# frank-xwang/InstanceDiffusion

Measured on AMD Instinct MI355X. Metric: images/sec at 512x512, 50 PLMS steps, N=8 instances (Multi-instance Sampler), higher is better.
Workload: dtype bf16; 1 GPU; C3: SD-1.5 InstanceDiffusion UNet (1.228B params, seeded random weights), 64x64 latent (512x512), 50 PLMS steps, CFG 7.5, N=8 boxes, MIS 0.36, alpha [0.8,0,0.2]; images_per_gpu=32, unet_forwards_per_image=406

## Files before the change

include/idf.h:

```cpp
#ifndef IDF_H_
#define IDF_H_

#include <stdint.h>

#ifdef __cplusplus
extern "C" {
#endif

#define IDF_ABI_VERSION 5

enum { IDF_BF16 = 0, IDF_F16 = 1 };
enum { IDF_E_ARG = -1, IDF_E_ALIGN = -2, IDF_E_UNSUPPORTED = -3 };

enum {
  IDF_EPI_BIAS     = 1,
  IDF_EPI_ROWBIAS  = 2,
  IDF_EPI_RES      = 4,
  IDF_EPI_GATE     = 8,
  IDF_EPI_SILU     = 16,
  IDF_EPI_GELU     = 32,
  IDF_EPI_GEGLU    = 64,
  IDF_EPI_OUT_F32  = 128,
  IDF_EPI_OUT_NCHW = 256,
  IDF_EPI_LN_ROW   = 512,
  IDF_EPI_LN_COL   = 1024,
  IDF_EPI_GEGLU_P32 = 2048,
  IDF_EPI_QUICKGELU = 4096
};

int idf_abi_version(void);
const char* idf_build_info(void);

enum { IDF_TUNE_GEMM_BIG = 0, IDF_TUNE_ATTN2 = 1, IDF_TUNE_GEMM_RING = 2, IDF_TUNE_BIG_MIN_EFF = 3, IDF_TUNE_ATTN8 = 4, IDF_TUNE_MLP = 5,
       IDF_TUNE_QKV_ROW = 6, IDF_TUNE_GEGLU_ROW = 7, IDF_TUNE_PROJ_ROW = 9  };
int idf_set_tuning(int knob, int value);
enum { IDF_STAT_GEMM_BIG_LAUNCHES = 0, IDF_STAT_ATTN2_LAUNCHES = 1, IDF_STAT_GEMM_RING_LAUNCHES = 2, IDF_STAT_ATTN8_LAUNCHES = 3,
       IDF_STAT_GN_EPI_LAUNCHES = 4 ,
       IDF_STAT_QKV_ROW_LAUNCHES = 6 ,
       IDF_STAT_GEGLU_ROW_LAUNCHES = 7 ,
       IDF_STAT_PROJ_ROW_LAUNCHES = 8 ,
       IDF_STAT_PROJ_ROW_MIN_M = 9 ,
       IDF_STAT_ATTN_RES_LAUNCHES = 10 ,
       IDF_STAT_CLIP_PREPROC_LAUNCHES = 12  };
long long idf_get_stat(int stat);

typedef struct {
  const void* A; const void* W; void* out;
  const float* bias; const void* rowbias; const void* res; const float* gate;
  int M, N, K;
  int lda, ldw, ldo, ldr, ld_rowbias;
  int rows_per_batch;
  int batch; long long strideA, strideW, strideO, strideR;
  int epi; int dtype;
  void* ws; long long ws_bytes;
  const float* ln_stats; long long stride_ln_stats;
  const float* ln_c;
  const float* ln_d;
  float* out_stats; float out_stats_eps;
  float ln_eps; float* ln_stats_out;
  void* vt_out; int ld_vt; int vt_col0;
} idf_gemm_args;
int idf_gemm(const idf_gemm_args* a, void* stream);

typedef struct {
  const void* x; int ldx;
  const float* ln_stats;
  const void* w1; int ldw1;
  const float* cd;
  const void* w2p; int ldw2;
  const float* b2;
  const float* gate;
  void* out; int ldo;
  int M, C;
  int dtype;
} idf_mlp_args;
int idf_mlp_geglu(const idf_mlp_args* a, void* stream);

int idf_row_stats(const void* x, int ldx, float* stats, int M, int C, float eps, int dtype, void* stream);

typedef struct {
  const void* x; const void* W; void* out;
  const float* bias; const void* rowbias; const void* res;
  int B, Hin, Win, Cin, Cout;
  int stride;
  int upsample;
  int ldx, ldo, ldr, ld_rowbias;
  int n_valid;
  int epi; int dtype;
  void* ws; long long ws_bytes;
  float* gn_partial;
} idf_conv3x3_args;
int idf_conv3x3(const idf_conv3x3_args* a, void* stream);
int idf_conv3x3_down(const idf_conv3x3_args* a, void* stream);
int idf_conv_up2x_folded(const idf_conv3x3_args* a, void* stream);

int idf_conv_in(const float* x_nchw, const float* w , const float* bias, void* out,
                int B, int Cin, int H, int W, int Cout, int dtype, void* stream);

typedef struct {
  const void* q; int ldq; long long strideQ; int nq;
  const void* k0; int ldk0; long long strideK0; const void* vt0; int ldv0; long long strideV0; int n0;
  const void* k1; int ldk1; long long strideK1; const void* vt1; int ldv1; long long strideV1; int n1;
  void* out; int ldo; long long strideO;
  int B, H, d;
  float scale;
  int dtype;
  const void* qbits; long long strideQb;
  const void* kbits0; long long strideKb0;
  const void* kbits1; long long strideKb1;
} idf_attn_args;
int idf_attention(const idf_attn_args* a, void* stream);

long long idf_groupnorm_ws_floats(int B, int HW);
int idf_groupnorm(const void* x, void* out, const float* gamma, const float* beta, float* ws,
                  int B, int HW, int C, float eps, int silu, int dtype, void* stream);
int idf_groupnorm_stats(const void* x, float* partial, int B, int HW, int C, int nchunks, int dtype, void* stream);
int idf_groupnorm_apply(const void* x, void* out, const float* gamma, const float* beta, const float* partial,
                        int B, int HW, int C, int nchunks, float eps, int silu, int dtype, void* stream);

int idf_layernorm(const void* x, int ldx, void* out, int ldo, const float* gamma, const float* beta,
                  int M, int C, float eps, int dtype, void* stream);

int idf_layernorm_patch2(const void* x, void* out, int ldo, const float* gamma, const float* beta,
                         int B, int H, int W, int C, float eps, int dtype, void* stream);

int idf_seg_in_conv(const float* segs, const float* w , const float* bias, void* out,
                    int B, int Cin, int S, int ldo, int dtype, void* stream);
int idf_dwconv7x7(const void* x, const float* w_tap_major, const float* bias, void* out, int B, int H, int W, int C,
                  int dtype, void* stream);

int idf_scaleu_concat(const void* h, const void* skip, void* out, const float* hscale, const float* sm1,
                      float* ws, int B, int H, int W, int Ch, int Cs, int dtype, void* stream);

int idf_timestep_embedding(const float* t, void* out, int B, int dim, int dtype, void* stream);

int idf_unifusion_embed(const float* text, const float* loc, const float* tmask, const float* lmask,
                        const float* null_text, const float* null_loc, const float* freqs , void* out,
                        int rows, int text_dim, int D, int dtype, void* stream);

int idf_cfg_combine(const float* eps_cond, const float* eps_uncond, float guidance, float* e_t,
                    long long n, void* stream);
int idf_plms_update(const float* x, const float* e_t, const float* e1, const float* e2, const float* e3,
                    const float* e_next, int mode, float a_t, float a_prev, float sqrt_1m_at,
                    float* x_out, long long n, void* stream);

int idf_ddim_update(const float* x, const float* eps_cond, const float* eps_uncond , float guidance,
                    float a_t, float a_prev, float sigma_t, float sqrt_1m_at, const float* noise ,
                    float* x_prev, float* pred_x0 , long long n, void* stream);
int idf_q_sample_blend(const float* x0, const float* noise, const float* mask, const float* img, float sqrt_ac, float sqrt_1m_ac,
                       float* out, int B, int C, long long HW, int mask_channels , void* stream);
int idf_ddim_update_units(const float* x, const float* eps_cond, const float* eps_uncond , float guidance,
                          float a_t, float a_prev, float sigma_t, float sqrt_1m_at, const float* noise ,
                          const int* img_of , float* x_prev, float* pred_x0 , int U, int B,
                          long long chw, void* stream);
int idf_q_sample_blend_units(const float* x0, const float* noise, const float* mask, const float* img, const int* img_of,
                             float sqrt_ac, float sqrt_1m_ac, float* out, int U, int B, int C, long long HW,
                             int mask_channels , void* stream);

int idf_dpmpp_update(const float* x, const float* eps_cond, const float* eps_uncond , float guidance,
                     float sqrt_at, float sqrt_1m_at, float c_x, float c_0, float c_1,
                     const float* x0_last ,
                     float* x_prev, float* x0_out , long long n, void* stream);

int idf_mis_merge(const float* lat, const int* boxes, float* out, int n_inst, int B, int C, int H, int W,
                  int mode, void* stream);
int idf_mis_merge_ragged(const float* lat, const int* unit_off, const int* boxes , float* out, int B, int U,
                         int C, int H, int W, int mode, void* stream);

int idf_softmax_rows(const float* s, void* p, long long rows, int n, long long lds, long long ldp, float scale,
                     int dtype, void* stream);
int idf_pointwise_nchw(const float* x, const float* w , const float* bias, float* out, int B, int Cin,
                       int Cout, long long HW, float in_scale, void* stream);

int idf_vae_posterior(const float* h, const float* w , const float* bias, const float* noise, float scale, float* z,
                      float* moments, int B, int C2, int E, long long HW, void* stream);

int idf_attention_causal(const void* qkv, int ld, void* out, int ldo, int B, int T, int H, int d, float scale, int dtype, void* stream);
int idf_clip_embed(const int* ids, const void* tok_emb, const void* pos_emb, void* out, int ldo, int B, int T, int C, int vocab,
                   int dtype, void* stream);

#define IDF_ATTENTION_QKV_TMAX 288
int idf_attention_qkv(const void* qkv, int ld, void* out, int ldo, int B, int T, int H, int d, float scale, int dtype, void* stream);
int idf_clip_patchify(const float* pixels, void* patches, int ldp, const void* cls_row, void* x, int ldx, int B, int S, int P, int C,
                      int dtype, void* stream);

enum { IDF_CLIP_SRC_U8 = 0, IDF_CLIP_SRC_F32 = 1 };
#define IDF_CLIP_RESIZE_KMAX 32
int idf_clip_crop_resize(const void* src, int kind, int B, int H, int W, const int* crops, int Ncrop, const int* tables, int Ntab,
                         const float* lut, float* out, int S, int K, void* stream);

int idf_rle_decode_planes(const unsigned* ends, int n_ends, const int* run_begin, const int* run_end, const int* src_hw,
                          const int* dst_plane, int M, float* out, int P, int S, int* area, void* stream);

int idf_cast_f32_to_16(const float* x, void* out, long long n, int dtype, void* stream);

#ifdef __cplusplus
}
#endif
#endif
```

instancediffusion_amd/_lib.py:

```python
from __future__ import annotations

import ctypes as C
import os

_HERE = os.path.dirname(os.path.abspath(__file__))
LIB_PATH = os.environ.get("IDF_LIB_PATH", os.path.join(_HERE, "libidf_gfx950.so"))

IDF_BF16, IDF_F16 = 0, 1
IDF_STAT_GEMM_BIG_LAUNCHES, IDF_STAT_ATTN2_LAUNCHES, IDF_STAT_GEMM_RING_LAUNCHES, IDF_STAT_ATTN8_LAUNCHES, IDF_STAT_GN_EPI_LAUNCHES = 0, 1, 2, 3, 4
IDF_STAT_QKV_ROW_LAUNCHES, IDF_STAT_GEGLU_ROW_LAUNCHES = 6, 7
IDF_STAT_PROJ_ROW_LAUNCHES, IDF_STAT_PROJ_ROW_MIN_M = 8, 9
IDF_STAT_ATTN_RES_LAUNCHES = 10
IDF_STAT_CLIP_PREPROC_LAUNCHES = 12
IDF_CLIP_SRC_U8, IDF_CLIP_SRC_F32 = 0, 1
CLIP_RESIZE_KMAX = 32
IDF_TUNE_PROJ_ROW = 9
IDF_TUNE_GEMM_BIG, IDF_TUNE_ATTN2, IDF_TUNE_GEMM_RING, IDF_TUNE_BIG_MIN_EFF, IDF_TUNE_ATTN8, IDF_TUNE_MLP, IDF_TUNE_QKV_ROW, IDF_TUNE_GEGLU_ROW = 0, 1, 2, 3, 4, 5, 6, 7
EPI_LN_ROW, EPI_LN_COL, EPI_GEGLU_P32, EPI_QUICKGELU = 512, 1024, 2048, 4096
EPI_BIAS, EPI_ROWBIAS, EPI_RES, EPI_GATE, EPI_SILU, EPI_GELU, EPI_GEGLU, EPI_OUT_F32, EPI_OUT_NCHW = \
    1, 2, 4, 8, 16, 32, 64, 128, 256

vp, ll, ci, cf = C.c_void_p, C.c_longlong, C.c_int, C.c_float


class GemmArgs(C.Structure):
    _fields_ = [("A", vp), ("W", vp), ("out", vp), ("bias", vp), ("rowbias", vp), ("res", vp), ("gate", vp),
                ("M", ci), ("N", ci), ("K", ci),
                ("lda", ci), ("ldw", ci), ("ldo", ci), ("ldr", ci), ("ld_rowbias", ci),
                ("rows_per_batch", ci),
                ("batch", ci), ("strideA", ll), ("strideW", ll), ("strideO", ll), ("strideR", ll),
                ("epi", ci), ("dtype", ci), ("ws", vp), ("ws_bytes", ll),
                ("ln_stats", vp), ("stride_ln_stats", ll), ("ln_c", vp), ("ln_d", vp),
                ("out_stats", vp), ("out_stats_eps", cf),
                ("ln_eps", cf), ("ln_stats_out", vp),
                ("vt_out", vp), ("ld_vt", ci), ("vt_col0", ci)]


E_UNSUPPORTED = -3
ATTENTION_QKV_TMAX = 288


class ConvArgs(C.Structure):
    _fields_ = [("x", vp), ("W", vp), ("out", vp), ("bias", vp), ("rowbias", vp), ("res", vp),
                ("B", ci), ("Hin", ci), ("Win", ci), ("Cin", ci), ("Cout", ci),
                ("stride", ci), ("upsample", ci),
                ("ldx", ci), ("ldo", ci), ("ldr", ci), ("ld_rowbias", ci),
                ("n_valid", ci), ("epi", ci), ("dtype", ci), ("ws", vp), ("ws_bytes", ll), ("gn_partial", vp)]


class AttnArgs(C.Structure):
    _fields_ = [("q", vp), ("ldq", ci), ("strideQ", ll), ("nq", ci),
                ("k0", vp), ("ldk0", ci), ("strideK0", ll), ("vt0", vp), ("ldv0", ci), ("strideV0", ll), ("n0", ci),
                ("k1", vp), ("ldk1", ci), ("strideK1", ll), ("vt1", vp), ("ldv1", ci), ("strideV1", ll), ("n1", ci),
                ("out", vp), ("ldo", ci), ("strideO", ll),
                ("B", ci), ("H", ci), ("d", ci), ("scale", cf), ("dtype", ci),
                ("qbits", vp), ("strideQb", ll), ("kbits0", vp), ("strideKb0", ll), ("kbits1", vp), ("strideKb1", ll)]


class MlpArgs(C.Structure):
    _fields_ = [("x", vp), ("ldx", ci), ("ln_stats", vp), ("w1", vp), ("ldw1", ci), ("cd", vp), ("w2p", vp), ("ldw2", ci),
                ("b2", vp), ("gate", vp), ("out", vp), ("ldo", ci), ("M", ci), ("C", ci), ("dtype", ci)]


SYMBOLS = {
    "idf_abi_version": (ci, []),
    "idf_build_info": (C.c_char_p, []),
    "idf_set_tuning": (ci, [ci, ci]),
    "idf_get_stat": (ll, [ci]),
    "idf_gemm": (ci, [C.POINTER(GemmArgs), vp]),
    "idf_conv3x3": (ci, [C.POINTER(ConvArgs), vp]),
    "idf_conv3x3_down": (ci, [C.POINTER(ConvArgs), vp]),
    "idf_conv_up2x_folded": (ci, [C.POINTER(ConvArgs), vp]),
    "idf_mlp_geglu": (ci, [C.POINTER(MlpArgs), vp]),
    "idf_conv_in": (ci, [vp, vp, vp, vp, ci, ci, ci, ci, ci, ci, vp]),
    "idf_attention": (ci, [C.POINTER(AttnArgs), vp]),
    "idf_groupnorm_ws_floats": (ll, [ci, ci]),
    "idf_groupnorm": (ci, [vp, vp, vp, vp, vp, ci, ci, ci, cf, ci, ci, vp]),
    "idf_groupnorm_stats": (ci, [vp, vp, ci, ci, ci, ci, ci, vp]),
    "idf_groupnorm_apply": (ci, [vp, vp, vp, vp, vp, ci, ci, ci, ci, cf, ci, ci, vp]),
    "idf_layernorm": (ci, [vp, ci, vp, ci, vp, vp, ci, ci, cf, ci, vp]),
    "idf_row_stats": (ci, [vp, ci, vp, ci, ci, cf, ci, vp]),
    "idf_layernorm_patch2": (ci, [vp, vp, ci, vp, vp, ci, ci, ci, ci, cf, ci, vp]),
    "idf_seg_in_conv": (ci, [vp, vp, vp, vp, ci, ci, ci, ci, ci, vp]),
    "idf_dwconv7x7": (ci, [vp, vp, vp, vp, ci, ci, ci, ci, ci, vp]),
    "idf_scaleu_concat": (ci, [vp, vp, vp, vp, vp, vp, ci, ci, ci, ci, ci, ci, vp]),
    "idf_timestep_embedding": (ci, [vp, vp, ci, ci, ci, vp]),
    "idf_unifusion_embed": (ci, [vp, vp, vp, vp, vp, vp, vp, vp, ci, ci, ci, ci, vp]),
    "idf_cfg_combine": (ci, [vp, vp, cf, vp, ll, vp]),
    "idf_plms_update": (ci, [vp, vp, vp, vp, vp, vp, ci, cf, cf, cf, vp, ll, vp]),
    "idf_ddim_update": (ci, [vp, vp, vp, cf, cf, cf, cf, cf, vp, vp, vp, ll, vp]),
    "idf_q_sample_blend": (ci, [vp, vp, vp, vp, cf, cf, vp, ci, ci, ll, ci, vp]),
    "idf_ddim_update_units": (ci, [vp, vp, vp, cf, cf, cf, cf, cf, vp, vp, vp, vp, ci, ci, ll, vp]),
    "idf_q_sample_blend_units": (ci, [vp, vp, vp, vp, vp, cf, cf, vp, ci, ci, ci, ll, ci, vp]),
    "idf_dpmpp_update": (ci, [vp, vp, vp, cf, cf, cf, cf, cf, cf, vp, vp, vp, ll, vp]),
    "idf_mis_merge": (ci, [vp, vp, vp, ci, ci, ci, ci, ci, ci, vp]),
    "idf_mis_merge_ragged": (ci, [vp, vp, vp, vp, ci, ci, ci, ci, ci, ci, vp]),
    "idf_cast_f32_to_16": (ci, [vp, vp, ll, ci, vp]),
    "idf_softmax_rows": (ci, [vp, vp, ll, ci, ll, ll, cf, ci, vp]),
    "idf_pointwise_nchw": (ci, [vp, vp, vp, vp, ci, ci, ci, ll, cf, vp]),
    "idf_vae_posterior": (ci, [vp, vp, vp, vp, cf, vp, vp, ci, ci, ci, ll, vp]),
    "idf_attention_causal": (ci, [vp, ci, vp, ci, ci, ci, ci, ci, cf, ci, vp]),
    "idf_clip_embed": (ci, [vp, vp, vp, vp, ci, ci, ci, ci, ci, ci, vp]),
    "idf_attention_qkv": (ci, [vp, ci, vp, ci, ci, ci, ci, ci, cf, ci, vp]),
    "idf_clip_patchify": (ci, [vp, vp, ci, vp, vp, ci, ci, ci, ci, ci, ci, vp]),
    "idf_clip_crop_resize": (ci, [vp, ci, ci, ci, ci, vp, ci, vp, ci, vp, vp, ci, ci, vp]),
    "idf_rle_decode_planes": (ci, [vp, ci, vp, vp, vp, vp, ci, vp, ci, ci, vp, vp]),
}

_lib = None


def load() -> C.CDLL:
    global _lib
    if _lib is not None:
        return _lib
    if not os.path.exists(LIB_PATH):
        raise RuntimeError(
            f"{LIB_PATH} is missing: the MI355X HIP extension has not been built "
            f"(run instancediffusion_amd/csrc/build.sh or __graft_entry__.build()). "
            f"There is no CPU fallback for the InstanceDiffusion sampling path.")
    import torch
    lib = C.CDLL(LIB_PATH)
    for name, (res, args) in SYMBOLS.items():
        fn = getattr(lib, name)
        fn.restype = res
        fn.argtypes = args
    if lib.idf_abi_version() != 5:
        raise RuntimeError("libidf_gfx950.so ABI version mismatch")
    _lib = lib
    return lib


class IdfError(RuntimeError):
    pass


def check(status: int, what: str):
    if status != 0:
        kind = {-1: "invalid argument", -2: "misaligned pointer/leading dimension", -3: "unsupported"}.get(
            status, f"hipError_t {status}")
        raise IdfError(f"{what} failed: {kind}")
```

instancediffusion_amd/csrc/gemm_big.hip:

```cpp
#include "gemm_core.h"
#include <cstdlib>

using namespace idfcore;

namespace {

IDF_ZERO_PAGE(idf_zero_page);

constexpr int WM = 64, TM = 2, NWAVES = 8;

template <int I> struct IC { static constexpr int value = I; };
template <int I, int N, int STEP, class F> __device__ __forceinline__ void static_for(F&& f) {
  if constexpr (I < N) { f(IC<I>{}); static_for<I + STEP, N, STEP>(f); }
}

template <int N, int L>
__device__ __forceinline__ void gst_scatter_step(float* t, int l31) {
  constexpr int H = N / 2;
  const bool up = (l31 & H) != 0;
#pragma unroll
  for (int i = 0; i < H; ++i) {
    const float keep = up ? t[i + H] : t[i];
    const float send = up ? t[i] : t[i + H];
    t[i] = keep + __shfl_xor(send, H, 64);
  }
}
__device__ __forceinline__ void swap16(const f32x16& c, float* v) {
#pragma unroll
  for (int e = 0; e < 4; ++e) {
    const auto s02 = __builtin_amdgcn_permlane32_swap(__float_as_uint(c[e]), __float_as_uint(c[8 + e]), false, false);
    const auto s13 = __builtin_amdgcn_permlane32_swap(__float_as_uint(c[4 + e]), __float_as_uint(c[12 + e]), false, false);
    v[e] = __uint_as_float(s02[0]); v[4 + e] = __uint_as_float(s02[1]);
    v[8 + e] = __uint_as_float(s13[0]); v[12 + e] = __uint_as_float(s13[1]);
  }
}
template <int DT, int BM, int BN, int TN, bool SPLIT, bool LNS = false, bool STATS = false, bool GLU = false, bool GST = false,
          bool QG = true >
__device__ __forceinline__ void big_epilogue(const CoreParams& p, f32x16 (&acc)[TN][TM], int seq, int slice, int tiles_n, int wm,
                                             int wn, int l31_in, int hi_in, float gate, char* stg_in, const float* lnm = nullptr,
                                             const float* lnr = nullptr) {
  constexpr int WN = BN / 2;
  const int epi = p.epi;
  int l31 = l31_in, hi = hi_in;
  asm volatile("" : "+v"(l31), "+v"(hi));
  char* const stg = stg_in;
  const int m_tile = seq / tiles_n;
  const int n0 = (seq - m_tile * tiles_n) * BN, m0 = m_tile * BM;
  const int mw = m0 + wm * WM, nw = n0 + wn * WN;
  if constexpr (LNS) {
    if (p.ln_stats_out && n0 == 0 && wn == 0 && hi == 0) {
#pragma unroll
      for (int b = 0; b < TM; ++b) {
        const int m = mw + b * 32 + l31;
        if (m < p.M) *reinterpret_cast<f32x2*>(p.ln_stats_out + 2 * (size_t)m) = f32x2{lnm[b], lnr[b]};
      }
    }
  }
  if constexpr (SPLIT) {
    static_for<0, TN, 1>([&](auto AI) {
      constexpr int a = decltype(AI)::value;
      const int n = nw + a * 32 + 16 * hi;
#pragma unroll
      for (int b = 0; b < TM; ++b) {
        float v[16];
        swap16(acc[a][b], v);
        const int m = mw + b * 32 + l31;
        if (m >= p.M) continue;
        float* o = p.ws + ((size_t)slice * p.tail_rows + (m - p.tail_m0)) * p.N + n;
#pragma unroll
        for (int j = 0; j < 4; ++j) *reinterpret_cast<f32x4*>(o + 4 * j) = f32x4{v[4 * j], v[4 * j + 1], v[4 * j + 2], v[4 * j + 3]};
      }
    });
    return;
  }
  if (GLU || (((TN & 1) == 0) && (epi & IDF_EPI_GEGLU) && (epi & IDF_EPI_GEGLU_P32))) {
   if constexpr (GLU || ((TN & 1) == 0)) {
#pragma unroll
    for (int b = 0; b < TM; ++b) {
     static_for<0, TN, 1>([&](auto AI) {
      constexpr int a = decltype(AI)::value;
      const int npk = nw + a * 32;
      {
        float o[8];
        f32x2 st = {0.0f, 1.0f};
        if (epi & IDF_EPI_LN_ROW) {
          const int mr = min(mw + b * 32 + l31, p.M - 1);
          if constexpr (LNS) st = f32x2{lnm[b], lnr[b]};
          else st = *reinterpret_cast<const f32x2*>(p.ln_stats + 2 * (size_t)mr);
        }
#pragma unroll
        for (int q = 0; q < 2; ++q) {
          const f32x4 bv = *reinterpret_cast<const f32x4*>(p.bias + npk + 8 * q + 4 * hi);
          const f32x4 bg = *reinterpret_cast<const f32x4*>(p.bias + npk + 16 + 8 * q + 4 * hi);
          f32x4 cv = {0.f, 0.f, 0.f, 0.f}, cg = {0.f, 0.f, 0.f, 0.f};
          if (epi & IDF_EPI_LN_ROW) {
            cv = *reinterpret_cast<const f32x4*>(p.ln_c + npk + 8 * q + 4 * hi);
            cg = *reinterpret_cast<const f32x4*>(p.ln_c + npk + 16 + 8 * q + 4 * hi);
          }
#pragma unroll
          for (int e = 0; e < 4; ++e) {
            float val = acc[a][b][4 * q + e], gat = acc[a][b][4 * (q + 2) + e];
            if (epi & IDF_EPI_LN_ROW) {
              val = fmaf(st[1], fmaf(-st[0], cv[e], val), bv[e]);
              gat = fmaf(st[1], fmaf(-st[0], cg[e], gat), bg[e]);
            } else {
              val += bv[e];
              gat += bg[e];
            }
            o[4 * q + e] = val * gelu_erf_f(gat);
          }
        }
        float v[8];
#pragma unroll
        for (int e = 0; e < 4; ++e) {
          const auto sw = __builtin_amdgcn_permlane32_swap(__float_as_uint(o[e]), __float_as_uint(o[4 + e]), false, false);
          v[e] = __uint_as_float(sw[0]); v[4 + e] = __uint_as_float(sw[1]);
        }
        const int m = mw + b * 32 + l31;
        unsigned short* const obase = reinterpret_cast<unsigned short*>(p.out);
        if (m < p.M) {
          unsigned short* op = obase + (size_t)m * p.ldo + (npk >> 1) + 8 * hi;
          *reinterpret_cast<u32x4*>(op) = pack8<DT>(v);
        }
      }
     });
    }
   }
  } else if (!GLU && (epi & IDF_EPI_GEGLU)) {
    if constexpr (!GLU && (TN & 1) == 0) {
      static_for<0, TN, 2>([&](auto AI) {
        constexpr int a = decltype(AI)::value;
        const int npk = nw + a * 32;
        f32x4 bv[4], bg[4], cv[4], cg[4];
#pragma unroll
        for (int q = 0; q < 4; ++q) {
          bv[q] = *reinterpret_cast<const f32x4*>(p.bias + npk + 8 * q + 4 * hi);
          bg[q] = *reinterpret_cast<const f32x4*>(p.bias + npk + 32 + 8 * q + 4 * hi);
          if (epi & IDF_EPI_LN_ROW) {
            cv[q] = *reinterpret_cast<const f32x4*>(p.ln_c + npk + 8 * q + 4 * hi);
            cg[q] = *reinterpret_cast<const f32x4*>(p.ln_c + npk + 32 + 8 * q + 4 * hi);
          }
        }
#pragma unroll
        for (int b = 0; b < TM; ++b) {
          f32x16 o;
          if (epi & IDF_EPI_LN_ROW) {
            const int mr = min(mw + b * 32 + l31, p.M - 1);
            f32x2 st;
            if constexpr (LNS) st = f32x2{lnm[b], lnr[b]};
            else st = *reinterpret_cast<const f32x2*>(p.ln_stats + 2 * (size_t)mr);
#pragma unroll
            for (int q = 0; q < 4; ++q)
#pragma unroll
              for (int e = 0; e < 4; ++e) {
                const float val = fmaf(st[1], fmaf(-st[0], cv[q][e], acc[a][b][4 * q + e]), bv[q][e]);
                const float gat = fmaf(st[1], fmaf(-st[0], cg[q][e], acc[a + 1][b][4 * q + e]), bg[q][e]);
                o[4 * q + e] = val * gelu_erf_f(gat);
              }
          } else {
#pragma unroll
          for (int q = 0; q < 4; ++q)
#pragma unroll
            for (int e = 0; e < 4; ++e)
              o[4 * q + e] = (acc[a][b][4 * q + e] + bv[q][e]) * gelu_erf_f(acc[a + 1][b][4 * q + e] + bg[q][e]);
          }
          float v[16];
          swap16(o, v);
          const int m = mw + b * 32 + l31;
          if (m < p.M) {
            unsigned short* op = reinterpret_cast<unsigned short*>(p.out) + (size_t)m * p.ldo + (npk >> 1) + 16 * hi;
            *reinterpret_cast<u32x4*>(op) = pack8<DT>(v);
            *reinterpret_cast<u32x4*>(op + 8) = pack8<DT>(v + 8);
          }
        }
      });
    }
  } else if constexpr (!GLU) {
    float st_p[TM], st_s1[TM], st_s2[TM];
#pragma unroll
    for (int b = 0; b < TM; ++b) { st_p[b] = 0.0f; st_s1[b] = 0.0f; st_s2[b] = 0.0f; }
    float gacc[GST ? TN : 1];
    static_for<0, TN, 1>([&](auto AI) {
      constexpr int a = decltype(AI)::value;
      const int n = nw + a * 32 + 16 * hi;
      f32x4 bs[4], cs[4];
      float gt[GST ? 32 : 1];
      if (epi & IDF_EPI_BIAS) {
#pragma unroll
        for (int j = 0; j < 4; ++j) bs[j] = *reinterpret_cast<const f32x4*>(p.bias + n + 4 * j);
      }
      if (epi & IDF_EPI_LN_ROW) {
#pragma unroll
        for (int j = 0; j < 4; ++j) cs[j] = *reinterpret_cast<const f32x4*>(p.ln_c + n + 4 * j);
      }
#pragma unroll
// ... 107 lines not shown
#pragma unroll
      for (int a = 0; a < TN; ++a) csl[(l31 >> 4) * WNC + a * 32 + 16 * hi + (l31 & 15)] = gacc[a];
      asm volatile("s_waitcnt lgkmcnt(0)" ::: "memory");
      __builtin_amdgcn_wave_barrier();
      const int cpg = p.N >> 5;
      const int g = l31 + 32 * hi;
      if (g * cpg < WNC && mw < p.M) {
        constexpr float rows = (float)WM, inv_rows = 1.0f / (float)WM;
        const float inv_cpg = 1.0f / (float)cpg;
        float ms = 0.f, q = 0.f;
        for (int j = 0; j < cpg; ++j) {
          const int col = g * cpg + j;
          const float s1 = csl[col], s2 = csl[WNC + col];
          float pc = (epi & IDF_EPI_BIAS) ? p.bias[nw + col] : 0.0f;
          if (epi & IDF_EPI_ROWBIAS)
            pc += Elem<DT>::to_f32(p.rowbias[(size_t)(mw / p.rows_per_batch) * p.ld_rowbias + nw + col]);
          const float dm = s1 * inv_rows;
          ms += pc + dm;
          q += fmaxf(s2 - s1 * dm, 0.0f);
        }
        const float mean = ms * inv_cpg;
        float dev = 0.f;
        for (int j = 0; j < cpg; ++j) {
          const int col = g * cpg + j;
          float pc = (epi & IDF_EPI_BIAS) ? p.bias[nw + col] : 0.0f;
          if (epi & IDF_EPI_ROWBIAS)
            pc += Elem<DT>::to_f32(p.rowbias[(size_t)(mw / p.rows_per_batch) * p.ld_rowbias + nw + col]);
          const float dd = pc + csl[col] * inv_rows - mean;
          dev = fmaf(dd, dd, dev);
        }
        const int smp = mw / p.gn_hw, chunk = (mw - smp * p.gn_hw) / WM, nch = p.gn_hw / WM;
        *reinterpret_cast<f32x2*>(p.gn_partial + (((size_t)smp * nch + chunk) * 32 + nw / cpg + g) * 2) =
            f32x2{mean, fmaf(rows, dev, q)};
      }
      __builtin_amdgcn_wave_barrier();
    }
    if constexpr (STATS) {
      constexpr float cnt = 16.0f * TN;
      const int n_tile = (seq - m_tile * tiles_n);
#pragma unroll
      for (int b = 0; b < TM; ++b) {
        const float mean = st_p[b] + st_s1[b] * (1.0f / cnt);
        const float m2 = fmaxf(st_s2[b] - st_s1[b] * st_s1[b] * (1.0f / cnt), 0.0f);
        const float mean_o = __shfl_xor(mean, 32, 64), m2_o = __shfl_xor(m2, 32, 64);
        const float dlt = mean_o - mean;
        const int m = mw + b * 32 + l31;
        if (hi == 0 && m < p.M)
          *reinterpret_cast<f32x2*>(p.stat_parts + ((size_t)m * p.parts + n_tile * 2 + wn) * 2) =
              f32x2{0.5f * (mean + mean_o), m2 + m2_o + dlt * dlt * (0.5f * cnt)};
      }
    }
  }
}

template <int DT, int BM, int BN, int TN>
__device__ __forceinline__ void big_epilogue_vt(const CoreParams& p, f32x16 (&acc)[TN][TM], int seq, int tiles_n, int wm, int wn,
                                                int l31, int hi, const float* stats , int stats_row0) {
  constexpr int WN = BN / 2;
  const int epi = p.epi;
  const int m_tile = seq / tiles_n;
  const int n0 = (seq - m_tile * tiles_n) * BN, m0 = m_tile * BM;
  const int mw = m0 + wm * WM, nw = n0 + wn * WN;
  static_for<0, TN, 1>([&](auto AI) {
    constexpr int a = decltype(AI)::value;
    const int n = nw + a * 32 + l31;
    const float cn = (epi & IDF_EPI_LN_ROW) ? p.ln_c[n] : 0.0f;
    const float bn = (epi & IDF_EPI_BIAS) ? p.bias[n] : 0.0f;
    unsigned short* orow = p.vt_out + (size_t)(n - p.vt_col0) * p.ld_vt;
#pragma unroll
    for (int b = 0; b < TM; ++b) {
#pragma unroll
      for (int half = 0; half < 2; ++half) {
        float v[8];
#pragma unroll
        for (int e = 0; e < 4; ++e) {
          const auto sw = __builtin_amdgcn_permlane32_swap(__float_as_uint(acc[a][b][4 * half + e]),
                                                           __float_as_uint(acc[a][b][4 * half + 8 + e]), false, false);
          v[e] = __uint_as_float(sw[0]); v[4 + e] = __uint_as_float(sw[1]);
        }
        const int mb = mw + b * 32 + 16 * hi + 8 * half;
        if (epi & IDF_EPI_LN_ROW) {
          const f32x4* st4 = reinterpret_cast<const f32x4*>(stats + 2 * (size_t)(min(mb, p.M - 8) - stats_row0));
#pragma unroll
          for (int j = 0; j < 4; ++j) {
            const f32x4 t = st4[j];
            v[2 * j] = t[1] * fmaf(-t[0], cn, v[2 * j]);
            v[2 * j + 1] = t[3] * fmaf(-t[2], cn, v[2 * j + 1]);
          }
        }
#pragma unroll
        for (int j = 0; j < 8; ++j) v[j] += bn;
        if (mb < p.M) *reinterpret_cast<u32x4*>(orow + mb) = pack8<DT>(v);
      }
    }
  });
}

template <int DT, int BM, int BN, int TN>
__device__ __forceinline__ void big_epilogue_fold(const CoreParams& p, f32x16 (&acc)[TN][TM], int tile, int ph, int tiles_n, int wm,
                                                  int wn, int l31_in, int hi_in) {
  constexpr int WN = BN / 2;
  int l31 = l31_in, hi = hi_in;
  asm volatile("" : "+v"(l31), "+v"(hi));
  const int m_tile = tile / tiles_n;
  const int n0 = (tile - m_tile * tiles_n) * BN, m0 = m_tile * BM;
  const int mw = m0 + wm * WM, nw = n0 + wn * WN;
  const int ph_row = (ph >> 1) * 2 * p.Wo + (ph & 1);
  unsigned short* orow[TM];
#pragma unroll
  for (int b = 0; b < TM; ++b) {
    const int m = min(mw + b * 32 + l31, p.M - 1);
    const int x = m % p.Wo;
    orow[b] = reinterpret_cast<unsigned short*>(p.out) + (size_t)(4 * m - 2 * x + ph_row) * p.ldo;
  }
  static_for<0, TN, 1>([&](auto AI) {
    constexpr int a = decltype(AI)::value;
    const int n = nw + a * 32 + 16 * hi;
    f32x4 bs[4];
    if (p.epi & IDF_EPI_BIAS) {
#pragma unroll
      for (int j = 0; j < 4; ++j) bs[j] = *reinterpret_cast<const f32x4*>(p.bias + n + 4 * j);
    }
#pragma unroll
    for (int b = 0; b < TM; ++b) {
      float v[16];
      swap16(acc[a][b], v);
      if (p.epi & IDF_EPI_BIAS) {
#pragma unroll
        for (int j = 0; j < 16; ++j) v[j] += bs[j >> 2][j & 3];
      }
      if (mw + b * 32 + l31 < p.M) {
        *reinterpret_cast<u32x4*>(orow[b] + n) = pack8<DT>(v);
        *reinterpret_cast<u32x4*>(orow[b] + n + 8) = pack8<DT>(v + 8);
      }
    }
  });
}

#ifdef IDF_BIG_TRACE
__device__ unsigned long long idf_big_trace_buf[4][8];
#define TR_DECL unsigned long long tr_last = __builtin_readcyclecounter(), tr_acc[8] = {0, 0, 0, 0, 0, 0, 0, 0};
#define TR(i) { const unsigned long long tr_now = __builtin_readcyclecounter(); tr_acc[i] += tr_now - tr_last; tr_last = tr_now; }
#define TR_COUNT(i) { tr_acc[i] += 1; }
#define TR_DUMP { const int trb = blockIdx.x == 0 ? 0 : ((int)blockIdx.x == (int)gridDim.x / 2 ? 1 : -1);                     \
    if (trb >= 0 && lane == 0 && (wave == 0 || wave == NWAVES / 2)) { for (int i = 0; i < 8; ++i) idf_big_trace_buf[trb * 2 + (wave ? 1 : 0)][i] = tr_acc[i]; } }
#else
#define TR_DECL
#define TR(i)
#define TR_COUNT(i)
#define TR_DUMP
#endif

template <int DT, int BM, int BN, int BKT, int NSTG, bool CONV, bool SPLIT, bool LNS = false, bool VT = false, bool STATS = false,
          bool GLU = false, bool GST = false, bool FOLD = false>
__global__ __launch_bounds__(64 * NWAVES, 1) void gemm_kernel_big(const CoreParams p, const int tiles_total) {
  constexpr int WN = BN / 2, TN = WN / 32;
  constexpr int NW = NWAVES;
  constexpr int RS = BKT;
  constexpr int CPR = BKT / 8;
  constexpr int RPI = 64 / CPR;
  constexpr int W_INST = BN / (RPI * NW), A_INST = BM / (RPI * NW);
  constexpr int DPW = W_INST + A_INST;
  constexpr int STAGE = (BM + BN) * RS;
  static_assert(BN % (RPI * NW) == 0 && BM % (RPI * NW) == 0, "tile rows must split evenly over the DMA instructions");
  extern __shared__ __attribute__((aligned(16))) unsigned short smem[];

  const int tid = threadIdx.x;
  const int lane = tid & 63, wave = __builtin_amdgcn_readfirstlane(tid >> 6);
  const int l31 = lane & 31, hi = lane >> 5;
  const int wn = wave & 1, wm = wave >> 1;
  const int G = gridDim.x;
  const int slot = ((G & 7) == 0) ? (int)(blockIdx.x & 7) * (G >> 3) + (int)(blockIdx.x >> 3) : (int)blockIdx.x;
  const int tiles_n = p.N / BN;
  int seq_step = G, seq_end = tiles_total, seq0 = slot;
  if (!SPLIT && p.tile_walk == 1 && tiles_total > G) {
    const int q = tiles_total / G, r = tiles_total - q * G;
    seq0 = slot * q + min(slot, r);
    seq_end = seq0 + q + (slot < r ? 1 : 0);
    seq_step = 1;
  }
  const int S = SPLIT ? p.splitk : 1;
  const int nk = p.kt_per_slice;
  const int full = SPLIT ? p.full_items : tiles_total;
  auto item_map = [&](int item, int& tile, int& slice, int& nki) {
    if (!SPLIT || item < full) { tile = item; slice = 0; nki = SPLIT ? p.kt_full : nk; }
    else { const int r = item - full; const int t = r / S; tile = full + t; slice = r - t * S; nki = nk; }
  };

  const int dr = lane / CPR, dc = lane % CPR;
  auto swz = [](int row) { return CPR == 8 ? ((row >> 1) & 7) : ((row >> 2) & 3); };
  unsigned woff[W_INST], aoff[A_INST];
  int ayx[A_INST];
  int l_seq, l_kt = 0, l_k0 = 0, l_nk = 0, tap = 0, ci0 = 0;

  auto setup_loader = [&](int item) {
    int tile, slice;
    item_map(item, tile, slice, l_nk);
    [[maybe_unused]] int ph = 0;
    if constexpr (FOLD) { ph = tile / p.fold_tiles; tile -= ph * p.fold_tiles; }
    const int m_tile = tile / tiles_n;
    const int n0 = (tile - m_tile * tiles_n) * BN, m0 = m_tile * BM;
    l_k0 = slice * nk;
#pragma unroll
    for (int j = 0; j < W_INST; ++j) {
      const int row = RPI * (wave + NW * j) + dr;
      if constexpr (FOLD) woff[j] = (unsigned)(ph * p.N + n0 + row) * (unsigned)p.ldw + (unsigned)((dc ^ swz(row)) * 8);
      else woff[j] = (unsigned)(n0 + row) * (unsigned)p.ldw + (unsigned)((dc ^ swz(row)) * 8);
    }
#pragma unroll
    for (int j = 0; j < A_INST; ++j) {
      const int row = RPI * (wave + NW * j) + dr;
      const int m = min(m0 + row, p.M - 1);
      const unsigned sw = (unsigned)((dc ^ swz(row)) * 8);
      if (CONV) {
        const auto [b, yo, xo] = conv_pixel(p, m);
        if constexpr (FOLD) {
          const int y0 = yo - 1 + (ph >> 1), x0 = xo - 1 + (ph & 1);
          int mask = 0;
#pragma unroll
          for (int t = 0; t < 4; ++t) {
            const int yi = y0 + (t >> 1), xi = x0 + (t & 1);
            mask |= ((yi >= 0) & (yi < p.Hin) & (xi >= 0) & (xi < p.Win)) << t;
          }
          ayx[j] = mask;
          aoff[j] = (unsigned)b * (unsigned)(p.Hin * p.Win) * (unsigned)p.lda + (unsigned)((y0 * p.Win + x0) * p.lda) + sw;
          continue;
        }
        const int y0 = yo * p.stride - p.pad_lo, x0 = xo * p.stride - p.pad_lo;
        if (p.up == 0) {
          int mask = 0;
#pragma unroll
          for (int t = 0; t < 9; ++t) {
            const int yi = y0 + t / 3, xi = x0 + t % 3;
            mask |= ((yi >= 0) & (yi < p.Hin) & (xi >= 0) & (xi < p.Win)) << t;
          }
          ayx[j] = mask;
          aoff[j] = (unsigned)b * (unsigned)(p.Hin * p.Win) * (unsigned)p.lda + (unsigned)((y0 * p.Win + x0) * p.lda) + sw;
        } else {
          ayx[j] = (y0 << 16) | (x0 & 0xffff);
          aoff[j] = (unsigned)b * (unsigned)(p.Hin * p.Win) * (unsigned)p.lda + sw;
        }
      } else {
        ayx[j] = 0;
        aoff[j] = (unsigned)m * (unsigned)p.lda + sw;
      }
    }
    if (CONV) conv_tap_at(p, l_k0 * BKT, tap, ci0);
  };

  auto issue_piece = [&](int stage, auto II) {
    constexpr int i = decltype(II)::value;
    unsigned short* Al = smem + stage * STAGE;
    if constexpr (i < W_INST) {
      constexpr int j = i;
      dma16_sv(p.W + (size_t)(l_k0 + l_kt) * BKT, woff[j] * 2u, lds_addr(Al + BM * RS + RPI * (wave + NW * j) * RS));
    } else {
      constexpr int j = i - W_INST;
      const unsigned dst = lds_addr(Al + RPI * (wave + NW * j) * RS);
      if constexpr (FOLD) {
        const unsigned tapoff = (unsigned)(((tap >> 1) * p.Win + (tap & 1)) * p.lda + ci0);
        const bool ok = (ayx[j] >> tap) & 1;
        const unsigned short* src = ok ? p.A + (aoff[j] + tapoff) : idf_zero_page + dc * 8;
        dma16_v(src, dst);
      } else if (CONV && p.up == 0) {
        const int ky = tap / 3, kx = tap - ky * 3;
        const unsigned tapoff = (unsigned)((ky * p.Win + kx) * p.lda + ci0);
        const bool ok = (ayx[j] >> tap) & 1;
        const unsigned short* src = ok ? p.A + (aoff[j] + tapoff) : idf_zero_page + dc * 8;
        dma16_v(src, dst);
      } else if (CONV) {
        const int ky = tap / 3, kx = tap - ky * 3;
        const int Hup = p.Hin << p.up, Wup = p.Win << p.up;
        const int yi = (ayx[j] >> 16) + ky, xi = (int)(short)(ayx[j] & 0xffff) + kx;
        const bool ok = conv_tap_inside(yi, xi, Hup, Wup);
        const int ys = yi >> p.up, xs = xi >> p.up;
        const unsigned short* src = ok ? p.A + ci0 + (aoff[j] + (unsigned)(ys * p.Win + xs) * (unsigned)p.lda) : idf_zero_page + dc * 8;
        dma16_v(src, dst);
      } else {
        dma16_sv(p.A + (size_t)(l_k0 + l_kt) * BKT, aoff[j] * 2u, dst);
      }
    }
  };
  auto advance_loader = [&]() {
    if (CONV) conv_tap_step(p, BKT, tap, ci0);
    if (++l_kt == l_nk) {
      l_kt = 0;
      l_seq += seq_step;
      if (l_seq < seq_end) setup_loader(l_seq);
    }
  };
  auto issue_dma = [&](int stage) {
    static_for<0, DPW, 1>([&](auto II) { issue_piece(stage, II); });
    advance_loader();
  };

  const int f_sw = swz(l31);
  int issued = 0;
  constexpr int NPOS = (BKT / 16) * TN;
  constexpr bool OLD_LATE = BN == 320;
  constexpr int LATE_POS = OLD_LATE ? NPOS * 7 / 8 : NPOS / 2;
  auto compute = [&](auto SWAPT, f32x16 (&acc)[TN][TM], float (&lsx)[TM], float (&lsq)[TM], int stage, bool late_fill, int st_fill) {
    constexpr bool SWAP = decltype(SWAPT)::value;
    const unsigned short* Al = smem + stage * STAGE;
    const unsigned short* Wl = Al + BM * RS;
    const unsigned short* af_base = Al + (wm * WM + l31) * RS;
    const unsigned short* wf_base = Wl + (wn * WN + l31) * RS;
    u32x4 wf[2][TN], af[2][TM];
    {
      const int s8 = (hi ^ f_sw) * 8;
#pragma unroll
      for (int a = 0; a < TN; ++a) wf[0][a] = *reinterpret_cast<const u32x4*>(wf_base + a * 32 * RS + s8);
#pragma unroll
      for (int b = 0; b < TM; ++b) af[0][b] = *reinterpret_cast<const u32x4*>(af_base + b * 32 * RS + s8);
    }
    static_for<0, BKT / 16, 1>([&](auto KS) {
      constexpr int ks = decltype(KS)::value;
      constexpr int cur = ks & 1, nxt = cur ^ 1;
      if constexpr (ks + 1 < BKT / 16) {
        const int s8 = (((ks + 1) * 2 + hi) ^ f_sw) * 8;
#pragma unroll
        for (int a = 0; a < TN; ++a) wf[nxt][a] = *reinterpret_cast<const u32x4*>(wf_base + a * 32 * RS + s8);
#pragma unroll
        for (int b = 0; b < TM; ++b) af[nxt][b] = *reinterpret_cast<const u32x4*>(af_base + b * 32 * RS + s8);
      }
      static_for<0, TN, 1>([&](auto AI) {
        constexpr int a = decltype(AI)::value;
        constexpr int pos = ks * TN + a;
#pragma unroll
        for (int b = 0; b < TM; ++b) {
          if constexpr (SWAP) acc[a][b] = Elem<DT>::mfma32(af[cur][b], wf[cur][a], acc[a][b]);
          else acc[a][b] = Elem<DT>::mfma32(wf[cur][a], af[cur][b], acc[a][b]);
        }
        if constexpr (LNS && a == 0) {
#pragma unroll
          for (int b = 0; b < TM; ++b)
#pragma unroll
            for (int w = 0; w < 4; ++w) {
              Elem<DT>::dot2c(lsx[b], af[cur][b][w], Elem<DT>::ONES2);
              Elem<DT>::dot2c(lsq[b], af[cur][b][w], af[cur][b][w]);
            }
        }
        if constexpr (pos == LATE_POS - 1) {
          if (late_fill) static_for<0, DPW, 1>([&](auto II) { issue_piece(st_fill, II); });
        }
      });
    });
    if (late_fill) { advance_loader(); ++issued; }
  };

  int seq = seq0;
  if (seq >= seq_end) return;
  if (p.dephase > 1) {
    const int ph = (int)(blockIdx.x >> 3) % p.dephase;
    const int units = ph * p.dephase_units / p.dephase;
    for (int i = 0; i < units; ++i) __builtin_amdgcn_s_sleep(16);
  }
  l_seq = seq;
  setup_loader(l_seq);
#pragma unroll
  for (int j = 0; j < NSTG - 1; ++j)
    if (l_seq < seq_end) { issue_dma(j); ++issued; }
  int it = 0, st_it = 0;
  int young_stores = 0;
  TR_DECL
  const int epi = p.epi;
  const float gate = (epi & IDF_EPI_GATE) ? p.gate[0] : 0.0f;
  char* const stg = reinterpret_cast<char*>(smem + NSTG * STAGE) + wave * 2048;

  auto run_tile = [&](auto SWAPT, auto SPLT) {
    constexpr bool SWAP = decltype(SWAPT)::value;
    constexpr bool SPL = decltype(SPLT)::value;
    int tile, slice, nki;
    item_map(seq, tile, slice, nki);
    [[maybe_unused]] int ph = 0;
    if constexpr (FOLD) { ph = tile / p.fold_tiles; tile -= ph * p.fold_tiles; }
    f32x16 acc[TN][TM];
    float lsx[TM], lsq[TM];
#pragma unroll
    for (int a = 0; a < TN; ++a)
#pragma unroll
      for (int b = 0; b < TM; ++b)
#pragma unroll
        for (int r = 0; r < 16; ++r) acc[a][b][r] = 0.0f;
#pragma unroll
    for (int b = 0; b < TM; ++b) { lsx[b] = 0.0f; lsq[b] = 0.0f; }
    TR(5) TR_COUNT(7)

    for (int kt = 0; kt < nki; ++kt) {
      if (NSTG > 2 && issued - it == NSTG - 1) asm volatile("s_waitcnt vmcnt(%0)" ::"n"((NSTG - 2) * DPW) : "memory");
      else if (NSTG == 2 && kt == 0 && young_stores > 0) {
        if (young_stores >= 40) asm volatile("s_waitcnt vmcnt(40)" ::: "memory");
        else if (young_stores >= 20) asm volatile("s_waitcnt vmcnt(20)" ::: "memory");
        else if (young_stores >= 16) asm volatile("s_waitcnt vmcnt(16)" ::: "memory");
        else if (young_stores >= 10) asm volatile("s_waitcnt vmcnt(10)" ::: "memory");
        else if (young_stores >= 8) asm volatile("s_waitcnt vmcnt(8)" ::: "memory");
        else asm volatile("s_waitcnt vmcnt(0)" ::: "memory");
      }
      else asm volatile("s_waitcnt vmcnt(0)" ::: "memory");
      TR(0)
      __builtin_amdgcn_s_barrier();
      asm volatile("" ::: "memory");
      TR(1)
      const bool fill = l_seq < seq_end;
      int st_fill = st_it + NSTG - 1;
      if (st_fill >= NSTG) st_fill -= NSTG;
      const bool late = fill && (OLD_LATE ? wave < NW / 2 : wave >= NW / 2);
      if (fill && !late) {
        issue_dma(st_fill);
        ++issued;
      }
      TR(2)
      compute(SWAPT, acc, lsx, lsq, st_it, late, st_fill);
      TR(3) TR_COUNT(6)
      ++it;
      if (++st_it == NSTG) st_it = 0;
    }

    float lnm[TM], lnr[TM];
    if constexpr (LNS) {
      const float inv_k = 1.0f / (float)p.K;
#pragma unroll
      for (int b = 0; b < TM; ++b) {
        const float sx = lsx[b] + __shfl_xor(lsx[b], 32, 64), sq = lsq[b] + __shfl_xor(lsq[b], 32, 64);
        const float mu = sx * inv_k;
        lnm[b] = mu;
        lnr[b] = rsqrtf(fmaxf(fmaf(-mu, mu, sq * inv_k), 0.0f) + p.ln_eps);
      }
    }
    if constexpr (SWAP) {
      if constexpr (LNS) {
        float* stw = reinterpret_cast<float*>(stg);
        if (hi == 0) {
#pragma unroll
          for (int b = 0; b < TM; ++b) *reinterpret_cast<f32x2*>(stw + 2 * (b * 32 + l31)) = f32x2{lnm[b], lnr[b]};
        }
        asm volatile("s_waitcnt lgkmcnt(0)" ::: "memory");
        __builtin_amdgcn_wave_barrier();
        big_epilogue_vt<DT, BM, BN, TN>(p, acc, seq, tiles_n, wm, wn, l31, hi, stw, (seq / tiles_n) * BM + wm * WM);
      } else {
        big_epilogue_vt<DT, BM, BN, TN>(p, acc, seq, tiles_n, wm, wn, l31, hi, p.ln_stats, 0);
      }
    } else if constexpr (FOLD) {
      big_epilogue_fold<DT, BM, BN, TN>(p, acc, tile, ph, tiles_n, wm, wn, l31, hi);
    } else {
      big_epilogue<DT, BM, BN, TN, SPL, LNS, STATS, GLU, GST, !CONV>(p, acc, tile, slice, tiles_n, wm, wn, l31, hi, gate, stg, lnm, lnr);
    }
    TR(4)
    young_stores = 0;
    if (p.epi_vmcnt && (tile / tiles_n) * BM + BM <= p.M) {
      if constexpr (SWAP) young_stores = 2 * TN * TM;
      else if constexpr (SPL) young_stores = 4 * TN * TM;
      else if constexpr (GLU) young_stores = TN * TM;
      else young_stores = (epi & IDF_EPI_GEGLU) ? TN * TM : ((epi & IDF_EPI_OUT_F32) ? 4 * TN * TM : 2 * TN * TM);
    }
  };

  for (; seq < seq_end; seq += seq_step) {
    if constexpr (VT) {
      if ((seq % tiles_n) * BN >= p.vt_col0) run_tile(IC<1>{}, IC<0>{});
      else run_tile(IC<0>{}, IC<0>{});
    } else if constexpr (SPLIT) {
      if (seq < full) run_tile(IC<0>{}, IC<0>{});
      else run_tile(IC<0>{}, IC<1>{});
    } else {
      run_tile(IC<0>{}, IC<0>{});
    }
  }
  TR_DUMP
}

int g_num_cu = 0;

int num_cu() {
  if (g_num_cu == 0) {
    int dev = 0, n = 0;
    if (hipGetDevice(&dev) != hipSuccess || hipDeviceGetAttribute(&n, hipDeviceAttributeMultiprocessorCount, dev) != hipSuccess || n <= 0) n = 256;
    g_num_cu = n;
  }
  return g_num_cu;
}

enum : unsigned { KB_CONV = 1, KB_SPLIT = 2, KB_LNS = 4, KB_VT = 8, KB_STATS = 16, KB_GLU = 32, KB_GST = 64, KB_FOLD = 128 };

template <int DT, int BN, int NSTG, unsigned FLAGS = 0>
int launch_big_cfg(const CoreParams& p, hipStream_t s, int splitk = 1) {
  constexpr int BM = 256, BKT = 64;
  constexpr bool CONV = FLAGS & KB_CONV, SPLIT = FLAGS & KB_SPLIT, LNS = FLAGS & KB_LNS, VT = FLAGS & KB_VT, STATS = FLAGS & KB_STATS,
                 GLU = FLAGS & KB_GLU, GST = FLAGS & KB_GST, FOLD = FLAGS & KB_FOLD;
  if constexpr (!(FLAGS & ~KB_CONV) && NSTG == 2) {
    if (splitk > 1) return launch_big_cfg<DT, BN, NSTG, (FLAGS & KB_CONV) | KB_SPLIT>(p, s, splitk);
  }
  if constexpr (!(FLAGS & (KB_SPLIT | KB_LNS | KB_CONV | KB_STATS | KB_GST)) && NSTG == 2) {
    if ((p.epi & IDF_EPI_LN_ROW) && !p.ln_stats) return launch_big_cfg<DT, BN, NSTG, (FLAGS & (KB_VT | KB_GLU)) | KB_LNS>(p, s, 1);
  }
  void (*kern)(const CoreParams, const int) = gemm_kernel_big<DT, BM, BN, BKT, NSTG, CONV, SPLIT, LNS, VT, STATS, GLU, GST, FOLD>;
  constexpr int smem = NSTG * (BM + BN) * BKT * 2 + NWAVES * 2048;
  static std::atomic<unsigned long long> attr_done{0};
  if (const int e = idf_lds_optin(reinterpret_cast<const void*>(kern), smem, attr_done)) return e;
  CoreParams q = p;
  q.splitk = splitk; q.kt_per_slice = p.K / BKT / splitk; q.kt_full = p.K / BKT;
  const int tiles_all = (p.N / BN) * ((p.M + BM - 1) / BM);
  if (!SPLIT) { q.full_items = tiles_all; q.tail_m0 = 0; q.tail_rows = p.M; }
  int tiles = q.full_items + (tiles_all - q.full_items) * splitk;
  if constexpr (FOLD) { q.fold_tiles = tiles_all; tiles = 4 * tiles_all; }
  const int slots = num_cu();
  const int grid = tiles < slots ? tiles : slots;
  q.tile_walk = !SPLIT && p.N / BN >= 32;
  q.epi_vmcnt = 1;
  q.dephase = 0; q.dephase_units = 0;
  hipLaunchKernelGGL(kern, dim3(grid), dim3(64 * NWAVES), smem, s, q, tiles);
  return idf_launch_status();
}

}

std::atomic<long long> idf_stat_big_launches{0};
int idf_num_cu() { return num_cu(); }

#ifndef IDF_BIG_MIN_EFF_DEFAULT
#define IDF_BIG_MIN_EFF_DEFAULT 50
#endif
int idf_big_min_eff_pct(int set) {
  static int v = -1;
  if (v < 0) {
    const char* e = getenv("IDF_BIG_MIN_EFF");
    const int x = e ? atoi(e) : IDF_BIG_MIN_EFF_DEFAULT;
    v = (x < 1 || x > 100) ? IDF_BIG_MIN_EFF_DEFAULT : x;
  }
  const int prev = v;
  if (set >= 0) v = set;
  return prev;
}

int idf_launch_big(const CoreParams& p, int dtype, bool conv, bool force, hipStream_t s, int* splitk_out, int* parts_out,
                   int* tail_m0_out, int* gst_out) {
  if (gst_out) *gst_out = 0;
  if (splitk_out) *splitk_out = 1;
  if (parts_out) *parts_out = 0;
  if (tail_m0_out) *tail_m0_out = 0;
  const bool geglu = (p.epi & IDF_EPI_GEGLU) != 0;
  if (p.K < 2 * BK || (p.K % BK) != 0) return IDF_BIG_UNSUPPORTED;
  if (p.epi & IDF_EPI_OUT_NCHW) return IDF_BIG_UNSUPPORTED;
  if (p.n_valid != p.N) return IDF_BIG_UNSUPPORTED;
  if ((p.lda % 8) || (p.ldw % 8)) return IDF_BIG_UNSUPPORTED;
  if ((p.ldo % 8) || ((p.epi & IDF_EPI_RES) && (p.ldr % 8)) || ((p.epi & IDF_EPI_ROWBIAS) && (p.ld_rowbias % 8))) return IDF_BIG_UNSUPPORTED;
  if (!aligned16(p.out) || ((p.epi & IDF_EPI_RES) && !aligned16(p.res)) || ((p.epi & IDF_EPI_ROWBIAS) && !aligned16(p.rowbias)) ||
      ((p.epi & (IDF_EPI_BIAS | IDF_EPI_GEGLU)) && !aligned16(p.bias))) return IDF_BIG_UNSUPPORTED;
  if ((p.epi & (IDF_EPI_LN_ROW | IDF_EPI_LN_COL)) && (!aligned16(p.ln_c) || !aligned16(p.ln_stats))) return IDF_BIG_UNSUPPORTED;
  const bool self_ln = (p.epi & IDF_EPI_LN_ROW) && !p.ln_stats;
  if (self_ln && conv) return IDF_BIG_UNSUPPORTED;
  const bool vt = p.vt_out != nullptr;
  if (vt && (conv || geglu || (p.N % 320) || (p.vt_col0 % 320) || p.vt_col0 <= 0 || p.vt_col0 >= p.N || (p.M % 16) || (p.ld_vt % 8) ||
             !aligned16(p.vt_out) || (p.epi & ~(IDF_EPI_BIAS | IDF_EPI_LN_ROW)))) return IDF_BIG_UNSUPPORTED;
  int bn = 0;
  if (geglu && (p.epi & IDF_EPI_GEGLU_P32)) bn = (p.N % 320 == 0) ? 320 : ((p.N % 256 == 0) ? 256 : 0);
  else if (geglu) bn = (p.N % 256 == 0) ? 256 : 0;
  else if (p.N % 320 == 0) bn = 320;
  else if (p.N % 256 == 0) bn = 256;
  else if (p.N % 128 == 0 && !self_ln) bn = 128;
  if (!bn) return IDF_BIG_UNSUPPORTED;
  const int bm = 256;
  const long long slots = (long long)num_cu();
  const long long tiles = (long long)(p.N / bn) * ((p.M + bm - 1) / bm);
  int splitk = 1;
  if (splitk_out && bn != 128 && !geglu && !self_ln && !vt && p.ws && tiles * 2 <= slots) {
    const int nkt = p.K / BK;
    for (int cand = (int)(slots / tiles); cand >= 2; --cand) {
      if (nkt % cand || nkt / cand < 16) continue;
      if ((size_t)cand * p.M * p.N * sizeof(float) > p.ws_bytes) continue;
      splitk = cand;
      break;
    }
  }
  long long full_items = 0;
  int tail_m0 = 0;
  if (!force) {
    const long long items = tiles * splitk;
    const long long rounds = (items + slots - 1) / slots;
    const double eff = (double)items / (double)(rounds * slots);
    if (eff * 100.0 < (double)idf_big_min_eff_pct(-1)) {
      const int tiles_n = p.N / bn;
      const long long whole = ((tiles / slots) * slots / tiles_n) * tiles_n;
      const long long rem = tiles - whole;
      const int nkt = p.K / BK;
      int S = 0;
      if (splitk == 1 && splitk_out && tail_m0_out && whole > 0 && rem > 0 && bn != 128 && !geglu && !self_ln && !vt && p.ws)
        for (int cand = (int)(slots / rem); cand >= 2; --cand) {
          if (nkt % cand || nkt / cand < 4) continue;
          S = cand;
          break;
        }
      tail_m0 = (int)(whole / tiles_n) * bm;
      if (S < 2 || (size_t)S * (size_t)(p.M - tail_m0) * p.N * sizeof(float) > p.ws_bytes) return IDF_BIG_UNSUPPORTED;
      full_items = whole;
      splitk = S;
    }
  }
  if (splitk_out) *splitk_out = splitk;
  if (tail_m0_out) *tail_m0_out = tail_m0;
  {
    const unsigned long long rows = conv ? (unsigned long long)(p.M / (p.Ho * p.Wo)) * p.Hin * p.Win : (unsigned long long)p.M;
    if (rows * (unsigned long long)p.lda >= (1ull << 31) || (unsigned long long)p.N * p.ldw >= (1ull << 31)) return IDF_BIG_UNSUPPORTED;
  }
  ++idf_stat_big_launches;
  const bool stats = parts_out && p.stat_parts && !conv && !geglu && !vt && !self_ln && splitk == 1 && bn != 128 &&
                     !(p.epi & IDF_EPI_OUT_F32) && (((uintptr_t)p.stat_parts) & 7u) == 0 &&
                     (size_t)p.M * (size_t)(2 * (p.N / bn)) * 2 * sizeof(float) <= p.ws_bytes;
  CoreParams ps = p;
  if (stats) { ps.parts = 2 * (p.N / bn); *parts_out = ps.parts; }
  const bool gst = gst_out && p.gn_partial && conv && bn == 320 && splitk == 1 && full_items == 0 && !(p.epi & IDF_EPI_OUT_F32) &&
                   p.gn_hw > 0 && (p.gn_hw % 64) == 0 && (p.M % p.gn_hw) == 0 && (p.N % 32) == 0 && (160 % (p.N / 32)) == 0 &&
                   (((uintptr_t)p.gn_partial) & 7u) == 0;
  if (gst) *gst_out = 1;
  CoreParams pq = p;
  pq.full_items = (int)full_items; pq.tail_m0 = tail_m0; pq.tail_rows = p.M - tail_m0;
  const bool glu320 = geglu && (p.epi & IDF_EPI_GEGLU_P32) && bn == 320;
#define IDF_BIG_DISPATCH(DT)                                                                                              \
  if (glu320) return launch_big_cfg<DT, 320, 2, KB_GLU>(p, s);                                                            \
  if (stats) return bn == 320 ? launch_big_cfg<DT, 320, 2, KB_STATS>(ps, s) : launch_big_cfg<DT, 256, 2, KB_STATS>(ps, s); \
  if (vt) return launch_big_cfg<DT, 320, 2, KB_VT>(p, s);                                                                 \
  if (bn == 128) {                         \
    if (conv) return launch_big_cfg<DT, 128, 3, KB_CONV>(p, s);                                                           \
    return launch_big_cfg<DT, 128, 3>(p, s);                                                                              \
  }                                                                                                                       \
  if (gst) return launch_big_cfg<DT, 320, 2, KB_CONV | KB_GST>(p, s);                                                     \
  if (conv) return bn == 320 ? launch_big_cfg<DT, 320, 2, KB_CONV>(pq, s, splitk) : launch_big_cfg<DT, 256, 2, KB_CONV>(pq, s, splitk);   \
  return bn == 320 ? launch_big_cfg<DT, 320, 2>(pq, s, splitk) : launch_big_cfg<DT, 256, 2>(pq, s, splitk);
  if (dtype == IDF_BF16) { IDF_BIG_DISPATCH(IDF_BF16) }
  if (dtype == IDF_F16) { IDF_BIG_DISPATCH(IDF_F16) }
#undef IDF_BIG_DISPATCH
  return IDF_E_UNSUPPORTED;
}

int idf_launch_big_fold(const CoreParams& p, int dtype, bool force, hipStream_t s) {
  if (p.Cin <= 0 || (p.Cin % BK) != 0 || p.K != 4 * p.Cin || p.ldw != p.K) return IDF_BIG_UNSUPPORTED;
  if ((p.N % 320) != 0 || p.n_valid != p.N || (p.epi & ~IDF_EPI_BIAS)) return IDF_BIG_UNSUPPORTED;
  if ((p.lda % 8) || (p.ldo % 8) || !aligned16(p.A) || !aligned16(p.W) || !aligned16(p.out)) return IDF_BIG_UNSUPPORTED;
  if ((p.epi & IDF_EPI_BIAS) && !aligned16(p.bias)) return IDF_BIG_UNSUPPORTED;
  if (p.Ho != p.Hin || p.Wo != p.Win || p.M <= 0 || (p.M % (p.Hin * p.Win)) != 0) return IDF_BIG_UNSUPPORTED;
  const long long slots = (long long)num_cu();
  const long long items = 4ll * (p.N / 320) * ((p.M + 255) / 256);
  if (!force) {
    const long long rounds = (items + slots - 1) / slots;
    if ((double)items / (double)(rounds * slots) * 100.0 < (double)idf_big_min_eff_pct(-1)) return IDF_BIG_UNSUPPORTED;
  }
  if ((unsigned long long)p.M * (unsigned long long)p.lda >= (1ull << 31) || 4ull * p.N * p.ldw >= (1ull << 31) ||
      items >= (1ll << 30) || (unsigned long long)p.M * 4ull >= (1ull << 31)) return IDF_BIG_UNSUPPORTED;
  ++idf_stat_big_launches;
  if (dtype == IDF_BF16) return launch_big_cfg<IDF_BF16, 320, 2, KB_CONV | KB_FOLD>(p, s);
  if (dtype == IDF_F16) return launch_big_cfg<IDF_F16, 320, 2, KB_CONV | KB_FOLD>(p, s);
  return IDF_E_UNSUPPORTED;
}
```

instancediffusion_amd/csrc/gemm_conv.hip:

```cpp
#include "gemm_core.h"
#include "attn_core.h"
#include <cstdlib>
extern std::atomic<long long> idf_stat_clip_preproc_launches;

using namespace idfcore;

namespace {

#ifndef IDF_GEMM_BIG_DEFAULT
#define IDF_GEMM_BIG_DEFAULT 1
#endif
constexpr int LSTR = 72;

template <int BM, int BN, int WM, int WN> constexpr int dma_lds_bytes(int stages) {
  const int kloop = stages * (BM + BN) * 64 * 2, cstage = 4 * WM * (WN + 4) * 4;
  return kloop > cstage ? kloop : cstage;
}

template <int DT, int BM, int BN, int WM, int WN, int KLOOP_LDS_BYTES>
__device__ __forceinline__ void tile_epilogue(const CoreParams& p, f32x16 (&acc)[WN / 32][WM / 32], unsigned short* smem,
                                              int m0, int n0, int bz, int wm, int wn, int lane, int wave) {
  constexpr int TM = WM / 32, TN = WN / 32;
  const int l31 = lane & 31, hi = lane >> 5;
  constexpr int CSTR = WN + 4;
// ... 247 lines not shown
    ktile_mfma<DT, TN, TM, RS, true>(acc, Al + BM * RS + (wn * WN + l31) * RS, Al + (wm * WM + l31) * RS, hi, f_sw);
  };

  dma_tile(0, 0);
  __syncthreads();
  for (int kt = 0; kt < nk; ++kt) {
    if (kt + 1 < nk) dma_tile(kt + 1, (kt + 1) & 1);
    compute(kt & 1);
    __syncthreads();
  }
  tile_epilogue<DT, BM, BN, WM, WN, dma_lds_bytes<BM, BN, WM, WN>(2)>(p, acc, smem, t.m0, t.n0, t.bz, wm, wn, lane, wave);
}

IDF_ZERO_PAGE(ring_zero_page);

template <int PT, int MAXA> __device__ __forceinline__ void ring_wait(int ahead) {
  if constexpr (MAXA <= 0) {
    asm volatile("s_waitcnt vmcnt(0)" ::: "memory");
  } else {
    static_assert(MAXA * PT < 64, "vmcnt is a 6-bit field");
    if (ahead >= MAXA) asm volatile("s_waitcnt vmcnt(%0)" ::"n"(MAXA * PT) : "memory");
    else ring_wait<PT, MAXA - 1>(ahead);
  }
}

template <int DT, int BM, int BN, int WM, int WN, bool CONV, int NS>
__global__ __launch_bounds__(256, 1) void gemm_kernel_ring(const CoreParams p) {
  constexpr int TM = WM / 32, TN = WN / 32;
  constexpr int WAVES_N = BN / WN;
  constexpr int RS = 64;
  constexpr int BUF = (BM + BN) * RS;
  constexpr int W_INST = BN / 8 / 4, A_INST = BM / 8 / 4;
  constexpr int PER_TILE = W_INST + A_INST;
  constexpr int LDS_BYTES = dma_lds_bytes<BM, BN, WM, WN>(NS);
  static_assert((BM / WM) * (BN / WN) == 4, "4 waves per workgroup");
  static_assert(NS >= 3 && LDS_BYTES <= 160 * 1024, "ring must fit the CU's LDS");
  extern __shared__ __attribute__((aligned(16))) unsigned short smem[];

  const int tid = threadIdx.x;
  const int lane = tid & 63, wave = __builtin_amdgcn_readfirstlane(tid >> 6);
  const int l31 = lane & 31, hi = lane >> 5;
  const int wn = wave % WAVES_N, wm = wave / WAVES_N;
  TileSlice t;
  tile_slice<BM, BN>(p, xcd_tile(blockIdx.x, gridDim.x), t);
  const int nk = t.nk;

  const int dc = lane & 7;
  const unsigned short* wsrc[W_INST];
  dma_src_rows(wsrc, t.Wb, p.ldw, t.n0, p.N, (size_t)t.kt_begin * BK, wave, lane);
  const unsigned short* asrc[A_INST];
  [[maybe_unused]] int ay[A_INST], ax[A_INST];
  int tap = 0, ci0 = 0;
  if constexpr (!CONV) {
    dma_src_rows(asrc, t.Ab, p.lda, t.m0, p.M, (size_t)t.kt_begin * BK, wave, lane);
  } else {
#pragma unroll
    for (int j = 0; j < A_INST; ++j) {
      const int row = dma_row(wave, j, lane);
      const int m = min(t.m0 + row, p.M - 1);
      asrc[j] = t.Ab + conv_row_origin(p, m, ay[j], ax[j]) + dma_chunk(row, lane);
    }
    conv_tap_at(p, t.kt_begin * BK, tap, ci0);
  }
  int kt_issue = 0, st_issue = 0;

  auto issue_tile = [&]() {
    unsigned short* Al = smem + st_issue * BUF;
    unsigned short* Wl = Al + BM * RS;
#pragma unroll
    for (int j = 0; j < W_INST; ++j) dma16_v(wsrc[j] + (size_t)kt_issue * BK, lds_addr(Wl + 8 * (wave + 4 * j) * RS));
    if constexpr (!CONV) {
#pragma unroll
      for (int j = 0; j < A_INST; ++j) dma16_v(asrc[j] + (size_t)kt_issue * BK, lds_addr(Al + 8 * (wave + 4 * j) * RS));
    } else {
      const int ky = tap / 3, kx = tap - ky * 3;
      const int Hup = p.Hin << p.up, Wup = p.Win << p.up;
#pragma unroll
      for (int j = 0; j < A_INST; ++j) {
        const int yi = ay[j] + ky, xi = ax[j] + kx;
        const bool ok = conv_tap_inside(yi, xi, Hup, Wup);
        const int ys = yi >> p.up, xs = xi >> p.up;
        const unsigned short* src = ok ? asrc[j] + ((size_t)ys * p.Win + xs) * p.lda + ci0 : ring_zero_page + dc * 8;
        dma16_v(src, lds_addr(Al + 8 * (wave + 4 * j) * RS));
      }
      conv_tap_step(p, BK, tap, ci0);
    }
    ++kt_issue;
    st_issue = (st_issue + 1 == NS) ? 0 : st_issue + 1;
  };

  f32x16 acc[TN][TM];
  clear_acc(acc);
  const int f_sw = (l31 >> 1) & 7;
  auto compute = [&](int st) {
    const unsigned short* Al = smem + st * BUF;
    ktile_mfma<DT, TN, TM, RS, true>(acc, Al + BM * RS + (wn * WN + l31) * RS, Al + (wm * WM + l31) * RS, hi, f_sw);
  };

  const int pre = min(NS - 1, nk);
  for (int i = 0; i < pre; ++i) issue_tile();
  int st = 0;
  for (int kt = 0; kt < nk; ++kt) {
    ring_wait<PER_TILE, NS - 2>(kt_issue - kt - 1);
    __builtin_amdgcn_s_barrier();
    if (kt_issue < nk) issue_tile();
    compute(st);
    st = (st + 1 == NS) ? 0 : st + 1;
  }
  tile_epilogue<DT, BM, BN, WM, WN, LDS_BYTES>(p, acc, smem, t.m0, t.n0, t.bz, wm, wn, lane, wave);
}

template <int DT>
__global__ __launch_bounds__(256) void splitk_reduce_kernel(const CoreParams p) {
  const int n8 = (p.N + 7) / 8;
  const size_t i = (size_t)blockIdx.x * 256 + threadIdx.x;
  if (i >= (size_t)p.tail_rows * n8) return;
  const int ml = (int)(i / n8), n = (int)(i - (size_t)ml * n8) * 8;
  const int m = p.tail_m0 + ml;
  float v[8] = {0.f, 0.f, 0.f, 0.f, 0.f, 0.f, 0.f, 0.f};
  const bool vec = (n + 7 < p.N) && ((p.N & 3) == 0);
  const size_t slab = (size_t)p.tail_rows * p.N;
  const float* w = p.ws + (size_t)ml * p.N + n;
  if (vec) {
    int s = 0;
    for (; s + 4 <= p.splitk; s += 4) {
      f32x4 a[4][2];
#pragma unroll
      for (int u = 0; u < 4; ++u) {
        a[u][0] = *reinterpret_cast<const f32x4*>(w + (size_t)(s + u) * slab);
        a[u][1] = *reinterpret_cast<const f32x4*>(w + (size_t)(s + u) * slab + 4);
      }
#pragma unroll
      for (int u = 0; u < 4; ++u)
#pragma unroll
        for (int e = 0; e < 4; ++e) { v[e] += a[u][0][e]; v[e + 4] += a[u][1][e]; }
    }
    for (; s < p.splitk; ++s) {
      const f32x4 w0 = *reinterpret_cast<const f32x4*>(w + (size_t)s * slab), w1 = *reinterpret_cast<const f32x4*>(w + (size_t)s * slab + 4);
#pragma unroll
      for (int e = 0; e < 4; ++e) { v[e] += w0[e]; v[e + 4] += w1[e]; }
    }
  } else {
    for (int s = 0; s < p.splitk; ++s) {
#pragma unroll
      for (int e = 0; e < 8; ++e) if (n + e < p.N) v[e] += w[(size_t)s * slab + e];
    }
  }
  const float gate = (p.epi & IDF_EPI_GATE) ? p.gate[0] : 0.0f;
  epilogue8<DT>(p, 0, m, n, v, gate);
}

std::atomic<long long> idf_stat_gn_epi_launches{0};
std::atomic<long long> idf_stat_ring_launches{0};
std::atomic<long long> idf_stat_gegluw_launches{0};
std::atomic<long long> idf_stat_qkvw_launches{0};
std::atomic<long long> idf_stat_projw_launches{0};
int g_big_mode = -2;
inline int gemm_big_mode() {
  if (g_big_mode == -2) {
    const char* e = getenv("IDF_GEMM_BIG");
    const int v = e ? atoi(e) : IDF_GEMM_BIG_DEFAULT;
    g_big_mode = (v < 0 || v > 3) ? IDF_GEMM_BIG_DEFAULT : v;
  }
  return g_big_mode;
}

template <int DT>
void launch_reduce(const CoreParams& q, hipStream_t s) {
  const size_t n8 = (size_t)q.tail_rows * ((q.N + 7) / 8);
  hipLaunchKernelGGL(splitk_reduce_kernel<DT>, dim3((unsigned)((n8 + 255) / 256)), dim3(256), 0, s, q);
}

template <int DT, int BM, int BN, void (*KERN)(const CoreParams), int SMEM>
int launch_kloop(const CoreParams& p, int batch, int want, hipStream_t s, std::atomic<long long>* launches = nullptr) {
  static std::atomic<unsigned long long> attr_done{0};
  if (const int e = idf_lds_optin(reinterpret_cast<const void*>(KERN), SMEM, attr_done)) return e;
  CoreParams q = p;
  const int tiles = ((p.N + BN - 1) / BN) * ((p.M + BM - 1) / BM);
  const int nk = p.K / BK;
  q.splitk = 1; q.kt_per_slice = nk;
  q.tail_m0 = 0; q.tail_rows = p.M;
  while (want > 1 && (size_t)want * p.M * p.N * sizeof(float) > p.ws_bytes) --want;
  if (want > 1) {
    q.kt_per_slice = (nk + want - 1) / want;
    q.splitk = (nk + q.kt_per_slice - 1) / q.kt_per_slice;
  }
  dim3 grid(tiles, 1, q.splitk > 1 ? q.splitk : batch);
  hipLaunchKernelGGL(KERN, grid, dim3(256), SMEM, s, q);
  if (launches) ++*launches;
  if (q.splitk > 1) launch_reduce<DT>(q, s);
  return idf_launch_status();
}

template <int DT, int BM, int BN, int WM, int WN, bool CONV>
int launch_cfg(const CoreParams& p, int batch, hipStream_t s) {
  const int tiles = ((p.N + BN - 1) / BN) * ((p.M + BM - 1) / BM);
  const int nk = p.K / BK;
  int want = 1;
  if (batch == 1 && p.ws && !(p.epi & IDF_EPI_GEGLU) && tiles < 192 && nk >= 8) {
    want = (512 + tiles - 1) / tiles;
    if (want > nk / 4) want = nk / 4;
    if (want > 64) want = 64;
  }
  if constexpr (CONV) return launch_kloop<DT, BM, BN, gemm_kernel<DT, BM, BN, WM, WN>, 2 * (BM + BN) * LSTR * 2>(p, batch, want, s);
  else return launch_kloop<DT, BM, BN, gemm_kernel_dma<DT, BM, BN, WM, WN>, dma_lds_bytes<BM, BN, WM, WN>(2)>(p, batch, want, s);
}

#ifndef IDF_GEMM_RING_DEFAULT
#define IDF_GEMM_RING_DEFAULT 256
#endif
int g_ring_tiles = -1;
inline int gemm_ring_tiles() {
  if (g_ring_tiles < 0) {
    const char* e = getenv("IDF_GEMM_RING");
    const int v = e ? atoi(e) : IDF_GEMM_RING_DEFAULT;
    g_ring_tiles = v < 0 ? IDF_GEMM_RING_DEFAULT : v;
  }
  return g_ring_tiles;
}

constexpr int RING_SLICE_KT = 8;

template <int DT, int BM, int BN, int WM, int WN, bool CONV, int NS>
int launch_ring_cfg(const CoreParams& p, int batch, hipStream_t s) {
  const int tiles = ((p.N + BN - 1) / BN) * ((p.M + BM - 1) / BM);
  const int nk = p.K / BK;
  if ((long long)tiles * batch > gemm_ring_tiles()) return IDF_BIG_UNSUPPORTED;
  const int slots = idf_num_cu();
  if (batch == 1 && p.ws && !(p.epi & IDF_EPI_GEGLU) && tiles * 2 > slots && tiles < 192 && nk >= 8) return IDF_BIG_UNSUPPORTED;
  int want = 1;
  if (batch == 1 && p.ws && !(p.epi & IDF_EPI_GEGLU) && tiles * 2 <= slots && nk >= 2 * RING_SLICE_KT) {
    want = slots / tiles;
    if (want > nk / RING_SLICE_KT) want = nk / RING_SLICE_KT;
    if (want > 64) want = 64;
  }
  return launch_kloop<DT, BM, BN, gemm_kernel_ring<DT, BM, BN, WM, WN, CONV, NS>, dma_lds_bytes<BM, BN, WM, WN>(NS)>(
      p, batch, want, s, &idf_stat_ring_launches);
}

template <int DT, bool CONV>
int launch(const CoreParams& p, int batch, hipStream_t s, int* parts_out = nullptr, int* gst_out = nullptr) {
  const bool geglu = (p.epi & IDF_EPI_GEGLU) != 0;
  constexpr bool use_wide = CONV;
  const int big = gemm_big_mode();
  const bool t128p = geglu || (p.N % 128 == 0) || p.N > 1024 || (use_wide && p.N > 128);
  const long long tiles_small = (long long)((p.N + (t128p ? 127 : 63)) / (t128p ? 128 : 64)) * ((p.M + 127) / 128);
  const bool ring_first = big != 2 && gemm_ring_tiles() > 0 && tiles_small <= 128 && tiles_small <= gemm_ring_tiles();
  if (big > 0 && batch == 1 && !ring_first) {
    int splitk = 1, tail_m0 = 0;
    const int rc = idf_launch_big(p, DT, CONV, big == 2, s, &splitk, parts_out, big == 3 ? &tail_m0 : nullptr, gst_out);
    if (rc != IDF_BIG_UNSUPPORTED) {
      if (rc == 0 && splitk > 1) {
        CoreParams q = p;
        q.splitk = splitk; q.tail_m0 = tail_m0; q.tail_rows = p.M - tail_m0;
        launch_reduce<DT>(q, s);
        return idf_launch_status();
      }
      return rc;
    }
  }
  CoreParams q = p;
  if ((p.epi & IDF_EPI_LN_ROW) && !p.ln_stats) {
    float* st = p.ln_stats_out ? p.ln_stats_out : p.ws;
    if (!st || (!p.ln_stats_out && p.ws_bytes < (size_t)p.M * 2 * sizeof(float))) return IDF_E_ARG;
    const int rc = idf_row_stats(p.A, p.lda, st, p.M, p.K, p.ln_eps, DT, s);
    if (rc) return rc;
    q.ln_stats = st; q.stride_ln_stats = 0;
    if (!p.ln_stats_out) { q.ws = nullptr; q.ws_bytes = 0; }
  }
  const bool t128 = geglu || (q.N % 128 == 0) || q.N > 1024 || (use_wide && q.N > 128);
  if (gemm_ring_tiles() > 0) {
    const int rc = t128 ? launch_ring_cfg<DT, 128, 128, 64, 64, CONV, 4>(q, batch, s) : launch_ring_cfg<DT, 128, 64, 64, 32, CONV, 5>(q, batch, s);
    if (rc != IDF_BIG_UNSUPPORTED) return rc;
  }
  if (t128) return launch_cfg<DT, 128, 128, 64, 64, CONV>(q, batch, s);
  return launch_cfg<DT, 128, 64, 64, 32, CONV>(q, batch, s);
}

template <bool CONV>
int launch_dt(int dtype, const CoreParams& p, int batch, hipStream_t s, int* parts_out = nullptr, int* gst_out = nullptr) {
  if (dtype == IDF_BF16) return launch<IDF_BF16, CONV>(p, batch, s, parts_out, gst_out);
  if (dtype == IDF_F16) return launch<IDF_F16, CONV>(p, batch, s, parts_out, gst_out);
  return IDF_E_UNSUPPORTED;
}

}

__global__ __launch_bounds__(256) void stats_finalize_kernel(const float* __restrict__ parts, int P, float cols, float* __restrict__ out,
                                                            int M, float eps) {
  const int m = blockIdx.x * 256 + threadIdx.x;
  if (m >= M) return;
  const f32x2* pp = reinterpret_cast<const f32x2*>(parts) + (size_t)m * P;
  f32x2 t = pp[0];
  float mean = t[0], m2 = t[1], n = cols;
  for (int i = 1; i < P; ++i) {
    t = pp[i];
    const float dlt = t[0] - mean, nn = n + cols;
    mean += dlt * (cols / nn);
    m2 += t[1] + dlt * dlt * (n * cols / nn);
    n = nn;
  }
  reinterpret_cast<f32x2*>(out)[m] = f32x2{mean, rsqrtf(m2 / n + eps)};
}

int idf_stats_finalize(const float* stat_parts, int parts, int cols_per_part, float* out_stats, int M, float eps, hipStream_t s) {
  hipLaunchKernelGGL(stats_finalize_kernel, dim3((M + 255) / 256), dim3(256), 0, s, stat_parts, parts, (float)cols_per_part,
                     out_stats, M, eps);
  return idf_launch_status();
}

extern "C" int idf_set_tuning(int knob, int value) {
  if (knob == IDF_TUNE_GEMM_BIG) {
    if (value < 0 || value > 3) return IDF_E_ARG;
    const int prev = gemm_big_mode();
    g_big_mode = value;
    return prev;
  }
  if (knob == IDF_TUNE_GEMM_RING) {
    if (value < 0) return IDF_E_ARG;
    const int prev = gemm_ring_tiles();
    g_ring_tiles = value;
    return prev;
  }
  if (knob == IDF_TUNE_BIG_MIN_EFF) {
    if (value < 1 || value > 100) return IDF_E_ARG;
    return idf_big_min_eff_pct(value);
  }
  if (knob == IDF_TUNE_ATTN2) {
    if (value < 0 || value > 6) return IDF_E_ARG;
    return idf_attn2_set_mode(value);
  }
  if (knob == IDF_TUNE_ATTN8) {
    if (value < 0 || value > 6) return IDF_E_ARG;
    return idf_attn8_set_mode(value);
  }
  if (knob == IDF_TUNE_GEGLU_ROW) {
    if (value < 0 || value > 1) return IDF_E_ARG;
    return idf_gegluw_set_mode(value);
  }
  if (knob == IDF_TUNE_QKV_ROW) {
    if (value < 0 || value > 1) return IDF_E_ARG;
    return idf_qkvw_set_mode(value);
  }
  if (knob == IDF_TUNE_PROJ_ROW) {
    if (value < 0 || value > 1) return IDF_E_ARG;
    return idf_projw_set_mode(value);
  }
  if (knob == IDF_TUNE_MLP) {
    if (value < 0 || value > 1) return IDF_E_ARG;
    return idf_mlp_set_mode(value);
  }
  return IDF_E_ARG;
}

extern "C" long long idf_get_stat(int stat) {
  if (stat == IDF_STAT_GEMM_BIG_LAUNCHES) return idf_stat_big_launches.load();
  if (stat == IDF_STAT_ATTN2_LAUNCHES) return idf_stat_attn2_launches.load();
  if (stat == IDF_STAT_GEMM_RING_LAUNCHES) return idf_stat_ring_launches.load();
  if (stat == IDF_STAT_ATTN8_LAUNCHES) return idf_stat_attn8_launches.load();
  if (stat == IDF_STAT_GN_EPI_LAUNCHES) return idf_stat_gn_epi_launches.load();
  if (stat == IDF_STAT_QKV_ROW_LAUNCHES) return idf_stat_qkvw_launches.load();
  if (stat == IDF_STAT_GEGLU_ROW_LAUNCHES) return idf_stat_gegluw_launches.load();
  if (stat == IDF_STAT_PROJ_ROW_LAUNCHES) return idf_stat_projw_launches.load();
  if (stat == IDF_STAT_PROJ_ROW_MIN_M) return gemm_big_mode() > 0 ? idf_projw_min_rows() : 0;
  if (stat == IDF_STAT_ATTN_RES_LAUNCHES) return idf_stat_attn_res_launches.load();
  if (stat == IDF_STAT_CLIP_PREPROC_LAUNCHES) return idf_stat_clip_preproc_launches.load();
  return -1;
}

extern "C" int idf_gemm(const idf_gemm_args* a, void* stream) {
  if (!a || !a->A || !a->W || !a->out) return IDF_E_ARG;
  if (a->M <= 0 || a->N <= 0 || a->K <= 0 || (a->K % BK) != 0) return IDF_E_ARG;
  if ((a->lda % 8) || (a->ldw % 8) || !aligned16(a->A) || !aligned16(a->W)) return IDF_E_ALIGN;
  if ((a->epi & IDF_EPI_GATE) && !(a->epi & IDF_EPI_RES)) return IDF_E_ARG;
  if ((a->epi & IDF_EPI_RES) && !a->res) return IDF_E_ARG;
  if ((a->epi & (IDF_EPI_BIAS | IDF_EPI_GEGLU)) && !a->bias) return IDF_E_ARG;
  if ((a->epi & IDF_EPI_GEGLU) && ((a->N % 64) || (a->ldo % 4))) return IDF_E_ARG;
  if ((a->epi & IDF_EPI_GEGLU_P32) && !(a->epi & IDF_EPI_GEGLU)) return IDF_E_ARG;
  if ((a->epi & IDF_EPI_ROWBIAS) && (!a->rowbias || a->rows_per_batch <= 0)) return IDF_E_ARG;
  if (a->epi & IDF_EPI_OUT_NCHW) return IDF_E_ARG;
  if ((a->epi & IDF_EPI_QUICKGELU) && (a->epi & (IDF_EPI_SILU | IDF_EPI_GELU | IDF_EPI_GEGLU))) return IDF_E_ARG;
  CoreParams p{};
  p.W = (const unsigned short*)a->W; p.ldw = a->ldw; p.strideW = a->strideW; p.N = a->N;
  p.A = (const unsigned short*)a->A; p.lda = a->lda; p.strideA = a->strideA; p.M = a->M; p.K = a->K;
  p.out = a->out; p.ldo = a->ldo; p.strideO = a->strideO;
  p.bias = a->bias; p.rowbias = (const unsigned short*)a->rowbias; p.ld_rowbias = a->ld_rowbias;
  p.rows_per_batch = a->rows_per_batch;
  p.res = (const unsigned short*)a->res; p.ldr = a->ldr; p.strideR = a->strideR;
  p.gate = a->gate; p.epi = a->epi; p.n_valid = a->N;
  p.ws = (float*)a->ws; p.ws_bytes = a->ws ? (size_t)a->ws_bytes : 0;
  const int batch = a->batch > 0 ? a->batch : 1;
  if (a->epi & (IDF_EPI_LN_ROW | IDF_EPI_LN_COL)) {
    if ((a->epi & IDF_EPI_LN_ROW) && (a->epi & IDF_EPI_LN_COL)) return IDF_E_ARG;
    if (!a->ln_c) return IDF_E_ARG;
    if (!a->ln_stats) {
      if (!(a->epi & IDF_EPI_LN_ROW) || batch != 1 || (a->K % 8) || a->K > 1536 || !(a->ln_eps > 0.0f)) return IDF_E_ARG;
      if (a->ln_stats_out && (((uintptr_t)a->ln_stats_out) & 7u)) return IDF_E_ALIGN;
      p.ln_eps = a->ln_eps; p.ln_stats_out = a->ln_stats_out;
    }
    if ((a->epi & IDF_EPI_LN_ROW) && !(a->epi & IDF_EPI_BIAS)) return IDF_E_ARG;
    if ((a->epi & IDF_EPI_LN_COL) && (!a->ln_d || (a->epi & IDF_EPI_GEGLU))) return IDF_E_ARG;
    if ((((uintptr_t)a->ln_stats) & 7u) || (a->stride_ln_stats & 1)) return IDF_E_ALIGN;
    p.ln_stats = a->ln_stats; p.stride_ln_stats = a->stride_ln_stats; p.ln_c = a->ln_c; p.ln_d = a->ln_d;
  }
  if (a->out_stats) {
    if ((a->epi & (IDF_EPI_GEGLU | IDF_EPI_OUT_F32)) || (a->N % 8) || a->N > 1536 || (a->ldo % 8)) return IDF_E_ARG;
    if (batch > 1 && a->strideO != (long long)a->M * a->ldo) return IDF_E_ARG;
  }
  hipStream_t s = (hipStream_t)stream;
  int rc = IDF_E_UNSUPPORTED;
  if (a->vt_out) {
    const int Nv = a->N - a->vt_col0;
    if (a->vt_col0 <= 0 || Nv <= 0 || batch != 1 || a->ld_vt < a->M || (a->ld_vt % 8) || !aligned16(a->vt_out)) return IDF_E_ARG;
    if (a->epi & ~(IDF_EPI_BIAS | IDF_EPI_LN_ROW)) return IDF_E_ARG;
    if (!(a->epi & IDF_EPI_LN_ROW)) return IDF_E_ARG;
    if (a->out_stats) return IDF_E_ARG;
    const bool self_ln = (a->epi & IDF_EPI_LN_ROW) && !a->ln_stats;
    if (self_ln && !a->ln_stats_out) return IDF_E_ARG;
    p.vt_out = (unsigned short*)a->vt_out; p.ld_vt = a->ld_vt; p.vt_col0 = a->vt_col0;
    if (gemm_big_mode() > 0) {
      int r = idf_launch_qkv320w(p, a->dtype, s);
      if (r == IDF_BIG_UNSUPPORTED) r = idf_launch_qkv640w(p, a->dtype, s);
      if (r != IDF_BIG_UNSUPPORTED) { if (r == 0) { ++idf_stat_big_launches; ++idf_stat_qkvw_launches; } return r; }
    }
    if (gemm_big_mode() > 0) {
      const int r = idf_launch_big(p, a->dtype, false, gemm_big_mode() == 2, s, nullptr);
      if (r != IDF_BIG_UNSUPPORTED) return r;
    }
    CoreParams p1 = p;
    p1.vt_out = nullptr; p1.vt_col0 = 0; p1.N = a->vt_col0; p1.n_valid = a->vt_col0;
    rc = launch_dt<false>(a->dtype, p1, 1, s);
    if (rc) return rc;
    CoreParams p2{};
    p2.A = p.W + (size_t)a->vt_col0 * p.ldw; p2.lda = p.ldw; p2.M = Nv; p2.K = a->K;
    p2.W = p.A; p2.ldw = p.lda; p2.N = a->M; p2.n_valid = a->M;
    p2.out = a->vt_out; p2.ldo = a->ld_vt;
    p2.ws = p.ws; p2.ws_bytes = p.ws_bytes;
    p2.epi = 0;
    if (a->epi & IDF_EPI_LN_ROW) {
      p2.epi |= IDF_EPI_LN_COL;
      p2.ln_stats = self_ln ? a->ln_stats_out : a->ln_stats; p2.stride_ln_stats = 0;
      p2.ln_c = a->ln_c + a->vt_col0; p2.ln_d = a->bias + a->vt_col0;
    }
    return launch_dt<false>(a->dtype, p2, 1, s);
  }
  int parts = 0;
  if ((a->epi & IDF_EPI_GEGLU) && batch == 1 && !a->out_stats && gemm_big_mode() > 0) {
    const int r = idf_launch_geglu640w(p, a->dtype, s);
    if (r != IDF_BIG_UNSUPPORTED) { if (r == 0) { ++idf_stat_big_launches; ++idf_stat_gegluw_launches; } return r; }
  }
  if (batch == 1 && gemm_big_mode() > 0) {
    const int r = idf_launch_proj320s(p, a->dtype, a->out_stats, a->out_stats_eps, s);
    if (r != IDF_BIG_UNSUPPORTED) { if (r == 0) { ++idf_stat_big_launches; ++idf_stat_projw_launches; } return r; }
  }
  if (a->out_stats && batch == 1 && p.ws) p.stat_parts = p.ws;
  rc = launch_dt<false>(a->dtype, p, batch, s, &parts);
  if (rc == 0 && a->out_stats) {
    if (parts > 0) rc = idf_stats_finalize(p.stat_parts, parts, a->N / parts, a->out_stats, a->M, a->out_stats_eps, s);
    else rc = idf_row_stats(a->out, a->ldo, a->out_stats, batch * a->M, a->N, a->out_stats_eps, a->dtype, stream);
  }
  return rc;
}

static int conv3x3_launch(const idf_conv3x3_args* a, int pad_lo, void* stream) {
  if (!a || !a->x || !a->W || !a->out) return IDF_E_ARG;
  if (a->B <= 0 || a->Cin <= 0 || (a->Cin % BK) != 0 || a->Cout <= 0) return IDF_E_ARG;
  if (a->stride != 1 && a->stride != 2) return IDF_E_ARG;
  if (a->upsample != 0 && a->upsample != 1) return IDF_E_ARG;
  if ((a->ldx % 8) || !aligned16(a->x) || !aligned16(a->W)) return IDF_E_ALIGN;
  if (a->epi & (IDF_EPI_GEGLU | IDF_EPI_GATE | IDF_EPI_QUICKGELU)) return IDF_E_ARG;
  if ((a->epi & IDF_EPI_RES) && !a->res) return IDF_E_ARG;
  if ((a->epi & IDF_EPI_BIAS) && !a->bias) return IDF_E_ARG;
  CoreParams p{};
  const int Hup = a->Hin << a->upsample, Wup = a->Win << a->upsample;
  p.Ho = (Hup + pad_lo - 2) / a->stride + 1; p.Wo = (Wup + pad_lo - 2) / a->stride + 1;
  p.W = (const unsigned short*)a->W; p.ldw = 9 * a->Cin; p.strideW = 0; p.N = a->Cout;
  p.A = (const unsigned short*)a->x; p.lda = a->ldx; p.strideA = 0; p.M = a->B * p.Ho * p.Wo; p.K = 9 * a->Cin;
  p.Hin = a->Hin; p.Win = a->Win; p.Cin = a->Cin; p.stride = a->stride; p.up = a->upsample; p.pad_lo = pad_lo;
  p.out = a->out; p.ldo = a->ldo; p.strideO = 0;
  p.bias = a->bias; p.rowbias = (const unsigned short*)a->rowbias; p.ld_rowbias = a->ld_rowbias;
  p.rows_per_batch = p.Ho * p.Wo;
  p.res = (const unsigned short*)a->res; p.ldr = a->ldr; p.strideR = 0;
  p.gate = nullptr; p.epi = a->epi; p.n_valid = a->n_valid > 0 ? a->n_valid : a->Cout;
  p.ws = (float*)a->ws; p.ws_bytes = a->ws ? (size_t)a->ws_bytes : 0;
  if ((a->epi & IDF_EPI_ROWBIAS) && !a->rowbias) return IDF_E_ARG;
  hipStream_t s = (hipStream_t)stream;
  if (a->gn_partial) {
    const int hw = p.Ho * p.Wo;
    if ((hw % 64) || (a->Cout % 32) || a->ldo != a->Cout || (a->epi & (IDF_EPI_OUT_F32 | IDF_EPI_OUT_NCHW))) return IDF_E_ARG;
    if (((uintptr_t)a->gn_partial) & 7u) return IDF_E_ALIGN;
    p.gn_partial = a->gn_partial; p.gn_hw = hw;
  }
  int gst = 0;
  int rc = launch_dt<true>(a->dtype, p, 1, s, nullptr, &gst);
  if (rc == 0 && gst) ++idf_stat_gn_epi_launches;
  if (rc == 0 && a->gn_partial && !gst)
    rc = idf_groupnorm_stats(a->out, a->gn_partial, a->B, p.Ho * p.Wo, a->Cout, p.Ho * p.Wo / 64, a->dtype, stream);
  return rc;
}

extern "C" int idf_conv3x3(const idf_conv3x3_args* a, void* stream) { return conv3x3_launch(a, 1, stream); }

extern "C" int idf_conv3x3_down(const idf_conv3x3_args* a, void* stream) {
  if (!a || a->stride != 2 || a->upsample != 0 || a->Hin < 2 || a->Win < 2) return IDF_E_ARG;
  return conv3x3_launch(a, 0, stream);
}

extern "C" int idf_conv_up2x_folded(const idf_conv3x3_args* a, void* stream) {
  if (!a || !a->x || !a->W || !a->out) return IDF_E_ARG;
  if (a->B <= 0 || a->Hin <= 0 || a->Win <= 0 || a->Cin <= 0 || (a->Cin % BK) != 0 || a->Cout <= 0) return IDF_E_ARG;
  if (a->stride != 1 || a->upsample != 1) return IDF_E_ARG;
  if ((a->epi & ~IDF_EPI_BIAS) || a->rowbias || a->res || a->gn_partial || a->n_valid) return IDF_E_ARG;
  if ((a->epi & IDF_EPI_BIAS) && !a->bias) return IDF_E_ARG;
  if ((a->ldx % 8) || (a->ldo % 8) || !aligned16(a->x) || !aligned16(a->W) || !aligned16(a->out)) return IDF_E_ALIGN;
  if (a->dtype != IDF_BF16 && a->dtype != IDF_F16) return IDF_E_UNSUPPORTED;
  const int big = gemm_big_mode();
  if (big == 0) return IDF_E_UNSUPPORTED;
  CoreParams p{};
  p.W = (const unsigned short*)a->W; p.ldw = 4 * a->Cin; p.N = a->Cout; p.n_valid = a->Cout;
  p.A = (const unsigned short*)a->x; p.lda = a->ldx; p.K = 4 * a->Cin;
  p.Hin = a->Hin; p.Win = a->Win; p.Cin = a->Cin; p.Ho = a->Hin; p.Wo = a->Win; p.stride = 1; p.up = 0; p.pad_lo = 1;
  p.M = a->B * a->Hin * a->Win;
  p.out = a->out; p.ldo = a->ldo; p.bias = a->bias; p.epi = a->epi; p.rows_per_batch = a->Hin * a->Win;
  const int rc = idf_launch_big_fold(p, a->dtype, big == 2, (hipStream_t)stream);
  return rc == IDF_BIG_UNSUPPORTED ? IDF_E_UNSUPPORTED : rc;
}
```

instancediffusion_amd/csrc/gemm_core.h:

```cpp
#pragma once
#include "common.h"
#include <atomic>

namespace idfcore {

struct CoreParams {
  const unsigned short* W; int ldw; long long strideW; int N;
  const unsigned short* A; int lda; long long strideA; int M; int K;
  int Hin, Win, Cin, Ho, Wo, stride, up;
  void* out; int ldo; long long strideO;
  const float* bias; const unsigned short* rowbias; int ld_rowbias; int rows_per_batch;
  const unsigned short* res; int ldr; long long strideR;
  const float* gate; int epi; int n_valid;
  float* ws; size_t ws_bytes; int splitk; int kt_per_slice;
  int full_items; int kt_full; int tail_m0; int tail_rows;
  const float* ln_stats; long long stride_ln_stats; const float* ln_c; const float* ln_d;
  float ln_eps; float* ln_stats_out;
  unsigned short* vt_out; int ld_vt; int vt_col0;
  float* stat_parts; int parts;
  float* gn_partial; int gn_hw;
  int tile_walk; int dephase; int dephase_units; int epi_vmcnt;
  int pad_lo;
  int fold_tiles;
};

constexpr int BK = 64;

__device__ __forceinline__ int xcd_tile(int L, int T) {
  const int q = T >> 3, r = T & 7, xcd = L & 7, i = L >> 3;
  return (xcd < r ? xcd * (q + 1) : r * (q + 1) + (xcd - r) * q) + i;
}
struct TileSlice { int m0, n0, bz; const unsigned short* Wb; const unsigned short* Ab; int kt_begin, nk; };
template <int BM, int BN>
__device__ __forceinline__ void tile_slice(const CoreParams& p, int tile, TileSlice& t) {
  const int tiles_n = (p.N + BN - 1) / BN;
  const int m_tile = tile / tiles_n;
  t.n0 = (tile - m_tile * tiles_n) * BN, t.m0 = m_tile * BM;
  t.bz = (p.splitk > 1) ? 0 : blockIdx.z;
  t.Wb = p.W + (size_t)t.bz * p.strideW;
  t.Ab = p.A + (size_t)t.bz * p.strideA;
  const int nk_all = p.K / BK;
  t.kt_begin = (p.splitk > 1) ? blockIdx.z * p.kt_per_slice : 0;
  t.nk = (p.splitk > 1) ? min(p.kt_per_slice, nk_all - t.kt_begin) : nk_all;
}

struct ConvPixel { int b, yo, xo; };
__device__ __forceinline__ ConvPixel conv_pixel(const CoreParams& p, int m) {
  const int hw = p.Ho * p.Wo;
  const int b = m / hw, rem = m - b * hw;
  const int yo = rem / p.Wo;
  return {b, yo, rem - yo * p.Wo};
}
__device__ __forceinline__ size_t conv_row_origin(const CoreParams& p, int m, int& ay, int& ax) {
  const ConvPixel px = conv_pixel(p, m);
  ay = px.yo * p.stride - p.pad_lo;
  ax = px.xo * p.stride - p.pad_lo;
  return (size_t)px.b * p.Hin * p.Win * p.lda;
}
__device__ __forceinline__ void conv_tap_at(const CoreParams& p, int k_elem, int& tap, int& ci0) {
  tap = k_elem / p.Cin;
  ci0 = k_elem - tap * p.Cin;
}
__device__ __forceinline__ void conv_tap_step(const CoreParams& p, int bk, int& tap, int& ci0) {
  ci0 += bk;
  if (ci0 >= p.Cin) { ci0 = 0; ++tap; }
}
__device__ __forceinline__ bool conv_tap_inside(int yi, int xi, int Hup, int Wup) { return (yi >= 0) & (yi < Hup) & (xi >= 0) & (xi < Wup); }

__device__ __forceinline__ int dma_row(int wave, int j, int lane) { return 8 * (wave + 4 * j) + (lane >> 3); }
__device__ __forceinline__ int dma_chunk(int row, int lane) { return ((lane & 7) ^ ((row >> 1) & 7)) * 8; }
__device__ __forceinline__ const unsigned short* dma_src_row(const unsigned short* base, int ld, int r0, int rows, size_t k0, int wave,
                                                             int j, int lane) {
  const int row = dma_row(wave, j, lane);
  const int n = min(r0 + row, rows - 1);
  return base + (size_t)n * ld + k0 + dma_chunk(row, lane);
}
template <int INST>
__device__ __forceinline__ void dma_src_rows(const unsigned short* (&src)[INST], const unsigned short* base, int ld, int r0, int rows,
                                             size_t k0, int wave, int lane) {
#pragma unroll
  for (int j = 0; j < INST; ++j) src[j] = dma_src_row(base, ld, r0, rows, k0, wave, j, lane);
}

template <int TN, int TM>
__device__ __forceinline__ void clear_acc(f32x16 (&acc)[TN][TM]) {
#pragma unroll
  for (int a = 0; a < TN; ++a)
#pragma unroll
    for (int b = 0; b < TM; ++b)
#pragma unroll
      for (int r = 0; r < 16; ++r) acc[a][b][r] = 0.0f;
}
template <int DT, int TN, int TM, int RS, bool SWZ>
__device__ __forceinline__ void ktile_mfma(f32x16 (&acc)[TN][TM], const unsigned short* wf_base, const unsigned short* af_base, int hi,
                                           int f_sw) {
  u32x4 wf[2][TN], af[2][TM];
  {
    const int slot = SWZ ? (hi ^ f_sw) * 8 : hi * 8;
#pragma unroll
    for (int a = 0; a < TN; ++a) wf[0][a] = *reinterpret_cast<const u32x4*>(wf_base + a * 32 * RS + slot);
#pragma unroll
    for (int b = 0; b < TM; ++b) af[0][b] = *reinterpret_cast<const u32x4*>(af_base + b * 32 * RS + slot);
  }
#pragma unroll
  for (int ks = 0; ks < BK / 16; ++ks) {
    const int cur = ks & 1, nxt = cur ^ 1;
    if (ks + 1 < BK / 16) {
      const int slot = SWZ ? (((ks + 1) * 2 + hi) ^ f_sw) * 8 : (ks + 1) * 16 + hi * 8;
#pragma unroll
      for (int a = 0; a < TN; ++a) wf[nxt][a] = *reinterpret_cast<const u32x4*>(wf_base + a * 32 * RS + slot);
#pragma unroll
      for (int b = 0; b < TM; ++b) af[nxt][b] = *reinterpret_cast<const u32x4*>(af_base + b * 32 * RS + slot);
    }
#pragma unroll
    for (int a = 0; a < TN; ++a)
#pragma unroll
      for (int b = 0; b < TM; ++b) acc[a][b] = Elem<DT>::mfma32(wf[cur][a], af[cur][b], acc[a][b]);
  }
}

template <int DT>
__device__ __forceinline__ void epilogue8(const CoreParams& p, int bz, int m, int n, float* v, float gate) {
  const int epi = p.epi;
  const bool full = (n + 7 < p.N);
  if (epi & IDF_EPI_LN_ROW) {
    const f32x2 st = *reinterpret_cast<const f32x2*>(p.ln_stats + (size_t)bz * p.stride_ln_stats + 2 * (size_t)m);
#pragma unroll
    for (int e = 0; e < 8; ++e) if (n + e < p.N) v[e] = st[1] * fmaf(-st[0], p.ln_c[n + e], v[e]);
  }
  if (epi & IDF_EPI_LN_COL) {
    const float cm = p.ln_c[m], dm = p.ln_d[m];
    const float* st = p.ln_stats + (size_t)bz * p.stride_ln_stats + 2 * (size_t)n;
#pragma unroll
    for (int e = 0; e < 8; ++e) if (n + e < p.N) v[e] = fmaf(st[2 * e + 1], fmaf(-cm, st[2 * e], v[e]), dm);
  }
  if (epi & IDF_EPI_BIAS) {
    if (full) {
      const f32x4 b0 = *reinterpret_cast<const f32x4*>(p.bias + n), b1 = *reinterpret_cast<const f32x4*>(p.bias + n + 4);
#pragma unroll
      for (int e = 0; e < 4; ++e) { v[e] += b0[e]; v[e + 4] += b1[e]; }
    } else {
#pragma unroll
      for (int e = 0; e < 8; ++e) if (n + e < p.N) v[e] += p.bias[n + e];
    }
  }
  if (epi & IDF_EPI_ROWBIAS) {
    const unsigned short* rb = p.rowbias + (size_t)(m / p.rows_per_batch) * p.ld_rowbias + n;
    if (full && ((p.ld_rowbias & 7) == 0)) {
      float r[8];
      unpack8<DT>(*reinterpret_cast<const u32x4*>(rb), r);
#pragma unroll
      for (int e = 0; e < 8; ++e) v[e] += r[e];
    } else {
#pragma unroll
      for (int e = 0; e < 8; ++e) if (n + e < p.N) v[e] += Elem<DT>::to_f32(rb[e]);
    }
  }
  if (epi & IDF_EPI_SILU) {
#pragma unroll
    for (int e = 0; e < 8; ++e) v[e] = silu_f(v[e]);
  }
  if (epi & IDF_EPI_GELU) {
#pragma unroll
    for (int e = 0; e < 8; ++e) v[e] = gelu_erf_f(v[e]);
  }
  if (epi & IDF_EPI_QUICKGELU) {
#pragma unroll
    for (int e = 0; e < 8; ++e) v[e] = quick_gelu_f(v[e]);
  }
  if (epi & IDF_EPI_RES) {
    const unsigned short* rr = p.res + (size_t)bz * p.strideR + (size_t)m * p.ldr + n;
    const float gm = (epi & IDF_EPI_GATE) ? gate : 1.0f;
    if (full && ((p.ldr & 7) == 0)) {
      float r[8];
      unpack8<DT>(*reinterpret_cast<const u32x4*>(rr), r);
#pragma unroll
      for (int e = 0; e < 8; ++e) v[e] = fmaf(gm, v[e], r[e]);
    } else {
#pragma unroll
      for (int e = 0; e < 8; ++e) if (n + e < p.N) v[e] = fmaf(gm, v[e], Elem<DT>::to_f32(rr[e]));
    }
  }
  if (epi & IDF_EPI_OUT_NCHW) {
    const int hw = p.Ho * p.Wo;
    const int bb = m / hw, rem = m - bb * hw;
    float* o = reinterpret_cast<float*>(p.out);
#pragma unroll
    for (int e = 0; e < 8; ++e)
      if (n + e < p.n_valid) o[((size_t)bb * p.n_valid + (n + e)) * hw + rem] = v[e];
  } else if (epi & IDF_EPI_OUT_F32) {
    float* o = reinterpret_cast<float*>(p.out) + (size_t)bz * p.strideO + (size_t)m * p.ldo + n;
    if (full && ((p.ldo & 3) == 0)) {
      *reinterpret_cast<f32x4*>(o) = f32x4{v[0], v[1], v[2], v[3]};
      *reinterpret_cast<f32x4*>(o + 4) = f32x4{v[4], v[5], v[6], v[7]};
    } else {
#pragma unroll
      for (int e = 0; e < 8; ++e) if (n + e < p.N) o[e] = v[e];
    }
  } else {
    unsigned short* o = reinterpret_cast<unsigned short*>(p.out) + (size_t)bz * p.strideO + (size_t)m * p.ldo + n;
    if (full && ((p.ldo & 7) == 0)) {
      *reinterpret_cast<u32x4*>(o) = pack8<DT>(v);
    } else {
#pragma unroll
      for (int e = 0; e < 8; ++e) if (n + e < p.N) o[e] = Elem<DT>::from_f32(v[e]);
    }
  }
}

}

#define IDF_BIG_UNSUPPORTED (-100)
extern std::atomic<long long> idf_stat_big_launches;
int idf_launch_big(const idfcore::CoreParams& p, int dtype, bool conv, bool force, hipStream_t s, int* splitk_out,
                   int* parts_out = nullptr, int* tail_m0_out = nullptr, int* gst_out = nullptr);
int idf_launch_big_fold(const idfcore::CoreParams& p, int dtype, bool force, hipStream_t s);
int idf_launch_qkv320w(const idfcore::CoreParams& p, int dtype, hipStream_t s);
int idf_launch_geglu640w(const idfcore::CoreParams& p, int dtype, hipStream_t s);
// ... 11 lines not shown
```

instancediffusion_amd/engine.py:

```python
from __future__ import annotations

import dataclasses
import os
from typing import Dict, List, Optional, Sequence, Tuple

import torch

from .engine_base import EngineBase, _Lin, capture_graph, pack_conv3x3
from .host.attention import SpatialTransformer
from .host.unet import Downsample, ResBlock, UNetModel, Upsample


OBJ_TOKENS = 184
MASK_RES = 64


def _round_up(x: int, m: int) -> int:
    return (x + m - 1) // m * m


@dataclasses.dataclass(frozen=True)
class EngineKnobs:
    ln_self: int = 1
    qkv_row: bool = True
    geglu_period: int = 32
    mlp_fused: bool = True
    mlp_min_m: int = 32768
    pair_hoist: bool = True
    gn_epi: bool = True
    up_fold: bool = True
    vt_global: bool = True
    vt_min_n: int = 256
    debug_paired: bool = False

    _ENV = (("ln_self", "IDF_LN_SELF", "1", int), ("qkv_row", "IDF_QKV_ROW", "1", lambda s: s != "0"), ("geglu_period", "IDF_GEGLU_PERIOD", "32", int),
            ("mlp_fused", "IDF_MLP_FUSED", "1", bool), ("mlp_min_m", "IDF_MLP_MIN_M", "32768", int), ("pair_hoist", "IDF_PAIR_HOIST", "1", bool),
            ("gn_epi", "IDF_GN_EPI", "1", bool), ("up_fold", "IDF_UP_FOLD", "1", bool), ("vt_global", "IDF_VT_GLOBAL", "1", lambda s: s != "0"),
            ("vt_min_n", "IDF_VT_MIN_N", "256", int), ("debug_paired", "IDF_DEBUG_PAIRED", "0", lambda s: s == "1"))

    def __post_init__(self):
        if self.ln_self not in (0, 1, 2):
            raise ValueError(f"IDF_LN_SELF={self.ln_self}: must be 0, 1 or 2")
        if self.geglu_period not in (32, 64):
            raise ValueError(f"IDF_GEGLU_PERIOD={self.geglu_period}: must be 32 or 64")
        if self.mlp_fused and self.geglu_period != 32:
            raise ValueError("mlp_fused needs geglu_period 32 (the fused kernel's operand images are packed from it)")
        if self.vt_min_n < 64 or self.vt_min_n % 64:
            raise ValueError(f"IDF_VT_MIN_N={self.vt_min_n}: a positive multiple of 64 (tokens per sample from which the fused "
                             "q | k | v launch is used; default 256)")

    @classmethod
    def from_env(cls) -> "EngineKnobs":
        v = {}
        for field, env, default, parse in cls._ENV:
            raw = os.environ.get(env, default)
            if parse is bool and raw not in ("0", "1"):
                raise ValueError(f"{env}={raw}: must be 0 or 1")
            v[field] = raw == "1" if parse is bool else parse(raw)
        v["mlp_fused"] = v["mlp_fused"] and v["geglu_period"] == 32
        return cls(**v)


def pack_geglu(w: torch.Tensor, b: torch.Tensor, period: int = 64) -> Tuple[torch.Tensor, torch.Tensor]:
    n2, k = w.shape
    n = n2 // 2
    h = period // 2
    assert n % h == 0
    wv, wg = w[:n].reshape(n // h, h, k), w[n:].reshape(n // h, h, k)
    bv, bg = b[:n].reshape(n // h, h), b[n:].reshape(n // h, h)
    return torch.cat([wv, wg], dim=1).reshape(n2, k).contiguous(), torch.cat([bv, bg], dim=1).reshape(n2).contiguous()


def pack_conv_up2x(w: torch.Tensor) -> torch.Tensor:
    assert w.dim() == 4 and tuple(w.shape[2:]) == (3, 3) and w.dtype == torch.float32
    co, ci = w.shape[0], w.shape[1]
    rows = ((w[:, :, 0], w[:, :, 1] + w[:, :, 2]), (w[:, :, 0] + w[:, :, 1], w[:, :, 2]))
    out = w.new_empty(4, co, 4 * ci)
    for py in range(2):
        for px in range(2):
            taps = []
            for ty in range(2):
                r = rows[py][ty]
                cols = (r[:, :, 0], r[:, :, 1] + r[:, :, 2]) if px == 0 else (r[:, :, 0] + r[:, :, 1], r[:, :, 2])
                taps += [cols[0], cols[1]]
            out[py * 2 + px] = torch.stack(taps, dim=1).reshape(co, 4 * ci)
    return out


class Cond:

    _next_uid = 0

    def __init__(self, B: int):
        Cond._next_uid += 1
        self.uid = Cond._next_uid
        self.B = B
        self.objs: Optional[torch.Tensor] = None
        self.k_ctx: List[torch.Tensor] = []
        self.vt_ctx: List[torch.Tensor] = []
        self.k_obj: List[torch.Tensor] = []
        self.vt_obj: List[torch.Tensor] = []
        self.n_ctx = 0
        self.vis: List[torch.Tensor] = []

    @staticmethod
    def cat(conds: Sequence["Cond"]) -> "Cond":
        out = Cond(sum(c.B for c in conds))
        out.n_ctx = conds[0].n_ctx
        out.objs = torch.cat([c.objs for c in conds], 0)
        for name in ("k_ctx", "vt_ctx", "k_obj", "vt_obj", "vis"):
            lists = [getattr(c, name) for c in conds]
            setattr(out, name, [torch.cat(ts, 0) for ts in zip(*lists)])
        return out

    def _tensors(self):
        return [self.objs] + self.k_ctx + self.vt_ctx + self.k_obj + self.vt_obj + self.vis

    def clone(self) -> "Cond":
        out = Cond(self.B)
        out.n_ctx = self.n_ctx
        out.objs = self.objs.clone()
        for name in ("k_ctx", "vt_ctx", "k_obj", "vt_obj", "vis"):
            setattr(out, name, [t.clone() for t in getattr(self, name)])
        return out

    def copy_from(self, other: "Cond"):
        for dst, src in zip(self._tensors(), other._tensors()):
            dst.copy_(src)

    def same_layout(self, other: "Cond") -> bool:
        a, b = self._tensors(), other._tensors()
        return len(a) == len(b) and all(x.shape == y.shape for x, y in zip(a, b)) and self.n_ctx == other.n_ctx

    def select(self, idx: torch.Tensor) -> "Cond":
        out = Cond(int(idx.numel()))
        out.n_ctx = self.n_ctx
        out.objs = self.objs[idx].contiguous()
        for name in ("k_ctx", "vt_ctx", "k_obj", "vt_obj", "vis"):
            setattr(out, name, [t[idx].contiguous() for t in getattr(self, name)])
        return out


class UNetEngine(EngineBase):
    def __init__(self, model: UNetModel, ops=None, dtype: torch.dtype = torch.bfloat16, use_graphs: bool = True,
                 knobs: Optional[EngineKnobs] = None):
        super().__init__(ops, dtype, use_graphs)
        self.model = model
        self.heads = model.num_heads
        self.masked_fuser = not getattr(model, "efficient_attention", True)
        self.knobs = knobs or EngineKnobs.from_env()
        self._paired_checked: set = set()
        self._cond_cache: Dict[tuple, Cond] = {}
        self._slots: Dict[int, Cond] = {}
        self._slot_bound: Dict[int, int] = {}
        self.fuser_scale = None
        self._pack(model)
        self.set_fuser_scale(1.0)

    def _pack_up(self, m) -> dict:
        if self.knobs.up_fold and hasattr(self.ops, "conv_up2x"):
            return dict(kind="up", conv=None, fold=self._w16(pack_conv_up2x(m.weight.detach().float())), b=self._f32(m.bias), mod=m)
        return dict(kind="up", conv=self._conv(m), fold=None)

    def _up_conv3(self, p) -> _Lin:
        if p["conv"] is None:
            p["conv"] = self._conv(p["mod"])
        return p["conv"]

    def _pack_ff(self, ff, norm):
        w = ff.net[0].proj.weight.detach().float()
        g, b = norm.weight.detach().float(), norm.bias.detach().float()
        wp, dp = pack_geglu(w * g[None, :], ff.net[0].proj.bias.detach().float() + w @ b, self.knobs.geglu_period)
        w16 = self._w16(wp)
        f = dict(w1=w16, b1=self._f32(dp), c1=w16.float().sum(1).contiguous(), l2=self._lin(ff.net[2]))
        C = w.shape[1]
        if self.knobs.mlp_fused and hasattr(self.ops, "mlp_geglu") and self.ops.mlp_supported(128, C):
            f["cd"], f["w2p"] = self.ops.mlp_pack(w16, f["c1"], f["b1"], f["l2"].w)
        return f

    def _attn(self, a, norm, self_attn: bool):
        d = dict(out=self._lin(a.to_out[0]))
        if self_attn:
            w3, c3, d3 = self._fold_ln(torch.cat([a.to_q.weight.detach(), a.to_k.weight.detach(), a.to_v.weight.detach()], 0),
                                       None, norm)
            C2 = 2 * a.to_q.weight.shape[0]
            d["wqkv"], d["cqkv"], d["dqkv"] = w3, c3, d3
            d["wqk"], d["cqk"], d["dqk"] = w3[:C2], c3[:C2], d3[:C2]
            d["wv"], d["cv"], d["dv"] = w3[C2:], c3[C2:], d3[C2:]
        else:
            d["wq"], d["cq"], d["dq"] = self._fold_ln(a.to_q.weight, None, norm)
            d["wk"], d["wv"] = self._w16(a.to_k.weight), self._w16(a.to_v.weight)
        return d

    def _attn_kv_plain(self, a):
        return dict(wk=self._w16(a.to_k.weight), wv=self._w16(a.to_v.weight))

    def _pack_res(self, rb: ResBlock, emb_w: list, emb_b: list, off: list):
        p = dict(kind="res", cin=rb.channels, cout=rb.out_channels,
                 gn1=(self._f32(rb.in_layers[0].weight), self._f32(rb.in_layers[0].bias)),
                 conv1=self._conv(rb.in_layers[2]),
                 gn2=(self._f32(rb.out_layers[0].weight), self._f32(rb.out_layers[0].bias)),
                 conv2=self._conv(rb.out_layers[3]),
                 skip=None if isinstance(rb.skip_connection, torch.nn.Identity) else self._lin(rb.skip_connection),
                 emb_off=off[0])
        emb_w.append(rb.emb_layers[1].weight.detach().float())
        emb_b.append(rb.emb_layers[1].bias.detach().float())
        off[0] += rb.out_channels
        return p

    def _pack_st(self, st: SpatialTransformer, tanh_alphas: list):
        blk = st.transformer_blocks[0]
        fz = blk.fuser
        idx = len(tanh_alphas)
        tanh_alphas.append(torch.stack([torch.tanh(fz.alpha_attn.detach().float()),
                                        torch.tanh(fz.alpha_dense.detach().float())]))
        return dict(kind="st", c=st.in_channels, idx=idx,
                    norm=(self._f32(st.norm.weight), self._f32(st.norm.bias)),
                    proj_in=self._lin(st.proj_in), proj_out=self._lin(st.proj_out),
                    n1=(self._f32(blk.norm1.weight), self._f32(blk.norm1.bias)),
                    n2=(self._f32(blk.norm2.weight), self._f32(blk.norm2.bias)),
                    n3=(self._f32(blk.norm3.weight), self._f32(blk.norm3.bias)),
                    attn1=self._attn(blk.attn1, blk.norm1, True), attn2=self._attn(blk.attn2, blk.norm2, False),
                    ff=self._pack_ff(blk.ff, blk.norm3),
                    f_lin=self._lin(fz.linear), f_attn=self._attn(fz.attn, fz.norm1, True), f_kv=self._attn_kv_plain(fz.attn),
                    f_ff=self._pack_ff(fz.ff, fz.norm2),
                    f_n1=(self._f32(fz.norm1.weight), self._f32(fz.norm1.bias)),
                    f_n2=(self._f32(fz.norm2.weight), self._f32(fz.norm2.bias)))

    def _pack_layers(self, seq, emb_w, emb_b, off, tanh_alphas):
        out = []
        for _, layer in seq.items():
            if isinstance(layer, ResBlock):
                out.append(self._pack_res(layer, emb_w, emb_b, off))
            elif isinstance(layer, SpatialTransformer):
                out.append(self._pack_st(layer, tanh_alphas))
            elif isinstance(layer, Downsample):
                out.append(dict(kind="down", conv=self._conv(layer.op)))
            elif isinstance(layer, Upsample):
                out.append(self._pack_up(layer.conv))
            else:
                out.append(dict(kind="conv_in", w=self._f32(layer.weight), b=self._f32(layer.bias)))
        return out

    def _pack(self, model: UNetModel):
        emb_w, emb_b, off, tanh_alphas = [], [], [0], []
        self.te0 = self._lin(model.time_embed[0])
        self.te2 = self._lin(model.time_embed[2])
        self.in_blocks = [self._pack_layers(b, emb_w, emb_b, off, tanh_alphas) for b in model.input_blocks]
        self.mid_block = self._pack_layers(model.middle_block, emb_w, emb_b, off, tanh_alphas)
        self.out_blocks = [self._pack_layers(b, emb_w, emb_b, off, tanh_alphas) for b in model.output_blocks]
        self.emb_all = _Lin(self._w16(torch.cat(emb_w, 0)), self._f32(torch.cat(emb_b, 0)))
        self.emb_total = off[0]
        self.tanh_alphas = torch.stack(tanh_alphas).to(self.device)
        self.gates = torch.zeros_like(self.tanh_alphas)
        self.n_st = len(tanh_alphas)
        self.scaleu = []
        for i in range(len(model.output_blocks)):
            b = getattr(model, f"scaleu_b_{i}").detach().float()
            s = getattr(model, f"scaleu_s_{i}").detach().float()
            self.scaleu.append((self._f32(torch.tanh(b) + 1.0), self._f32(torch.tanh(s))))
        self.out_gn = (self._f32(model.out[0].weight), self._f32(model.out[0].bias))
        self.out_conv = self._conv_out_padded(model.out[2])
        self.n_out = model.out[2].weight.shape[0]
        self._pack_tokenizer(model.position_net)

    def repack_first_conv(self, conv):
        p = self.in_blocks[0][0]
        p["w"].copy_(conv.weight.detach().float())
        p["b"].copy_(conv.bias.detach().float())

    def _pack_tokenizer(self, pn):
        self.pn = pn
        self.tok_mlps = []
        for i in range(5):
            seq = pn.linears_list[i]
            self.tok_mlps.append([self._lin(seq[0]), self._lin(seq[2]), self._lin(seq[4])])
        self.tok_null = dict(
            text=self._f32(pn.null_positive_feature), box=self._f32(pn.null_position_feature),
            point=self._f32(pn.null_point_feature), scribble=self._f32(pn.null_scribble_feature),
            polygon=self._f32(pn.null_polygon_feature), seg=self._f32(pn.null_seg_feature))
        self.tok_pos = self._f32(pn.pos_embedding)
        self.tok_freqs = (100.0 ** (torch.arange(16) / 16)).to(device=self.device, dtype=torch.float32)
        self._pack_convnext(pn)

    def _pack_convnext(self, pn):
        bb = pn.convnext_tiny_backbone
        cn = dict(in_w=self._f32(pn.in_conv.weight), in_b=self._f32(pn.in_conv.bias), stages=[], down=[])
        stem = bb.downsample_layers[0]
        w = stem[0].weight.detach().float().reshape(stem[0].weight.shape[0], -1)
        wp = torch.zeros(w.shape[0], 64)
        wp[:, :w.shape[1]] = w
        cn["stem"] = _Lin(self._w16(wp), self._f32(stem[0].bias))
        cn["stem_ln"] = (self._f32(stem[1].weight), self._f32(stem[1].bias))
        for i in range(1, 4):
            dl = bb.downsample_layers[i]
            wd = dl[1].weight.detach().float()
            cn["down"].append(dict(ln=(self._f32(dl[0].weight), self._f32(dl[0].bias)),
                                   conv=_Lin(self._w16(wd.permute(0, 2, 3, 1).reshape(wd.shape[0], -1)),
                                             self._f32(dl[1].bias))))
        for i in range(4):
            blocks = []
            for _, blk in bb.stages[i].items():
                C = blk.dwconv.weight.shape[0]
                kpad = _round_up(C, 64)
                w1 = torch.zeros(4 * C, kpad)
                w1[:, :C] = blk.pwconv1.weight.detach().float()
                g = blk.gamma.detach().float()
                blocks.append(dict(
                    C=C, kpad=kpad,
                    dw_w=self._f32(blk.dwconv.weight.detach().float().reshape(C, 49).t().contiguous()),
                    dw_b=self._f32(blk.dwconv.bias), ln=(self._f32(blk.norm.weight), self._f32(blk.norm.bias)),
                    l1=_Lin(self._w16(w1), self._f32(blk.pwconv1.bias)),
                    l2=_Lin(self._w16(g[:, None] * blk.pwconv2.weight.detach().float()),
                            self._f32(g * blk.pwconv2.bias.detach().float()))))
            cn["stages"].append(blocks)
        self.cn = cn
        t = torch.arange(64)
        i = torch.arange(3072)
        self.seg_gather = (((i[None, :] % 4) * 4 + t[:, None] // 16) * 16 + (t[:, None] % 16)) * 768 + i[None, :] // 4
        self.seg_gather = self.seg_gather.to(self.device)

    def convnext_features(self, segs: torch.Tensor) -> torch.Tensor:
        ops, cn = self.ops, self.cn
        B, Cin, S, _ = segs.shape
        P = S // 4
        pm = ops.zeros((B * P * P, 64))
        ops.seg_in_conv(segs.contiguous(), cn["in_w"], cn["in_b"], pm)
        x = ops.gemm(pm, cn["stem"].w, ops.empty((B * P * P, cn["stem"].w.shape[0])), bias=cn["stem"].b)
        C = x.shape[1]
        x = ops.layernorm(x, ops.empty(x.shape), cn["stem_ln"][0], cn["stem_ln"][1], 1e-6).view(B, P, P, C)
        H = P
        for i in range(4):
            if i > 0:
                d = cn["down"][i - 1]
                pmat = ops.layernorm_patch2(x, ops.empty((B * (H // 2) * (H // 2), 4 * C)), d["ln"][0], d["ln"][1], 1e-6)
                H //= 2
                Cn = d["conv"].w.shape[0]
                x = ops.gemm(pmat, d["conv"].w, ops.empty((B * H * H, Cn)), bias=d["conv"].b).view(B, H, H, Cn)
                C = Cn
            M = B * H * H
            for blk in cn["stages"][i]:
                y = ops.dwconv7x7(x, blk["dw_w"], blk["dw_b"], ops.empty(x.shape))
                ln = ops.zeros((M, blk["kpad"])) if blk["kpad"] != C else ops.empty((M, C))
                ops.layernorm(y.view(M, C), ln[:, :C], blk["ln"][0], blk["ln"][1], 1e-6)
                hmid = ops.gemm(ln, blk["l1"].w, ops.empty((M, 4 * C)), bias=blk["l1"].b, act="gelu")
                ops.gemm(hmid, blk["l2"].w, x.view(M, C), bias=blk["l2"].b, res=x.view(M, C))
        return x

    def set_fuser_scale(self, scale: float):
        scale = float(scale)
        if scale != self.fuser_scale:
            self.fuser_scale = scale
            self.gates.copy_(self.tanh_alphas * scale)

    def sync_fuser_scale_from_modules(self):
        from .host.attention import GatedSelfAttentionDense
        for m in self.model.modules():
            if type(m) == GatedSelfAttentionDense:
                self.set_fuser_scale(m.scale)
                return

    def tokens(self, g: Dict[str, torch.Tensor]) -> torch.Tensor:
        ops, pn = self.ops, self.pn
        dev = self.device
        boxes = g["boxes"].to(dev, torch.float32)
        B, N, _ = boxes.shape
        m = g["masks"].to(dev, torch.float32).reshape(B * N)
        text = g["positive_embeddings"].to(dev, torch.float32).reshape(B * N, -1).contiguous()
        points = g.get("points")
        points = ((boxes[..., :2] + boxes[..., 2:]) / 2.0) if points is None else points.to(dev, torch.float32)
        scribbles = g["scribbles"].to(dev, torch.float32)
        polygons = g["polygons"].to(dev, torch.float32)
        drop_point, drop_box, drop_scribble, drop_polygons, drop_segs = pn.eval_drops()
        zero = torch.zeros_like(m)
        masks = [
            zero if drop_box else m,
            zero if drop_point else m,
            zero if drop_scribble else ((scribbles.sum(-1).reshape(-1) + m) > 0).float(),
            zero if drop_polygons else ((polygons.sum(-1).reshape(-1) + m) > 0).float(),
        ]
        locs = [boxes.reshape(B * N, 4), points.reshape(B * N, 2), scribbles.reshape(B * N, -1),
                polygons.reshape(B * N, -1)]
        nulls = [self.tok_null["box"], self.tok_null["point"], self.tok_null["scribble"], self.tok_null["polygon"]]
        objs = ops.zeros((B, OBJ_TOKENS, pn.out_dim))
        for i in range(4):
            loc = locs[i].contiguous()
            inp = ops.empty((B * N, text.shape[1] + 32 * loc.shape[1]))
            ops.unifusion_embed(text, loc, m.contiguous(), masks[i].contiguous(), self.tok_null["text"], nulls[i],
                                self.tok_freqs, inp)
            l0, l1, l2 = self.tok_mlps[i]
            h0 = ops.gemm(inp, l0.w, ops.empty((B * N, l0.w.shape[0])), bias=l0.b, act="silu")
            h1 = ops.gemm(h0, l1.w, ops.empty((B * N, l1.w.shape[0])), bias=l1.b, act="silu")
            ops.gemm(h1.view(B, N, -1), l2.w, objs[:, i * N:(i + 1) * N, :], bias=l2.b)
        segs = g["segs"]
        if segs.dim() == 4 and segs.shape[0] > 1 and segs.stride(0) == 0:
            segs = segs[:1]
        Bs = segs.shape[0]
        use_segs = (not drop_segs) and bool((segs.reshape(Bs, -1).sum(1) > 0).any())
        l0, l1, l2 = self.tok_mlps[4]
        null_in = self.tok_null["seg"].view(1, 1, -1) + self.tok_pos
        if use_segs:
            segs_r = segs.to(dev, torch.float32)
            if segs_r.shape[-1] != pn.resize_input:
                segs_r = torch.nn.functional.interpolate(segs_r, pn.resize_input, mode="nearest")
            feat = self.convnext_features(segs_r)
            sf = feat.reshape(Bs, -1).float()[:, self.seg_gather.reshape(-1)].reshape(Bs, 64, -1)
            sm = (segs_r.reshape(Bs, -1).sum(1) > 0).float().view(Bs, 1, 1)
            seg_in = sf * sm + (1 - sm) * self.tok_null["seg"].view(1, 1, -1) + self.tok_pos
            rows = Bs * 64
        else:
            seg_in, rows = null_in, 64
        seg_in = seg_in.reshape(rows, -1).contiguous()
        seg16 = ops.cast16(seg_in, ops.empty(seg_in.shape))
        h0 = ops.gemm(seg16, l0.w, ops.empty((rows, l0.w.shape[0])), bias=l0.b, act="silu")
        h1 = ops.gemm(h0, l1.w, ops.empty((rows, l1.w.shape[0])), bias=l1.b, act="silu")
        seg_tok = ops.gemm(h1, l2.w, ops.empty((rows, l2.w.shape[0])), bias=l2.b)
        objs[:, 4 * N:, :] = seg_tok.view(-1, 64, seg_tok.shape[-1])
        return objs

    def _st_layers(self):
        for blk in self.in_blocks + [self.mid_block] + self.out_blocks:
            for p in blk:
                if p["kind"] == "st":
                    yield p

    def prepare_cond(self, context: torch.Tensor, grounding: Dict[str, torch.Tensor]) -> Cond:
        ops = self.ops
        B, n_ctx, cd = context.shape
        c = Cond(B)
        c.n_ctx = n_ctx
        c.objs = self.tokens(grounding)
        if self.masked_fuser:
            from .host.attention import visibility_words
            am = grounding.get("att_masks")
            any_flag = grounding.get("att_masks_any")
            if am is None or self.pn.drop_box_mask or any_flag is False:
                am = torch.zeros(B, 1, MASK_RES, MASK_RES, device=self.device)
            assert am.shape[-2:] == (MASK_RES, MASK_RES), "the reference masks at the 64x64 resolution only"
            am = am.to(self.device)
            if am.shape[0] != B:
                am = am.expand(B, *am.shape[1:])
            n_objs = (OBJ_TOKENS - 64) // 4
            if am.shape[1] < n_objs:
                am = torch.cat([am, torch.zeros(B, n_objs - am.shape[1], MASK_RES, MASK_RES, device=self.device)], 1)
            c.vis = list(visibility_words(am, force_masked=bool(any_flag) and not self.pn.drop_box_mask))
        ctx16 = ops.cast16(context.to(self.device, torch.float32).contiguous(), ops.empty((B, n_ctx, cd)))
        ld_ctx, ld_obj = _round_up(n_ctx, 64), _round_up(OBJ_TOKENS, 64)
        for p in self._st_layers():
            C = p["c"]
            a2, fa = p["attn2"], p["f_kv"]
            k = ops.gemm(ctx16.view(B * n_ctx, cd), a2["wk"], ops.empty((B * n_ctx, C))).view(B, n_ctx, C)
            vt = ops.zeros((B, C, ld_ctx))
            ops.gemm(a2["wv"], ctx16, vt[:, :, :n_ctx])
            c.k_ctx.append(k)
            c.vt_ctx.append(vt)
            o = ops.gemm(c.objs.view(B * OBJ_TOKENS, -1), p["f_lin"].w, ops.empty((B * OBJ_TOKENS, C)), bias=p["f_lin"].b)
            ln = ops.layernorm(o, ops.empty((B * OBJ_TOKENS, C)), *p["f_n1"])
            ko = ops.gemm(ln, fa["wk"], ops.empty((B * OBJ_TOKENS, C))).view(B, OBJ_TOKENS, C)
            vo = ops.zeros((B, C, ld_obj))
            ops.gemm(fa["wv"], ln.view(B, OBJ_TOKENS, C), vo[:, :, :OBJ_TOKENS])
            c.k_obj.append(ko)
            c.vt_obj.append(vo)
        return c

    def _gnp(self, role, B, HW, C):
        shape = self.ops.gn_partial_shape(B, HW, C) if (self.knobs.gn_epi and hasattr(self.ops, "gn_partial_shape")) else None
        return None if shape is None else self.buf(role, shape, torch.float32)

    def _res(self, p, x, emb_all, out_role, gnp=None, want_out=True):
        ops = self.ops
        B, H, W, Cin = x.shape
        Cout = p["cout"]
        g = ops.groupnorm(x, self.buf("gn", x.shape), p["gn1"][0], p["gn1"][1], 1e-5, True, partial=gnp)
        rb = emb_all[:, p["emb_off"]:p["emb_off"] + Cout]
        p1 = self._gnp("gnp.h1", B, H * W, Cout)
        h1 = ops.conv3x3(g, p["conv1"].w, self.buf("rb.h1", (B, H, W, Cout)), bias=p["conv1"].b, rowbias=rb, gn_partial=p1)
        g2 = ops.groupnorm(h1, self.buf("gn", h1.shape), p["gn2"][0], p["gn2"][1], 1e-5, True, partial=p1)
        if p["skip"] is not None:
            xs = ops.gemm(x.view(B * H * W, Cin), p["skip"].w, self.buf("rb.skip", (B * H * W, Cout)),
                          bias=p["skip"].b).view(B, H, W, Cout)
        else:
            xs = x
        p2 = self._gnp("gnp.out", B, H * W, Cout) if want_out else None
        return ops.conv3x3(g2, p["conv2"].w, self.buf(out_role, (B, H, W, Cout)), bias=p["conv2"].b, res=xs, gn_partial=p2), p2

    def _self_attn(self, a, y, st, handed, B, N, C, kv_extra=None, vis=None):
        ops = self.ops
        if self._qkv_fused(N):
            vtg = self.buf("st.vtg", (C, B * N))
            qk = ops.gemm(y, a["wqkv"], self.buf("st.qk", (B * N, 2 * C)), bias=a["dqkv"], ln_row=(st if handed else None, a["cqkv"]),
                          ln_stats_out=None if handed else st, vt_out=vtg).view(B, N, 2 * C)
            vt = vtg.view(C, B, N).permute(1, 0, 2)
        else:
            qk = ops.gemm(y, a["wqk"], self.buf("st.qk", (B * N, 2 * C)), bias=a["dqk"], ln_row=(st if handed else None, a["cqk"]),
                          ln_stats_out=None if handed else st).view(B, N, 2 * C)
            ldv = _round_up(N, 64)
            vt = self.buf("st.vt", (B, C, ldv), zero=True)
            ops.gemm(a["wv"], y.view(B, N, C), vt[:, :, :N], ln_col=(st.view(B, N, 2), a["cv"], a["dv"]))
        att = self.buf("st.att", (B, N, C))
        k1, vt1 = kv_extra or (None, None)
        qbits, kbits0, kbits1 = vis or (None, None, None)
        ops.attention(qk[:, :, :C], qk[:, :, C:], vt, N, att, self.heads, k1=k1, vt1=vt1, n1=OBJ_TOKENS if kv_extra else 0,
                      qbits=qbits, kbits0=kbits0, kbits1=kbits1)
        return att

    def _qkv_fused(self, N):
        return self.knobs.vt_global and N % 64 == 0 and N >= self.knobs.vt_min_n

    def _ff(self, f, y, st, handed, M, C, gate=None, out_stats=None):
        ops = self.ops
        if handed and out_stats is None and self._ff_fused(f, M, C):
            return ops.mlp_geglu(y, st, f["w1"], f["cd"], f["w2p"], f["l2"].b, y, gate=gate)
        mid = ops.gemm(y, f["w1"], self.buf("st.ffmid", (M, 4 * C)), bias=f["b1"], geglu=True, geglu_period=self.knobs.geglu_period,
                       ln_row=(st if handed else None, f["c1"]))
        return ops.gemm(mid, f["l2"].w, y, bias=f["l2"].b, res=y, gate=gate, out_stats=out_stats)

    def _ff_fused(self, f, M, C):
        return "w2p" in f and M >= self.knobs.mlp_min_m and self.ops.mlp_supported(M, C)

    def _ln_routing(self, p, C, N, M, fuser_on):
        k = self.knobs
        ln_self = k.ln_self == 2 or (k.ln_self == 1 and C <= 320)
        qkv_self = ln_self and not (k.qkv_row and C == 320 and self._qkv_fused(N))
        takes = getattr(self.ops, "proj_row_takes", None)
        q_self = ln_self and not (k.ln_self == 1 and takes is not None and takes(M, C)
                                  and not (fuser_on and self._ff_fused(p["f_ff"], M, C)))
        handed = dict(attn1=not qkv_self, **(dict(f_attn=not qkv_self, f_ff=k.ln_self <= 1) if fuser_on else {}),
                      attn2=not q_self, ff=k.ln_self <= 1)
        return handed, dict(zip(["proj_in", *handed], [*handed.values(), False]))

    def _dup(self, t: torch.Tensor, role: str) -> torch.Tensor:
        n = t.shape[0]
        out = self.buf(role, (2 * n,) + tuple(t.shape[1:]), t.dtype)
        out[:n].copy_(t)
        out[n:].copy_(t)
        return out

    def _st(self, p, x, cond: Cond, fuser_on: bool, dup: bool = False, gnp=None):
        ops = self.ops
        B, H, W, C = x.shape
        N, M = H * W, B * H * W
        g = ops.groupnorm(x, self.buf("gn", x.shape), p["norm"][0], p["norm"][1], 1e-6, False, partial=gnp)
        st = self.buf("st.stats", (M, 2), torch.float32)
        handed, emits = self._ln_routing(p, C, N, 2 * M if dup else M, fuser_on)
        y = ops.gemm(g.view(M, C), p["proj_in"].w, self.buf("st.x", (M, C)), bias=p["proj_in"].b,
                     out_stats=st if emits["proj_in"] else None)
        att = self._self_attn(p["attn1"], y, st, handed["attn1"], B, N, C)
        ops.gemm(att.view(M, C), p["attn1"]["out"].w, y, bias=p["attn1"]["out"].b, res=y, out_stats=st if emits["attn1"] else None)
        if dup:
            x, y = self._dup(x, "st.x_in2"), self._dup(y.view(B, N, C), "st.x2").view(2 * M, C)
            st = (self._dup(st.view(B, N, 2), "st.stats2").view(2 * M, 2) if emits["attn1"]
                  else self.buf("st.stats", (2 * M, 2), torch.float32))
            B, M = 2 * B, 2 * M
        i = p["idx"]
        if fuser_on:
            vis = cond.vis if (cond.vis and N == MASK_RES * MASK_RES) else None
            att = self._self_attn(p["f_attn"], y, st, handed["f_attn"], B, N, C, kv_extra=(cond.k_obj[i], cond.vt_obj[i]), vis=vis)
            ops.gemm(att.view(M, C), p["f_attn"]["out"].w, y, bias=p["f_attn"]["out"].b, res=y, gate=self.gates[i, 0:1],
                     out_stats=st if emits["f_attn"] else None)
            self._ff(p["f_ff"], y, st, handed["f_ff"], M, C, gate=self.gates[i, 1:2], out_stats=st if emits["f_ff"] else None)
        a2 = p["attn2"]
        q = ops.gemm(y, a2["wq"], self.buf("st.q", (M, C)), bias=a2["dq"],
                     ln_row=(st if handed["attn2"] else None, a2["cq"])).view(B, N, C)
        att = self.buf("st.att", (B, N, C))
        ops.attention(q, cond.k_ctx[i], cond.vt_ctx[i], cond.n_ctx, att, self.heads)
        ops.gemm(att.view(M, C), a2["out"].w, y, bias=a2["out"].b, res=y, out_stats=st if emits["attn2"] else None)
        self._ff(p["ff"], y, st, handed["ff"], M, C)
        ops.gemm(y, p["proj_out"].w, x.view(M, C), bias=p["proj_out"].b, res=x.view(M, C))
        return x

    def _run_block(self, layers, h, x_nchw, emb_all, cond, fuser_on, out_role, dup_st: bool = False, gnp=None, next_kind=None):
        for j, p in enumerate(layers):
            k = p["kind"]
            nxt = layers[j + 1]["kind"] if j + 1 < len(layers) else next_kind
            norm_next = nxt in ("res", "st")
            if k == "conv_in":
                B, _, H, W = x_nchw.shape
                h = self.ops.conv_in(x_nchw, p["w"], p["b"], self.buf(out_role, (B, H, W, p["w"].shape[0])))
                gnp = None
            elif k == "res":
                h, gnp = self._res(p, h, emb_all, out_role, gnp, want_out=norm_next)
            elif k == "st":
                h = self._st(p, h, cond, fuser_on, dup=dup_st, gnp=gnp)
                gnp = None
            elif k == "down":
                B, H, W, C = h.shape
                Ho, Wo = (H + 1) // 2, (W + 1) // 2
                gnp = self._gnp("gnp.out", B, Ho * Wo, C) if norm_next else None
                h = self.ops.conv3x3(h, p["conv"].w, self.buf(out_role, (B, Ho, Wo, C)), bias=p["conv"].b, stride=2, gn_partial=gnp)
            elif k == "up":
                B, H, W, C = h.shape
                up = self.buf(out_role + ".up", (B, 2 * H, 2 * W, C))
                if p["fold"] is None or not self.ops.conv_up2x(h, p["fold"], up, bias=p["b"]):
                    conv = self._up_conv3(p)
                    self.ops.conv3x3(h, conv.w, up, bias=conv.b, upsample=1)
                h = up
                gnp = None
        return h, gnp

    def _forward_ops(self, x: torch.Tensor, t_f32: torch.Tensor, cond: Cond, eps: torch.Tensor, fuser_on: bool,
                     paired: bool = False):
        ops = self.ops
        B = x.shape[0]
        hoist = (paired and self.knobs.pair_hoist and B % 2 == 0 and len(self.in_blocks) > 1
                 and [p["kind"] for p in self.in_blocks[0]] == ["conv_in"] and [p["kind"] for p in self.in_blocks[1]] == ["res", "st"])
        n = B // 2
        mc = self.model.model_channels
        te = ops.timestep_embedding(t_f32, self.buf("temb.sin", (B, mc)))
        e1 = ops.gemm(te, self.te0.w, self.buf("temb.1", (B, 4 * mc)), bias=self.te0.b, act="silu")
        es = ops.gemm(e1, self.te2.w, self.buf("temb.2", (B, 4 * mc)), bias=self.te2.b, act="silu")
        emb_all = ops.gemm(es, self.emb_all.w, self.buf("temb.all", (B, self.emb_total)), bias=self.emb_all.b)
        hs = []
        h, gnp = None, None
        for i, layers in enumerate(self.in_blocks):
            nk = (self.in_blocks[i + 1] if i + 1 < len(self.in_blocks) else self.mid_block)[0]["kind"]
            if hoist and i == 0:
                h, gnp = self._run_block(layers, h, x[:n], emb_all[:n], cond, fuser_on, "in0.half")
                hs.append(self._dup(h, "in0"))
                continue
            if hoist and i == 1:
                h, gnp = self._run_block(layers, h, x[:n], emb_all[:n], cond, fuser_on, "in1.half", dup_st=True, gnp=gnp, next_kind=nk)
                hs.append(h)
                continue
            h, gnp = self._run_block(layers, h, x, emb_all, cond, fuser_on, f"in{i}", gnp=gnp, next_kind=nk)
            hs.append(h)
        h, gnp = self._run_block(self.mid_block, h, x, emb_all, cond, fuser_on, "mid", gnp=gnp)
        for i, layers in enumerate(self.out_blocks):
            skip = hs.pop()
            Bq, H, W, Ch = h.shape
            cat = ops.scaleu_concat(h, skip, self.buf("cat", (Bq, H, W, Ch + skip.shape[-1])), *self.scaleu[i])
            h, gnp = self._run_block(layers, cat, x, emb_all, cond, fuser_on, f"out{i}")
        g = ops.groupnorm(h, self.buf("gn", h.shape), self.out_gn[0], self.out_gn[1], 1e-5, True)
        ops.conv3x3(g, self.out_conv.w, eps, bias=self.out_conv.b, n_valid=self.n_out)
        return eps

    def _bind(self, cond: Cond) -> Cond:
        B = cond.B
# ... 74 lines not shown
```

instancediffusion_amd/ops.py:

```python
from __future__ import annotations

import ctypes as C
from typing import Optional

import torch

from . import _lib
from ._lib import (EPI_BIAS, EPI_GATE, EPI_GEGLU, EPI_GEGLU_P32, EPI_GELU, EPI_LN_COL, EPI_LN_ROW, EPI_OUT_F32, EPI_OUT_NCHW,
                   EPI_QUICKGELU, EPI_RES, EPI_ROWBIAS, EPI_SILU)

_DT = {torch.bfloat16: _lib.IDF_BF16, torch.float16: _lib.IDF_F16}


def _p(t: Optional[torch.Tensor]):
    return None if t is None else C.c_void_p(t.data_ptr())


def _rows2d(t: torch.Tensor):
    assert t.stride(-1) == 1 or t.shape[-1] == 1, "last dim must be contiguous"
    return t.stride(-2), (t.stride(0) if t.dim() == 3 else 0)


class HipOps:

# ... 74 lines not shown
        s_ln = 0
        if ln_row is not None:
            ln_stats, ln_c = ln_row
            assert bias is not None and ln_c.numel() == N
            assert ln_stats is None or (ln_stats.shape[-2] == M and ln_stats.dtype == torch.float32)
            if ln_stats is None:
                assert not batched
                if ln_stats_out is not None:
                    assert ln_stats_out.is_contiguous() and ln_stats_out.dtype == torch.float32 and ln_stats_out.numel() == 2 * M
            epi |= EPI_LN_ROW
        elif ln_col is not None:
            ln_stats, ln_c, ln_d = ln_col
            assert ln_stats.shape[-2] == N and ln_c.numel() == M and ln_d.numel() == M and ln_stats.dtype == torch.float32
            epi |= EPI_LN_COL
        if ln_stats is not None:
            assert ln_stats.is_contiguous() and ln_stats.shape[-1] == 2
            s_ln = ln_stats.stride(0) if (batched and ln_stats.dim() == 3) else 0
        if out_stats is not None:
            assert out_stats.is_contiguous() and out_stats.dtype == torch.float32 and out_stats.numel() == 2 * out.numel() // N
        args = _lib.GemmArgs(
            A=a.data_ptr(), W=w.data_ptr(), out=out.data_ptr(),
            bias=None if bias is None else bias.data_ptr(),
            rowbias=None if rowbias is None else rowbias.data_ptr(),
            res=None if res is None else res.data_ptr(),
            gate=None if gate is None else gate.data_ptr(),
            M=M, N=N, K=K, lda=lda, ldw=ldw, ldo=ldo, ldr=ldr,
            ld_rowbias=0 if rowbias is None else rowbias.stride(-2), rows_per_batch=rows_per_batch,
            batch=out.shape[0] if batched else 1, strideA=sA, strideW=sW, strideO=sO, strideR=sR,
            epi=epi, dtype=self.dt, ws=self._splitk_ws().data_ptr(), ws_bytes=self.SPLITK_WS_BYTES,
            ln_stats=None if ln_stats is None else ln_stats.data_ptr(), stride_ln_stats=s_ln,
            ln_c=None if ln_c is None else ln_c.data_ptr(), ln_d=None if ln_d is None else ln_d.data_ptr(),
            out_stats=None if out_stats is None else out_stats.data_ptr(), out_stats_eps=float(out_stats_eps),
            ln_eps=float(ln_eps), ln_stats_out=None if ln_stats_out is None else ln_stats_out.data_ptr(),
            vt_out=None if vt_out is None else vt_out.data_ptr(), ld_vt=0 if vt_out is None else vt_out.stride(0),
            vt_col0=0 if vt_out is None else out.shape[-1])
        _lib.check(self.lib.idf_gemm(C.byref(args), self._stream()), "idf_gemm")
        return out

    MLP_W2_PERM = (0, 1, 2, 3, 8, 9, 10, 11, 4, 5, 6, 7, 12, 13, 14, 15)

    def proj_row_takes(self, M: int, C: int) -> bool:
        if C != 320 or M % 32:
            return False
        min_m = self.lib.idf_get_stat(_lib.IDF_STAT_PROJ_ROW_MIN_M)
        return 0 < min_m <= M

    @staticmethod
    def mlp_supported(M: int, C: int) -> bool:
        return C == 320 and M % 128 == 0

    @classmethod
    def mlp_pack(cls, w1p16, c1, d1, w2_16):
        n2 = c1.numel()
        cd = torch.cat([c1.float().view(n2 // 64, 64), d1.float().view(n2 // 64, 64)], dim=1).contiguous()
        perm = torch.tensor(cls.MLP_W2_PERM, device=w2_16.device)
        n, k = w2_16.shape
        w2p = w2_16.view(n, k // 16, 16).index_select(2, perm).reshape(n, k).contiguous()
        return cd, w2p

    def mlp_geglu(self, x, stats, w1, cd, w2p, b2, out, *, gate=None):
        M, Cc = x.shape
        assert self.mlp_supported(M, Cc) and out.shape == x.shape and x.stride(-1) == 1 and out.stride(-1) == 1
        assert stats.is_contiguous() and stats.dtype == torch.float32 and stats.numel() == 2 * M
        assert w1.shape == (8 * Cc, Cc) and w2p.shape == (Cc, 4 * Cc) and cd.is_contiguous() and cd.numel() == 16 * Cc
        assert w1.stride(-1) == 1 and w2p.stride(-1) == 1 and b2.dtype == torch.float32 and cd.dtype == torch.float32
        args = _lib.MlpArgs(x=x.data_ptr(), ldx=x.stride(0), ln_stats=stats.data_ptr(), w1=w1.data_ptr(), ldw1=w1.stride(0),
                            cd=cd.data_ptr(), w2p=w2p.data_ptr(), ldw2=w2p.stride(0), b2=b2.data_ptr(),
                            gate=None if gate is None else gate.data_ptr(), out=out.data_ptr(), ldo=out.stride(0), M=M, C=Cc,
                            dtype=self.dt)
        _lib.check(self.lib.idf_mlp_geglu(C.byref(args), self._stream()), "idf_mlp_geglu")
        return out

    @staticmethod
    def gn_partial_shape(B, HW, C):
        return (B, HW // 64, 32, 2) if (HW % 64 == 0 and C % 32 == 0) else None

    def conv3x3(self, x, w, out, *, bias=None, rowbias=None, res=None, stride=1, upsample=0, n_valid=0, gn_partial=None):
        B, H, W_, Cin = x.shape
        assert x.stride(-1) == 1 and x.stride(1) == W_ * x.stride(2) and x.stride(0) == H * x.stride(1)
        Cout = w.shape[0]
        epi = 0
        if bias is not None:
            epi |= EPI_BIAS
        if rowbias is not None:
            epi |= EPI_ROWBIAS
        if res is not None:
            epi |= EPI_RES
        if n_valid:
            epi |= EPI_OUT_NCHW
            assert out.dtype == torch.float32 and out.is_contiguous()
            ldo = 0
        else:
            ldo = out.stride(2)
        args = _lib.ConvArgs(
            x=x.data_ptr(), W=w.data_ptr(), out=out.data_ptr(),
            bias=None if bias is None else bias.data_ptr(),
            rowbias=None if rowbias is None else rowbias.data_ptr(),
            res=None if res is None else res.data_ptr(),
            B=B, Hin=H, Win=W_, Cin=Cin, Cout=Cout, stride=stride, upsample=upsample,
            ldx=x.stride(2), ldo=ldo, ldr=0 if res is None else res.stride(2),
            ld_rowbias=0 if rowbias is None else rowbias.stride(-2), n_valid=n_valid, epi=epi, dtype=self.dt,
            ws=self._splitk_ws().data_ptr(), ws_bytes=self.SPLITK_WS_BYTES,
            gn_partial=None if gn_partial is None else gn_partial.data_ptr())
        if gn_partial is not None:
            assert gn_partial.dtype == torch.float32 and gn_partial.is_contiguous() and out.is_contiguous()
            assert tuple(gn_partial.shape) == self.gn_partial_shape(out.shape[0], out.shape[1] * out.shape[2], Cout)
        _lib.check(self.lib.idf_conv3x3(C.byref(args), self._stream()), "idf_conv3x3")
        return out

    def conv3x3_down(self, x, w, out, *, bias=None, res=None, gn_partial=None):
        B, H, W_, Cin = x.shape
        assert x.stride(-1) == 1 and x.stride(1) == W_ * x.stride(2) and x.stride(0) == H * x.stride(1)
        Cout = w.shape[0]
        assert tuple(out.shape) == (B, (H - 2) // 2 + 1, (W_ - 2) // 2 + 1, Cout) and out.stride(-1) == 1
        assert out.stride(1) == out.shape[2] * out.stride(2) and out.stride(0) == out.shape[1] * out.stride(1)
        epi = 0
        if bias is not None:
            epi |= EPI_BIAS
        if res is not None:
            epi |= EPI_RES
        args = _lib.ConvArgs(
            x=x.data_ptr(), W=w.data_ptr(), out=out.data_ptr(),
            bias=None if bias is None else bias.data_ptr(), rowbias=None,
            res=None if res is None else res.data_ptr(),
            B=B, Hin=H, Win=W_, Cin=Cin, Cout=Cout, stride=2, upsample=0,
            ldx=x.stride(2), ldo=out.stride(2), ldr=0 if res is None else res.stride(2),
            ld_rowbias=0, n_valid=0, epi=epi, dtype=self.dt,
            ws=self._splitk_ws().data_ptr(), ws_bytes=self.SPLITK_WS_BYTES,
            gn_partial=None if gn_partial is None else gn_partial.data_ptr())
        if gn_partial is not None:
            assert gn_partial.dtype == torch.float32 and gn_partial.is_contiguous() and out.is_contiguous()
            assert tuple(gn_partial.shape) == self.gn_partial_shape(out.shape[0], out.shape[1] * out.shape[2], Cout)
        _lib.check(self.lib.idf_conv3x3_down(C.byref(args), self._stream()), "idf_conv3x3_down")
        return out

    def conv_up2x(self, x, wf, out, *, bias=None) -> bool:
        B, H, W_, Cin = x.shape
        assert x.stride(-1) == 1 and x.stride(1) == W_ * x.stride(2) and x.stride(0) == H * x.stride(1)
        Cout = wf.shape[1]
        assert tuple(wf.shape) == (4, Cout, 4 * Cin) and wf.is_contiguous() and wf.dtype == self.dtype
        assert tuple(out.shape) == (B, 2 * H, 2 * W_, Cout) and out.stride(-1) == 1 and out.dtype == self.dtype
        assert out.stride(1) == out.shape[2] * out.stride(2) and out.stride(0) == out.shape[1] * out.stride(1)
        args = _lib.ConvArgs(
            x=x.data_ptr(), W=wf.data_ptr(), out=out.data_ptr(), bias=None if bias is None else bias.data_ptr(),
            rowbias=None, res=None, B=B, Hin=H, Win=W_, Cin=Cin, Cout=Cout, stride=1, upsample=1,
            ldx=x.stride(2), ldo=out.stride(2), ldr=0, ld_rowbias=0, n_valid=0, epi=0 if bias is None else EPI_BIAS,
            dtype=self.dt, ws=None, ws_bytes=0, gn_partial=None)
        rc = self.lib.idf_conv_up2x_folded(C.byref(args), self._stream())
        if rc == _lib.E_UNSUPPORTED:
            return False
        _lib.check(rc, "idf_conv_up2x_folded")
        return True

    def conv_in(self, x_nchw, w, bias, out):
        B, Cin, H, W_ = x_nchw.shape
        assert x_nchw.dtype == torch.float32 and x_nchw.is_contiguous() and out.is_contiguous()
        _lib.check(self.lib.idf_conv_in(_p(x_nchw), _p(w), _p(bias), _p(out), B, Cin, H, W_, out.shape[-1], self.dt,
                                        self._stream()), "idf_conv_in")
        return out

    def attention(self, q, k0, vt0, n0, out, heads, *, k1=None, vt1=None, n1=0, qbits=None, kbits0=None, kbits1=None):
        if qbits is not None:
            for t in (qbits, kbits0) + ((kbits1,) if n1 else ()):
                assert t.dtype == torch.int32 and t.stride(-1) == 1 and t.dim() == 2
        B, Nq, Cc = q.shape
        d = Cc // heads
        a = _lib.AttnArgs(
            q=q.data_ptr(), ldq=q.stride(1), strideQ=q.stride(0), nq=Nq,
            k0=k0.data_ptr(), ldk0=k0.stride(1), strideK0=k0.stride(0),
            vt0=vt0.data_ptr(), ldv0=vt0.stride(1), strideV0=vt0.stride(0), n0=n0,
            k1=None if k1 is None else k1.data_ptr(), ldk1=0 if k1 is None else k1.stride(1),
            strideK1=0 if k1 is None else k1.stride(0),
            vt1=None if vt1 is None else vt1.data_ptr(), ldv1=0 if vt1 is None else vt1.stride(1),
            strideV1=0 if vt1 is None else vt1.stride(0), n1=n1,
            out=out.data_ptr(), ldo=out.stride(1), strideO=out.stride(0),
            B=B, H=heads, d=d, scale=float(d) ** -0.5, dtype=self.dt,
            qbits=None if qbits is None else qbits.data_ptr(), strideQb=0 if qbits is None else qbits.stride(0),
            kbits0=None if qbits is None else kbits0.data_ptr(), strideKb0=0 if qbits is None else kbits0.stride(0),
            kbits1=None if (qbits is None or not n1) else kbits1.data_ptr(),
            strideKb1=0 if (qbits is None or not n1) else kbits1.stride(0))
        _lib.check(self.lib.idf_attention(C.byref(a), self._stream()), "idf_attention")
        return out

    def attention_causal(self, qkv, out, heads, T):
        Cc = out.shape[-1]
        B = out.shape[0] // T
        assert qkv.dim() == 2 and out.dim() == 2 and qkv.shape[-1] == 3 * Cc and qkv.shape[0] >= B * T and Cc % heads == 0
        assert qkv.stride(-1) == 1 and out.stride(-1) == 1 and qkv.dtype == self.dtype and out.dtype == self.dtype
        d = Cc // heads
        _lib.check(self.lib.idf_attention_causal(_p(qkv), qkv.stride(0), _p(out), out.stride(0), B, T, heads, d, float(d) ** -0.5,
                                                 self.dt, self._stream()), "idf_attention_causal")
        return out

    def clip_embed(self, ids_i32, tok_emb, pos_emb, out):
        B, T = ids_i32.shape
        vocab, Cc = tok_emb.shape
        assert ids_i32.dtype == torch.int32 and ids_i32.is_contiguous() and tok_emb.is_contiguous() and pos_emb.is_contiguous()
        assert tok_emb.dtype == self.dtype and pos_emb.dtype == self.dtype and out.dtype == self.dtype
        assert pos_emb.shape[0] >= T and pos_emb.shape[1] == Cc and out.shape[0] >= B * T and out.shape[1] == Cc and out.stride(-1) == 1
        _lib.check(self.lib.idf_clip_embed(_p(ids_i32), _p(tok_emb), _p(pos_emb), _p(out), out.stride(0), B, T, Cc, vocab, self.dt,
                                           self._stream()), "idf_clip_embed")
        return out

    ATTENTION_QKV_TMAX = _lib.ATTENTION_QKV_TMAX

    def attention_qkv(self, qkv, out, heads, T):
        Cc = out.shape[-1]
        B = out.shape[0] // T
        assert qkv.dim() == 2 and out.dim() == 2 and qkv.shape[-1] == 3 * Cc and qkv.shape[0] >= B * T and Cc % heads == 0
        assert qkv.stride(-1) == 1 and out.stride(-1) == 1 and qkv.dtype == self.dtype and out.dtype == self.dtype
        d = Cc // heads
        _lib.check(self.lib.idf_attention_qkv(_p(qkv), qkv.stride(0), _p(out), out.stride(0), B, T, heads, d, float(d) ** -0.5,
                                              self.dt, self._stream()), "idf_attention_qkv")
        return out

    def clip_patchify(self, pixels, patch, cls_row, x, patch_size):
        B, ch, S, S2 = pixels.shape
        G = S // patch_size
        Cc = cls_row.numel()
        assert ch == 3 and S == S2 and pixels.dtype == torch.float32 and pixels.is_contiguous()
        assert patch.dim() == 2 and patch.shape[0] >= B * G * G and patch.shape[1] == (3 * patch_size * patch_size + 63) // 64 * 64
        assert x.dim() == 2 and x.shape[0] >= B * (G * G + 1) and x.shape[1] == Cc and x.stride(-1) == 1 and patch.stride(-1) == 1
        assert patch.dtype == self.dtype and x.dtype == self.dtype and cls_row.dtype == self.dtype and cls_row.is_contiguous()
        _lib.check(self.lib.idf_clip_patchify(_p(pixels), _p(patch), patch.stride(0), _p(cls_row), _p(x), x.stride(0), B, S, patch_size,
                                              Cc, self.dt, self._stream()), "idf_clip_patchify")
        return patch

    CLIP_RESIZE_KMAX = _lib.CLIP_RESIZE_KMAX

    def clip_crop_resize(self, src, crops, tables, ntab, lut, out, K):
        import numpy as np
        if src.dtype == torch.uint8:
            kind, (B, H, W, ch) = _lib.IDF_CLIP_SRC_U8, src.shape
        else:
            kind, (B, ch, H, W) = _lib.IDF_CLIP_SRC_F32, src.shape
            assert src.dtype == torch.float32
        Ncrop, S = out.shape[0], out.shape[-1]
        assert ch == 3 and src.is_contiguous() and src.is_cuda and out.is_contiguous() and out.dtype == torch.float32
        assert tuple(out.shape) == (Ncrop, 3, S, S) and lut.dtype == torch.float32 and tuple(lut.shape) == (3, 256) and lut.is_contiguous()
        assert isinstance(crops, np.ndarray) and crops.dtype == np.int32 and crops.shape == (Ncrop, 8) and crops.flags.c_contiguous
        assert tables.dtype == torch.int32 and tables.is_contiguous() and tables.numel() >= Ncrop * 8 + ntab * (4 * S + 2 * K * S)
        _lib.check(self.lib.idf_clip_crop_resize(_p(src), kind, B, H, W, C.c_void_p(crops.ctypes.data), Ncrop, _p(tables), int(ntab),
                                                 _p(lut), _p(out), S, int(K), self._stream()), "idf_clip_crop_resize")
        return out

    def rle_decode_planes(self, table, dst_plane, out, area=None, zero=True):
        import numpy as np
        ends, rb, re, hw = (np.ascontiguousarray(table[k]) for k in ("ends", "run_begin", "run_end", "src_hw"))
        dst = np.ascontiguousarray(np.asarray(dst_plane, dtype=np.int64))
        M, S = int(rb.shape[0]), int(out.shape[-1])
        P = out.numel() // (S * S) if S else 0
        if not (out.is_cuda and out.dtype == torch.float32 and out.is_contiguous() and out.dim() >= 2 and out.shape[-2] == S):
            raise ValueError("rle_decode_planes: out must be a contiguous fp32 [.., S, S] tensor on the device")
        if S < 1 or S % 4 or P * S * S >= 2 ** 31:
            raise ValueError(f"rle_decode_planes: S = {S} must be a positive multiple of 4 and out smaller than 2^31 elements")
        if not (ends.dtype == np.uint32 and rb.dtype == np.int32 and re.dtype == np.int32 and hw.dtype == np.int32):
            raise ValueError("rle_decode_planes: not a pack_masks table")
        if re.shape != (M,) or hw.shape != (M, 2) or dst.shape != (M,):
            raise ValueError(f"rle_decode_planes: {M} jobs need {M} run ranges, source sizes and destination planes")
        if M and (rb.min() < 0 or (rb > re).any() or re.max() > ends.size or dst.min() < 0 or dst.max() >= P or hw.min() < 1
                  or int(hw.max()) * S >= 2 ** 31 or len(set(dst.tolist())) != M):
            raise ValueError("rle_decode_planes: a run range, source size or destination plane is out of range, or a plane is named twice")
        if area is None:
            area = torch.zeros(M, dtype=torch.int32, device=out.device)
        else:
            assert area.is_cuda and area.dtype == torch.int32 and area.is_contiguous() and area.numel() == M
            area.zero_()
        if zero:
            out.zero_()
        if M == 0:
            return out, area
        ints = np.concatenate([rb, re, hw.reshape(-1), dst.astype(np.int32), ends.view(np.int32)])
        dev = torch.from_numpy(ints).to(out.device)
        base, n_ends = dev.data_ptr(), int(ends.size)
        at = lambda k: C.c_void_p(base + 4 * k * M)
        _lib.check(self.lib.idf_rle_decode_planes(C.c_void_p(base + 20 * M), n_ends, at(0), at(1), at(2), at(4), M, _p(out), P, S,
                                                  _p(area), self._stream()), "idf_rle_decode_planes")
        return out, area

    def groupnorm(self, x, out, gamma, beta, eps, silu, partial=None):
        assert x.is_contiguous() and out.is_contiguous()
        B, Cc = x.shape[0], x.shape[-1]
        HW = x.numel() // (B * Cc)
        if partial is not None:
            assert partial.dtype == torch.float32 and partial.is_contiguous() and partial.shape[0] == B and partial.shape[2:] == (32, 2)
            _lib.check(self.lib.idf_groupnorm_apply(_p(x), _p(out), _p(gamma), _p(beta), _p(partial), B, HW, Cc,
                                                    int(partial.shape[1]), float(eps), int(bool(silu)), self.dt,
                                                    self._stream()), "idf_groupnorm_apply")
            return out
        ws = self._workspace("gn", self.lib.idf_groupnorm_ws_floats(B, HW))
        _lib.check(self.lib.idf_groupnorm(_p(x), _p(out), _p(gamma), _p(beta), _p(ws), B, HW, Cc, float(eps),
                                          int(bool(silu)), self.dt, self._stream()), "idf_groupnorm")
        return out

    def layernorm(self, x, out, gamma, beta, eps=1e-5):
        M, Cc = x.shape
        _lib.check(self.lib.idf_layernorm(_p(x), x.stride(0), _p(out), out.stride(0), _p(gamma), _p(beta), M, Cc,
                                          float(eps), self.dt, self._stream()), "idf_layernorm")
        return out

    def row_stats(self, x, stats, eps=1e-5):
        M, Cc = x.shape
        assert stats.is_contiguous() and stats.dtype == torch.float32 and stats.numel() == 2 * M
        _lib.check(self.lib.idf_row_stats(_p(x), x.stride(0), _p(stats), M, Cc, float(eps), self.dt, self._stream()),
                   "idf_row_stats")
        return stats
# ... 184 lines not shown
```

Before: 2.120 img/s.

## Fold ResBlock 1x1 skip projection into conv2 as extra K-tiles

For ResBlocks whose skip connection is a 1x1 projection, the skip weights are concatenated onto the packed conv2 weights and the biases summed. The big GEMM kernel gains a SKIPK mode whose loader reads a tenth 'tap' from the block input x. This removes the separate skip GEMM launch and the round trip of its output through memory as a residual. The cost is a longer K dimension, extra template instantiations, and a fallback to the old path when shapes are unsupported (Cout not a multiple of 320, no big mode).

```diff
diff --git a/include/idf.h b/include/idf.h
--- a/include/idf.h
+++ b/include/idf.h
@@ -41,7 +41,8 @@
        IDF_STAT_PROJ_ROW_LAUNCHES = 8 ,
        IDF_STAT_PROJ_ROW_MIN_M = 9 ,
        IDF_STAT_ATTN_RES_LAUNCHES = 10 ,
-       IDF_STAT_CLIP_PREPROC_LAUNCHES = 12  };
+       IDF_STAT_CLIP_PREPROC_LAUNCHES = 12 ,
+       IDF_STAT_SKIP_FOLD_LAUNCHES = 13  };
 long long idf_get_stat(int stat);
 
 typedef struct {
@@ -93,6 +94,16 @@
 int idf_conv3x3(const idf_conv3x3_args* a, void* stream);
 int idf_conv3x3_down(const idf_conv3x3_args* a, void* stream);
 int idf_conv_up2x_folded(const idf_conv3x3_args* a, void* stream);
+typedef struct {
+  const void* g; const void* x; const void* W; void* out;
+  const float* bias;
+  int B, H, Wd, C2, Cx, Cout;
+  int ldg, ldx, ldo;
+  int dtype;
+  void* ws; long long ws_bytes;
+  float* gn_partial;
+} idf_conv3x3_skip_args;
+int idf_conv3x3_skip(const idf_conv3x3_skip_args* a, void* stream);
 
 int idf_conv_in(const float* x_nchw, const float* w , const float* bias, void* out,
                 int B, int Cin, int H, int W, int Cout, int dtype, void* stream);
diff --git a/instancediffusion_amd/_lib.py b/instancediffusion_amd/_lib.py
--- a/instancediffusion_amd/_lib.py
+++ b/instancediffusion_amd/_lib.py
@@ -12,6 +12,7 @@
 IDF_STAT_PROJ_ROW_LAUNCHES, IDF_STAT_PROJ_ROW_MIN_M = 8, 9
 IDF_STAT_ATTN_RES_LAUNCHES = 10
 IDF_STAT_CLIP_PREPROC_LAUNCHES = 12
+IDF_STAT_SKIP_FOLD_LAUNCHES = 13
 IDF_CLIP_SRC_U8, IDF_CLIP_SRC_F32 = 0, 1
 CLIP_RESIZE_KMAX = 32
 IDF_TUNE_PROJ_ROW = 9
@@ -48,6 +49,12 @@
                 ("n_valid", ci), ("epi", ci), ("dtype", ci), ("ws", vp), ("ws_bytes", ll), ("gn_partial", vp)]
 
 
+class ConvSkipArgs(C.Structure):
+    _fields_ = [("g", vp), ("x", vp), ("W", vp), ("out", vp), ("bias", vp),
+                ("B", ci), ("H", ci), ("Wd", ci), ("C2", ci), ("Cx", ci), ("Cout", ci),
+                ("ldg", ci), ("ldx", ci), ("ldo", ci), ("dtype", ci), ("ws", vp), ("ws_bytes", ll), ("gn_partial", vp)]
+
+
 class AttnArgs(C.Structure):
     _fields_ = [("q", vp), ("ldq", ci), ("strideQ", ll), ("nq", ci),
                 ("k0", vp), ("ldk0", ci), ("strideK0", ll), ("vt0", vp), ("ldv0", ci), ("strideV0", ll), ("n0", ci),
@@ -71,6 +78,7 @@
     "idf_conv3x3": (ci, [C.POINTER(ConvArgs), vp]),
     "idf_conv3x3_down": (ci, [C.POINTER(ConvArgs), vp]),
     "idf_conv_up2x_folded": (ci, [C.POINTER(ConvArgs), vp]),
+    "idf_conv3x3_skip": (ci, [C.POINTER(ConvSkipArgs), vp]),
     "idf_mlp_geglu": (ci, [C.POINTER(MlpArgs), vp]),
     "idf_conv_in": (ci, [vp, vp, vp, vp, ci, ci, ci, ci, ci, ci, vp]),
     "idf_attention": (ci, [C.POINTER(AttnArgs), vp]),
diff --git a/instancediffusion_amd/csrc/gemm_big.hip b/instancediffusion_amd/csrc/gemm_big.hip
--- a/instancediffusion_amd/csrc/gemm_big.hip
+++ b/instancediffusion_amd/csrc/gemm_big.hip
@@ -35,12 +35,13 @@
   }
 }
 template <int DT, int BM, int BN, int TN, bool SPLIT, bool LNS = false, bool STATS = false, bool GLU = false, bool GST = false,
-          bool QG = true >
+          bool QG = true ,
+          int EPI_MASK = -1 >
 __device__ __forceinline__ void big_epilogue(const CoreParams& p, f32x16 (&acc)[TN][TM], int seq, int slice, int tiles_n, int wm,
                                              int wn, int l31_in, int hi_in, float gate, char* stg_in, const float* lnm = nullptr,
                                              const float* lnr = nullptr) {
   constexpr int WN = BN / 2;
-  const int epi = p.epi;
+  const int epi = p.epi & EPI_MASK;
   int l31 = l31_in, hi = hi_in;
   asm volatile("" : "+v"(l31), "+v"(hi));
   char* const stg = stg_in;
@@ -454,7 +455,7 @@
 #endif
 
 template <int DT, int BM, int BN, int BKT, int NSTG, bool CONV, bool SPLIT, bool LNS = false, bool VT = false, bool STATS = false,
-          bool GLU = false, bool GST = false, bool FOLD = false>
+          bool GLU = false, bool GST = false, bool FOLD = false, bool SKIPK = false>
 __global__ __launch_bounds__(64 * NWAVES, 1) void gemm_kernel_big(const CoreParams p, const int tiles_total) {
   constexpr int WN = BN / 2, TN = WN / 32;
   constexpr int NW = NWAVES;
@@ -493,6 +494,7 @@
   auto swz = [](int row) { return CPR == 8 ? ((row >> 1) & 7) : ((row >> 2) & 3); };
   unsigned woff[W_INST], aoff[A_INST];
   int ayx[A_INST];
+  [[maybe_unused]] int l_m0 = 0;
   int l_seq, l_kt = 0, l_k0 = 0, l_nk = 0, tap = 0, ci0 = 0;
 
   auto setup_loader = [&](int item) {
@@ -503,6 +505,7 @@
     const int m_tile = tile / tiles_n;
     const int n0 = (tile - m_tile * tiles_n) * BN, m0 = m_tile * BM;
     l_k0 = slice * nk;
+    if constexpr (SKIPK) l_m0 = m0;
 #pragma unroll
     for (int j = 0; j < W_INST; ++j) {
       const int row = RPI * (wave + NW * j) + dr;
@@ -529,7 +532,7 @@
           continue;
         }
         const int y0 = yo * p.stride - p.pad_lo, x0 = xo * p.stride - p.pad_lo;
-        if (p.up == 0) {
+        if (SKIPK || p.up == 0) {
           int mask = 0;
 #pragma unroll
           for (int t = 0; t < 9; ++t) {
@@ -547,7 +550,8 @@
         aoff[j] = (unsigned)m * (unsigned)p.lda + sw;
       }
     }
-    if (CONV) conv_tap_at(p, l_k0 * BKT, tap, ci0);
+    if constexpr (SKIPK) conv_tap_at_skip(p, l_k0 * BKT, tap, ci0);
+    else if (CONV) conv_tap_at(p, l_k0 * BKT, tap, ci0);
   };
 
   auto issue_piece = [&](int stage, auto II) {
@@ -564,6 +568,18 @@
         const bool ok = (ayx[j] >> tap) & 1;
         const unsigned short* src = ok ? p.A + (aoff[j] + tapoff) : idf_zero_page + dc * 8;
         dma16_v(src, dst);
+      } else if constexpr (SKIPK) {
+        if (tap == 9) {
+          const int row = RPI * (wave + NW * j) + dr;
+          const unsigned off2 = (unsigned)min(l_m0 + row, p.M - 1) * (unsigned)p.lda2 + (unsigned)((dc ^ swz(row)) * 8 + ci0);
+          dma16_v(p.A2 + off2, dst);
+        } else {
+          const int ky = tap / 3, kx = tap - ky * 3;
+          const unsigned tapoff = (unsigned)((ky * p.Win + kx) * p.lda + ci0);
+          const bool ok = (ayx[j] >> tap) & 1;
+          const unsigned short* src = ok ? p.A + (aoff[j] + tapoff) : idf_zero_page + dc * 8;
+          dma16_v(src, dst);
+        }
       } else if (CONV && p.up == 0) {
         const int ky = tap / 3, kx = tap - ky * 3;
         const unsigned tapoff = (unsigned)((ky * p.Win + kx) * p.lda + ci0);
@@ -584,7 +600,8 @@
     }
   };
   auto advance_loader = [&]() {
-    if (CONV) conv_tap_step(p, BKT, tap, ci0);
+    if constexpr (SKIPK) conv_tap_step_skip(p, BKT, tap, ci0);
+    else if (CONV) conv_tap_step(p, BKT, tap, ci0);
     if (++l_kt == l_nk) {
       l_kt = 0;
       l_seq += seq_step;
@@ -745,7 +762,7 @@
     } else if constexpr (FOLD) {
       big_epilogue_fold<DT, BM, BN, TN>(p, acc, tile, ph, tiles_n, wm, wn, l31, hi);
     } else {
-      big_epilogue<DT, BM, BN, TN, SPL, LNS, STATS, GLU, GST, !CONV>(p, acc, tile, slice, tiles_n, wm, wn, l31, hi, gate, stg, lnm, lnr);
+      big_epilogue<DT, BM, BN, TN, SPL, LNS, STATS, GLU, GST, !CONV, SKIPK ? IDF_EPI_BIAS : -1>(p, acc, tile, slice, tiles_n, wm, wn, l31, hi, gate, stg, lnm, lnr);
     }
     TR(4)
     young_stores = 0;
@@ -782,20 +799,21 @@
   return g_num_cu;
 }
 
-enum : unsigned { KB_CONV = 1, KB_SPLIT = 2, KB_LNS = 4, KB_VT = 8, KB_STATS = 16, KB_GLU = 32, KB_GST = 64, KB_FOLD = 128 };
+enum : unsigned { KB_CONV = 1, KB_SPLIT = 2, KB_LNS = 4, KB_VT = 8, KB_STATS = 16, KB_GLU = 32, KB_GST = 64, KB_FOLD = 128, KB_SKIP = 256 };
 
 template <int DT, int BN, int NSTG, unsigned FLAGS = 0>
 int launch_big_cfg(const CoreParams& p, hipStream_t s, int splitk = 1) {
   constexpr int BM = 256, BKT = 64;
   constexpr bool CONV = FLAGS & KB_CONV, SPLIT = FLAGS & KB_SPLIT, LNS = FLAGS & KB_LNS, VT = FLAGS & KB_VT, STATS = FLAGS & KB_STATS,
-                 GLU = FLAGS & KB_GLU, GST = FLAGS & KB_GST, FOLD = FLAGS & KB_FOLD;
-  if constexpr (!(FLAGS & ~KB_CONV) && NSTG == 2) {
-    if (splitk > 1) return launch_big_cfg<DT, BN, NSTG, (FLAGS & KB_CONV) | KB_SPLIT>(p, s, splitk);
+                 GLU = FLAGS & KB_GLU, GST = FLAGS & KB_GST, FOLD = FLAGS & KB_FOLD, SKIPK = FLAGS & KB_SKIP;
+  static_assert(!SKIPK || (CONV && !FOLD), "the shortcut K-tiles extend the plain 3x3 conv only");
+  if constexpr (!(FLAGS & ~(KB_CONV | KB_SKIP)) && NSTG == 2) {
+    if (splitk > 1) return launch_big_cfg<DT, BN, NSTG, (FLAGS & (KB_CONV | KB_SKIP)) | KB_SPLIT>(p, s, splitk);
   }
   if constexpr (!(FLAGS & (KB_SPLIT | KB_LNS | KB_CONV | KB_STATS | KB_GST)) && NSTG == 2) {
     if ((p.epi & IDF_EPI_LN_ROW) && !p.ln_stats) return launch_big_cfg<DT, BN, NSTG, (FLAGS & (KB_VT | KB_GLU)) | KB_LNS>(p, s, 1);
   }
-  void (*kern)(const CoreParams, const int) = gemm_kernel_big<DT, BM, BN, BKT, NSTG, CONV, SPLIT, LNS, VT, STATS, GLU, GST, FOLD>;
+  void (*kern)(const CoreParams, const int) = gemm_kernel_big<DT, BM, BN, BKT, NSTG, CONV, SPLIT, LNS, VT, STATS, GLU, GST, FOLD, SKIPK>;
   constexpr int smem = NSTG * (BM + BN) * BKT * 2 + NWAVES * 2048;
   static std::atomic<unsigned long long> attr_done{0};
   if (const int e = idf_lds_optin(reinterpret_cast<const void*>(kern), smem, attr_done)) return e;
@@ -854,6 +872,10 @@
   const bool vt = p.vt_out != nullptr;
   if (vt && (conv || geglu || (p.N % 320) || (p.vt_col0 % 320) || p.vt_col0 <= 0 || p.vt_col0 >= p.N || (p.M % 16) || (p.ld_vt % 8) ||
              !aligned16(p.vt_out) || (p.epi & ~(IDF_EPI_BIAS | IDF_EPI_LN_ROW)))) return IDF_BIG_UNSUPPORTED;
+  const bool skip = p.A2 != nullptr;
+  if (skip && (!conv || p.stride != 1 || p.up != 0 || p.pad_lo != 1 || p.Cin <= 0 || (p.Cin % BK) || p.Cx <= 0 || (p.Cx % BK) ||
+               p.K != 9 * p.Cin + p.Cx || (p.N % 320) || (p.lda2 % 8) || !aligned16(p.A2) || (p.epi & ~IDF_EPI_BIAS) ||
+               p.Ho != p.Hin || p.Wo != p.Win)) return IDF_BIG_UNSUPPORTED;
   int bn = 0;
   if (geglu && (p.epi & IDF_EPI_GEGLU_P32)) bn = (p.N % 320 == 0) ? 320 : ((p.N % 256 == 0) ? 256 : 0);
   else if (geglu) bn = (p.N % 256 == 0) ? 256 : 0;
@@ -903,6 +925,7 @@
   {
     const unsigned long long rows = conv ? (unsigned long long)(p.M / (p.Ho * p.Wo)) * p.Hin * p.Win : (unsigned long long)p.M;
     if (rows * (unsigned long long)p.lda >= (1ull << 31) || (unsigned long long)p.N * p.ldw >= (1ull << 31)) return IDF_BIG_UNSUPPORTED;
+    if (skip && (unsigned long long)p.M * (unsigned long long)p.lda2 >= (1ull << 31)) return IDF_BIG_UNSUPPORTED;
   }
   ++idf_stat_big_launches;
   const bool stats = parts_out && p.stat_parts && !conv && !geglu && !vt && !self_ln && splitk == 1 && bn != 128 &&
@@ -925,6 +948,8 @@
     if (conv) return launch_big_cfg<DT, 128, 3, KB_CONV>(p, s);                                                           \
     return launch_big_cfg<DT, 128, 3>(p, s);                                                                              \
   }                                                                                                                       \
+  if (skip) return gst ? launch_big_cfg<DT, 320, 2, KB_CONV | KB_GST | KB_SKIP>(p, s)                                     \
+                       : launch_big_cfg<DT, 320, 2, KB_CONV | KB_SKIP>(pq, s, splitk);                                    \
   if (gst) return launch_big_cfg<DT, 320, 2, KB_CONV | KB_GST>(p, s);                                                     \
   if (conv) return bn == 320 ? launch_big_cfg<DT, 320, 2, KB_CONV>(pq, s, splitk) : launch_big_cfg<DT, 256, 2, KB_CONV>(pq, s, splitk);   \
   return bn == 320 ? launch_big_cfg<DT, 320, 2>(pq, s, splitk) : launch_big_cfg<DT, 256, 2>(pq, s, splitk);
diff --git a/instancediffusion_amd/csrc/gemm_conv.hip b/instancediffusion_amd/csrc/gemm_conv.hip
--- a/instancediffusion_amd/csrc/gemm_conv.hip
+++ b/instancediffusion_amd/csrc/gemm_conv.hip
@@ -423,6 +423,7 @@
 
 std::atomic<long long> idf_stat_gn_epi_launches{0};
 std::atomic<long long> idf_stat_ring_launches{0};
+std::atomic<long long> idf_stat_skip_fold_launches{0};
 std::atomic<long long> idf_stat_gegluw_launches{0};
 std::atomic<long long> idf_stat_qkvw_launches{0};
 std::atomic<long long> idf_stat_projw_launches{0};
@@ -636,6 +637,7 @@
   if (stat == IDF_STAT_PROJ_ROW_MIN_M) return gemm_big_mode() > 0 ? idf_projw_min_rows() : 0;
   if (stat == IDF_STAT_ATTN_RES_LAUNCHES) return idf_stat_attn_res_launches.load();
   if (stat == IDF_STAT_CLIP_PREPROC_LAUNCHES) return idf_stat_clip_preproc_launches.load();
+  if (stat == IDF_STAT_SKIP_FOLD_LAUNCHES) return idf_stat_skip_fold_launches.load();
   return -1;
 }
 
@@ -796,3 +798,48 @@
   const int rc = idf_launch_big_fold(p, a->dtype, big == 2, (hipStream_t)stream);
   return rc == IDF_BIG_UNSUPPORTED ? IDF_E_UNSUPPORTED : rc;
 }
+
+extern "C" int idf_conv3x3_skip(const idf_conv3x3_skip_args* a, void* stream) {
+  if (!a || !a->g || !a->x || !a->W || !a->out) return IDF_E_ARG;
+  if (a->B <= 0 || a->H <= 0 || a->Wd <= 0 || a->Cout <= 0) return IDF_E_ARG;
+  if (a->C2 <= 0 || (a->C2 % BK) != 0 || a->Cx <= 0 || (a->Cx % BK) != 0) return IDF_E_ARG;
+  if (a->ldg < a->C2 || a->ldx < a->Cx || a->ldo < a->Cout) return IDF_E_ARG;
+  if ((a->ldg % 8) || (a->ldx % 8) || (a->ldo % 8) || !aligned16(a->g) || !aligned16(a->x) || !aligned16(a->W) || !aligned16(a->out) ||
+      (a->bias && !aligned16(a->bias))) return IDF_E_ALIGN;
+  const long long hw = (long long)a->H * a->Wd;
+  if (hw * a->B >= (1ll << 31) || 9ll * a->C2 + a->Cx >= (1ll << 24)) return IDF_E_ARG;
+  if (a->gn_partial) {
+    if ((hw % 64) || (a->Cout % 32) || a->ldo != a->Cout) return IDF_E_ARG;
+    if (((uintptr_t)a->gn_partial) & 7u) return IDF_E_ALIGN;
+  }
+  if (a->dtype != IDF_BF16 && a->dtype != IDF_F16) return IDF_E_UNSUPPORTED;
+  const int big = gemm_big_mode();
+  if (big == 0 || (a->Cout % 320) != 0) return IDF_E_UNSUPPORTED;
+  CoreParams p{};
+  p.Ho = a->H; p.Wo = a->Wd; p.Hin = a->H; p.Win = a->Wd; p.Cin = a->C2; p.stride = 1; p.up = 0; p.pad_lo = 1;
+  p.K = 9 * a->C2 + a->Cx;
+  p.W = (const unsigned short*)a->W; p.ldw = p.K; p.N = a->Cout; p.n_valid = a->Cout;
+  p.A = (const unsigned short*)a->g; p.lda = a->ldg; p.M = a->B * a->H * a->Wd;
+  p.A2 = (const unsigned short*)a->x; p.lda2 = a->ldx; p.Cx = a->Cx;
+  p.out = a->out; p.ldo = a->ldo; p.bias = a->bias; p.epi = a->bias ? IDF_EPI_BIAS : 0; p.rows_per_batch = a->H * a->Wd;
+  p.ws = (float*)a->ws; p.ws_bytes = a->ws ? (size_t)a->ws_bytes : 0;
+  if (a->gn_partial) { p.gn_partial = a->gn_partial; p.gn_hw = (int)hw; }
+  const long long tiles_small = (long long)((p.N + 127) / 128) * ((p.M + 127) / 128);
+  if (big != 2 && gemm_ring_tiles() > 0 && tiles_small <= 128 && tiles_small <= gemm_ring_tiles()) return IDF_E_UNSUPPORTED;
+  hipStream_t s = (hipStream_t)stream;
+  int splitk = 1, tail_m0 = 0, gst = 0;
+  int rc = idf_launch_big(p, a->dtype, true, big == 2, s, &splitk, nullptr, big == 3 ? &tail_m0 : nullptr, &gst);
+  if (rc == IDF_BIG_UNSUPPORTED) return IDF_E_UNSUPPORTED;
+  if (rc == 0 && splitk > 1) {
+    CoreParams q = p;
+    q.splitk = splitk; q.tail_m0 = tail_m0; q.tail_rows = p.M - tail_m0;
+    if (a->dtype == IDF_BF16) launch_reduce<IDF_BF16>(q, s);
+    else launch_reduce<IDF_F16>(q, s);
+    rc = idf_launch_status();
+  }
+  if (rc == 0) ++idf_stat_skip_fold_launches;
+  if (rc == 0 && gst) ++idf_stat_gn_epi_launches;
+  if (rc == 0 && a->gn_partial && !gst)
+    rc = idf_groupnorm_stats(a->out, a->gn_partial, a->B, (int)hw, a->Cout, (int)hw / 64, a->dtype, stream);
+  return rc;
+}
diff --git a/instancediffusion_amd/csrc/gemm_core.h b/instancediffusion_amd/csrc/gemm_core.h
--- a/instancediffusion_amd/csrc/gemm_core.h
+++ b/instancediffusion_amd/csrc/gemm_core.h
@@ -22,6 +22,7 @@
   int tile_walk; int dephase; int dephase_units; int epi_vmcnt;
   int pad_lo;
   int fold_tiles;
+  const unsigned short* A2; int lda2; int Cx;
 };
 
 constexpr int BK = 64;
@@ -64,6 +65,14 @@
 __device__ __forceinline__ void conv_tap_step(const CoreParams& p, int bk, int& tap, int& ci0) {
   ci0 += bk;
   if (ci0 >= p.Cin) { ci0 = 0; ++tap; }
+}
+__device__ __forceinline__ void conv_tap_at_skip(const CoreParams& p, int k_elem, int& tap, int& ci0) {
+  tap = min(k_elem / p.Cin, 9);
+  ci0 = k_elem - tap * p.Cin;
+}
+__device__ __forceinline__ void conv_tap_step_skip(const CoreParams& p, int bk, int& tap, int& ci0) {
+  ci0 += bk;
+  if (tap < 9 && ci0 >= p.Cin) { ci0 = 0; ++tap; }
 }
 __device__ __forceinline__ bool conv_tap_inside(int yi, int xi, int Hup, int Wup) { return (yi >= 0) & (yi < Hup) & (xi >= 0) & (xi < Wup); }
 
diff --git a/instancediffusion_amd/engine.py b/instancediffusion_amd/engine.py
--- a/instancediffusion_amd/engine.py
+++ b/instancediffusion_amd/engine.py
@@ -29,13 +29,15 @@
     pair_hoist: bool = True
     gn_epi: bool = True
     up_fold: bool = True
+    skip_fold: bool = True
     vt_global: bool = True
     vt_min_n: int = 256
     debug_paired: bool = False
 
     _ENV = (("ln_self", "IDF_LN_SELF", "1", int), ("qkv_row", "IDF_QKV_ROW", "1", lambda s: s != "0"), ("geglu_period", "IDF_GEGLU_PERIOD", "32", int),
             ("mlp_fused", "IDF_MLP_FUSED", "1", bool), ("mlp_min_m", "IDF_MLP_MIN_M", "32768", int), ("pair_hoist", "IDF_PAIR_HOIST", "1", bool),
-            ("gn_epi", "IDF_GN_EPI", "1", bool), ("up_fold", "IDF_UP_FOLD", "1", bool), ("vt_global", "IDF_VT_GLOBAL", "1", lambda s: s != "0"),
+            ("gn_epi", "IDF_GN_EPI", "1", bool), ("up_fold", "IDF_UP_FOLD", "1", bool), ("skip_fold", "IDF_SKIP_FOLD", "1", bool),
+            ("vt_global", "IDF_VT_GLOBAL", "1", lambda s: s != "0"),
             ("vt_min_n", "IDF_VT_MIN_N", "256", int), ("debug_paired", "IDF_DEBUG_PAIRED", "0", lambda s: s == "1"))
 
     def __post_init__(self):
@@ -85,6 +87,13 @@
                 taps += [cols[0], cols[1]]
             out[py * 2 + px] = torch.stack(taps, dim=1).reshape(co, 4 * ci)
     return out
+
+
+def pack_conv3x3_skip(w_conv: torch.Tensor, b_conv: torch.Tensor, w_skip: torch.Tensor, b_skip: torch.Tensor):
+    assert w_conv.dim() == 4 and tuple(w_conv.shape[2:]) == (3, 3) and w_conv.dtype == w_skip.dtype
+    w_skip = w_skip.reshape(w_skip.shape[0], w_skip.shape[1])
+    assert w_skip.shape[0] == w_conv.shape[0]
+    return torch.cat([pack_conv3x3(w_conv), w_skip], dim=1).contiguous(), b_conv + b_skip
 
 
 class Cond:
@@ -202,7 +211,11 @@
                  gn2=(self._f32(rb.out_layers[0].weight), self._f32(rb.out_layers[0].bias)),
                  conv2=self._conv(rb.out_layers[3]),
                  skip=None if isinstance(rb.skip_connection, torch.nn.Identity) else self._lin(rb.skip_connection),
-                 emb_off=off[0])
+                 emb_off=off[0], tail=None)
+        if p["skip"] is not None and self.knobs.skip_fold and hasattr(self.ops, "conv3x3_skip"):
+            wt, bt = pack_conv3x3_skip(rb.out_layers[3].weight.detach().float(), rb.out_layers[3].bias.detach().float(),
+                                       rb.skip_connection.weight.detach().float(), rb.skip_connection.bias.detach().float())
+            p["tail"] = _Lin(self._w16(wt), self._f32(bt))
         emb_w.append(rb.emb_layers[1].weight.detach().float())
         emb_b.append(rb.emb_layers[1].bias.detach().float())
         off[0] += rb.out_channels
@@ -476,13 +489,16 @@
         p1 = self._gnp("gnp.h1", B, H * W, Cout)
         h1 = ops.conv3x3(g, p["conv1"].w, self.buf("rb.h1", (B, H, W, Cout)), bias=p["conv1"].b, rowbias=rb, gn_partial=p1)
         g2 = ops.groupnorm(h1, self.buf("gn", h1.shape), p["gn2"][0], p["gn2"][1], 1e-5, True, partial=p1)
+        p2 = self._gnp("gnp.out", B, H * W, Cout) if want_out else None
+        out = self.buf(out_role, (B, H, W, Cout))
+        if p["tail"] is not None and ops.conv3x3_skip(g2, p["tail"].w, x, out, bias=p["tail"].b, gn_partial=p2):
+            return out, p2
         if p["skip"] is not None:
             xs = ops.gemm(x.view(B * H * W, Cin), p["skip"].w, self.buf("rb.skip", (B * H * W, Cout)),
                           bias=p["skip"].b).view(B, H, W, Cout)
         else:
             xs = x
-        p2 = self._gnp("gnp.out", B, H * W, Cout) if want_out else None
-        return ops.conv3x3(g2, p["conv2"].w, self.buf(out_role, (B, H, W, Cout)), bias=p["conv2"].b, res=xs, gn_partial=p2), p2
+        return ops.conv3x3(g2, p["conv2"].w, out, bias=p["conv2"].b, res=xs, gn_partial=p2), p2
 
     def _self_attn(self, a, y, st, handed, B, N, C, kv_extra=None, vis=None):
         ops = self.ops
diff --git a/instancediffusion_amd/ops.py b/instancediffusion_amd/ops.py
--- a/instancediffusion_amd/ops.py
+++ b/instancediffusion_amd/ops.py
@@ -250,6 +250,31 @@
         _lib.check(rc, "idf_conv_up2x_folded")
         return True
 
+    def conv3x3_skip(self, g2, w_packed, x, out, *, bias=None, gn_partial=None) -> bool:
+        B, H, W_, C2 = g2.shape
+        Cx, Cout = x.shape[-1], w_packed.shape[0]
+        for t in (g2, x, out):
+            assert t.shape[:3] == (B, H, W_) and t.dtype == self.dtype
+            assert t.stride(-1) == 1 and t.stride(1) == W_ * t.stride(2) and t.stride(0) == H * t.stride(1)
+        assert tuple(w_packed.shape) == (Cout, 9 * C2 + Cx) and w_packed.is_contiguous() and w_packed.dtype == self.dtype
+        assert out.shape[-1] == Cout
+        if bias is not None:
+            assert bias.dtype == torch.float32 and bias.is_contiguous() and bias.numel() == Cout
+        if gn_partial is not None:
+            assert gn_partial.dtype == torch.float32 and gn_partial.is_contiguous() and out.is_contiguous()
+            assert tuple(gn_partial.shape) == self.gn_partial_shape(B, H * W_, Cout)
+        args = _lib.ConvSkipArgs(
+            g=g2.data_ptr(), x=x.data_ptr(), W=w_packed.data_ptr(), out=out.data_ptr(),
+            bias=None if bias is None else bias.data_ptr(), B=B, H=H, Wd=W_, C2=C2, Cx=Cx, Cout=Cout,
+            ldg=g2.stride(2), ldx=x.stride(2), ldo=out.stride(2), dtype=self.dt,
+            ws=self._splitk_ws().data_ptr(), ws_bytes=self.SPLITK_WS_BYTES,
+            gn_partial=None if gn_partial is None else gn_partial.data_ptr())
+        rc = self.lib.idf_conv3x3_skip(C.byref(args), self._stream())
+        if rc == _lib.E_UNSUPPORTED:
+            return False
+        _lib.check(rc, "idf_conv3x3_skip")
+        return True
+
     def conv_in(self, x_nchw, w, bias, out):
         B, Cin, H, W_ = x_nchw.shape
         assert x_nchw.dtype == torch.float32 and x_nchw.is_contiguous() and out.is_contiguous()
```

Result: faster. 2.146 img/s (median of 6 runs) (+1.2%).
